# vthost/DAGNN

Hardware: AMD Instinct MI355X
Metric: graphs/sec (higher is better)
Workload: dtype f32

## Files before the change

### dagnn_amd/_lib.py

```python
from __future__ import annotations

import ctypes as C
import os
import threading

from . import build as _build

MAX_DIRS = 2
MAX_GROUPS = 4
MAX_READOUT_JOBS = 24
ATTN_GRAD_MAX_JOBS = 16

DAGNN_OK = 0
_ERRORS = {-22: "DAGNN_EINVAL (bad argument)", -28: "DAGNN_ENOSPC (workspace too small)"}


class DagnnHipError(RuntimeError):
    pass


class OptTensor(C.Structure):
    _fields_ = [("param", C.c_void_p), ("grad", C.c_void_p), ("exp_avg", C.c_void_p), ("exp_avg_sq", C.c_void_p), ("numel", C.c_int64)]


# ... 205 lines not shown

class DvaeSampleArgs(C.Structure):
    _fields_ = [("G", C.c_int64), ("B", C.c_int64), ("n", C.c_int), ("hs", C.c_int), ("L", C.c_int), ("nvt", C.c_int),
                ("start_type", C.c_int), ("end_type", C.c_int), ("bn", C.c_int), ("stochastic", C.c_int),
                ("edge_hidden", C.c_int), ("vertex_hidden", C.c_int), ("h0", C.c_void_p),
                ("w_ih", C.c_void_p * MAX_STACKED), ("w_hh", C.c_void_p * MAX_STACKED), ("b_ih", C.c_void_p * MAX_STACKED),
                ("b_hh", C.c_void_p * MAX_STACKED), ("w_key", C.c_void_p), ("vid_bias", C.c_void_p),
                ("av_w1", C.c_void_p), ("av_b1", C.c_void_p), ("av_w2", C.c_void_p), ("av_b2", C.c_void_p),
                ("ae_w1", C.c_void_p), ("ae_b1", C.c_void_p), ("ae_w2", C.c_void_p), ("ae_b2", C.c_void_p),
                ("u_type", C.c_void_p), ("u_edge", C.c_void_p), ("types", C.c_void_p), ("preds", C.c_void_p),
                ("nv", C.c_void_p), ("states", C.c_void_p), ("work", C.c_void_p), ("work_bytes", C.c_size_t),
                ("agg", C.c_int), ("gate_w", C.c_void_p), ("gate_b", C.c_void_p), ("mapper_w", C.c_void_p)]


DVAE_ENAS, DVAE_BN = 0, 1
DVAE_FIRST_VALID, DVAE_MOST_FREQUENT = 0, 1


class DvaeSelectArgs(C.Structure):
    _fields_ = [("A", C.c_int64), ("B", C.c_int64), ("n", C.c_int), ("nvt", C.c_int), ("start_type", C.c_int),
                ("end_type", C.c_int), ("kind", C.c_int), ("n_nodes", C.c_int), ("select", C.c_int),
                ("types", C.c_void_p), ("preds", C.c_void_p), ("nv", C.c_void_p), ("valid", C.c_void_p),
                ("pick", C.c_void_p), ("n_valid", C.c_void_p), ("n_same", C.c_void_p), ("work", C.c_void_p),
                ("work_bytes", C.c_size_t)]


LP_INT64, LP_FLOAT32, LP_FLOAT64 = 0, 1, 2
PREDICTOR_MAX_NZ, PREDICTOR_MAX_HS, PREDICTOR_ROWS = 128, 1024, 8
DVAE_SET_GRAPHS, DVAE_SET_KEYS = 0, 1
DVAE_SET_MAX_ROWS = 1 << 20
DVAE_SET_HEADER_WORDS, DVAE_SET_COUNT, DVAE_SET_ERR = 16, 4, 5
DVAE_SET_ERR_FULL, DVAE_SET_ERR_HEADER = 1, 2


class DvaeSameDagArgs(C.Structure):
    _fields_ = [("A", C.c_int64), ("B", C.c_int64), ("n", C.c_int), ("types", C.c_void_p), ("preds", C.c_void_p),
                ("nv", C.c_void_p), ("types_true", C.c_void_p), ("preds_true", C.c_void_p), ("nv_true", C.c_void_p),
                ("same", C.c_void_p), ("per_graph", C.c_void_p), ("total", C.c_void_p)]


class DvaeSet(C.Structure):
    _fields_ = [("form", C.c_int), ("width", C.c_int), ("max_rows", C.c_int64), ("data", C.c_void_p), ("bytes", C.c_size_t)]


class DvaeSetRowsArgs(C.Structure):
    _fields_ = [("set", DvaeSet), ("base", C.c_int64), ("A", C.c_int64), ("B", C.c_int64), ("types", C.c_void_p),
                ("preds", C.c_void_p), ("nv", C.c_void_p), ("keys", C.c_void_p), ("mask", C.c_void_p),
                ("member", C.c_void_p), ("count", C.c_void_p)]


class VariantBwdCell(C.Structure):
    _fields_ = [("mode", C.c_int32), ("lands", C.c_int32), ("in_dim", C.c_int32), ("proj_dim", C.c_int32),
                ("recurrent", C.c_int32), ("reserved", C.c_int32)] + \
        [(k, C.c_void_p) for k in ("h", "a", "gi", "gh", "node0", "node1", "alpha", "edge_mat0", "edge_vec0", "edge_mat1",
                                   "edge_vec1", "w_node", "w_query", "w_hh", "w_ih", "g", "g_in", "da", "dgi", "dgh",
                                   "dnode0", "dnode1", "dlogit", "esum", "w_node2")] + \
        [("w_ld", C.c_int32), ("ld_in", C.c_int32), ("ties", C.c_void_p)]


class VariantBwdArgs(C.Structure):
    _fields_ = [("cell", (VariantBwdCell * MAX_STACKED) * MAX_DIRS), ("num_stacked", C.c_int), ("dir_mask", C.c_int),
                ("H", C.c_int), ("ld", C.c_int)]


class VariantArgs(C.Structure):
    _fields_ = [("cell", (VariantCell * MAX_STACKED) * MAX_DIRS), ("num_stacked", C.c_int), ("dir_mask", C.c_int),
                ("H", C.c_int)]


class PrepTable(C.Structure):
    _fields_ = [("type_emb", C.c_void_p), ("attr_emb", C.c_void_p), ("depth_emb", C.c_void_p), ("out", C.c_void_p),
                ("width", C.c_int), ("ld_out", C.c_int)]


PREPARE_MAX_TABLES = 3


class PrepareRows(C.Structure):
    _fields_ = [("x", C.c_void_p), ("depth", C.c_void_p), ("max_depth", C.c_int), ("num_tables", C.c_int),
                ("table", PrepTable * PREPARE_MAX_TABLES), ("stack_src", C.c_void_p * 4), ("stack_out", C.c_void_p)]


class StoreGatherArgs(C.Structure):
    _fields_ = [(k, C.c_void_p) for k in ("node_ptr", "edge_ptr", "tok_ptr", "x", "depth", "layer_f", "layer_b", "src", "dst",
                                          "tok", "depth_max", "y_arr", "ref_ids", "ref_extra", "idx", "offsets")] + \
        [(k, C.c_int64) for k in ("ld_offsets", "B", "N", "E", "S", "R")] + \
        [(k, C.c_void_p) for k in ("out_x", "out_depth", "out_edge_index", "out_edge_attr", "out_batch", "out_ptr",
                                   "out_index0", "out_index1", "out_layer_f", "out_layer_b", "out_llp", "out_y_arr",
                                   "out_ref_ids", "out_ref_extra")]


class DagStoreGatherArgs(C.Structure):
    _fields_ = [(k, C.c_void_p) for k in ("types", "preds", "succs", "layer_f", "layer_b", "y", "idx", "offsets")] + \
        [(k, C.c_int64) for k in ("B", "n", "nvt", "E")] + \
        [(k, C.c_void_p) for k in ("out_x", "out_edge_index", "out_bi_layer_index", "out_batch", "out_ptr", "out_types",
                                   "out_preds", "out_y")]


BN_TABLE_CELLS, BN_MAX_VARS = 8192, 30
BN_STAGE_AUTO, BN_STAGE_LDS, BN_STAGE_GLOBAL = 0, 1, 2


class BnData(C.Structure):
    _fields_ = [("cols", C.c_void_p), ("ld", C.c_int64), ("S", C.c_int64), ("n_var", C.c_int32), ("reserved", C.c_int32),
                ("cards", C.c_int32 * BN_MAX_VARS)]


TABLE_GRADS_MAX_TABLES, TABLE_GRADS_CHUNK = 3, 32


class TableGradsTable(C.Structure):
    _fields_ = [("keys", C.c_void_p), ("key_stride", C.c_int64), ("R", C.c_int64), ("out", C.c_void_p), ("ld_out", C.c_int64)]


class TableGradsArgs(C.Structure):
    _fields_ = [("g", C.c_void_p), ("ld_g", C.c_int64), ("N", C.c_int64), ("H", C.c_int32), ("num_tables", C.c_int32),
                ("table", TableGradsTable * TABLE_GRADS_MAX_TABLES), ("workspace", C.c_void_p), ("workspace_bytes", C.c_size_t),
                ("stages", C.c_int32), ("reserved", C.c_int32)]


TABLE_GRADS_INDEX, TABLE_GRADS_SUM = 1, 2


SGP_MAX_M, SGP_MAX_D, SGP_MAX_Q = 512, 128, 128
SGP_ARGMIN_MEAN, SGP_ARGMIN_EI = 0, 1
SGP_REFINE_MAX_STARTS, SGP_REFINE_HISTORY = 32, 8
SGP_REFINE_MEAN, SGP_REFINE_EI = 0, 1
SGP_REFINE_STATUS = ("running", "converged", "stalled", "budget", "dead")

SYMBOLS = {
    "dagnn_version": (C.c_char_p, []),
    "dagnn_store_gather": (C.c_int, [C.POINTER(StoreGatherArgs), C.c_void_p]),
    "dagnn_dag_store_gather": (C.c_int, [C.POINTER(DagStoreGatherArgs), C.c_void_p]),
    "dagnn_dag_store_layers": (C.c_int, [C.c_void_p, C.c_void_p, C.c_int64, C.c_int, C.c_void_p, C.c_void_p, C.c_void_p]),
    "dagnn_plan_bytes": (C.c_size_t, [C.c_int64, C.c_int64, C.c_int64, C.c_int]),
    "dagnn_plan_is_small": (C.c_int, [C.c_int64, C.c_int64, C.c_int64]),
    "dagnn_plan_layout": (C.c_int, [C.c_int64, C.c_int64, C.c_int64, C.c_int, C.POINTER(C.c_int64)]),
    "dagnn_plan_build": (C.c_int, [C.POINTER(Plan), C.c_void_p, C.c_void_p, C.c_void_p, C.c_void_p, C.c_void_p,
                                   C.c_void_p, C.c_void_p]),
    "dagnn_prepare": (C.c_int, [C.POINTER(Plan), C.c_void_p, C.c_void_p, C.c_void_p, C.c_void_p, C.c_void_p, C.c_void_p,
                                C.c_void_p, C.c_size_t, C.c_int, C.c_int, C.c_int, C.POINTER(PrepareRows), C.c_void_p]),
    "dagnn_encode_ast": (C.c_int, [C.c_void_p, C.c_void_p, C.c_void_p, C.c_void_p, C.c_void_p, C.c_int, C.c_void_p,
                                   C.c_int, C.c_int64, C.c_int, C.c_void_p]),
    "dagnn_gemm_nt_bias": (C.c_int, [C.POINTER(GemmGroup), C.c_int, C.c_int64, C.c_int, C.c_int, C.c_int, C.c_int,
                                     C.c_int, C.c_void_p]),
    "dagnn_pack_whh": (C.c_int, [C.c_void_p, C.c_void_p, C.c_int, C.c_void_p]),
    "dagnn_recurrence_layer": (C.c_int, [C.POINTER(Plan), C.POINTER(LayerArgs), C.c_int, C.c_int, C.c_void_p]),
    "dagnn_pack_slices": (C.c_int, [C.c_void_p, C.c_void_p, C.c_int, C.c_int, C.c_int, C.c_void_p]),
    "dagnn_pack_batch": (C.c_int, [C.POINTER(PackJob), C.c_int, C.c_void_p]),
    "dagnn_pack_mfma": (C.c_int, [C.c_void_p, C.c_void_p, C.c_int, C.c_int, C.c_void_p]),
    "dagnn_frontier_run": (C.c_int, [C.POINTER(Plan), C.POINTER(FrontierArgs), C.POINTER(C.POINTER(C.c_int32)),
                                     C.POINTER(C.c_int32), C.c_void_p]),
    "dagnn_dataflow_groups": (C.c_int, [C.c_int, C.c_int, C.c_int, C.c_int, C.c_int64]),
    "dagnn_dataflow_bytes": (C.c_size_t, [C.c_int64, C.c_int64, C.c_int]),
    "dagnn_dataflow_layout": (C.c_int, [C.c_int64, C.c_int64, C.c_int, C.POINTER(C.c_int64)]),
    "dagnn_dataflow_schedule": (C.c_int, [C.POINTER(Plan), C.c_void_p, C.c_size_t, C.c_int, C.c_int, C.c_int,
                                          C.c_void_p, C.c_void_p]),
    "dagnn_dataflow_run": (C.c_int, [C.POINTER(Plan), C.POINTER(DataflowArgs), C.c_void_p]),
    "dagnn_dataflow_run_wide": (C.c_int, [C.POINTER(Plan), C.POINTER(DataflowArgs), C.c_void_p]),
    "dagnn_tiles_launches": (C.c_int, [C.c_int, C.c_int, C.c_int, C.c_int, C.c_int]),
    "dagnn_tiles_run": (C.c_int, [C.POINTER(Plan), C.POINTER(TilesArgs), C.c_void_p]),
    "dagnn_pack_dataflow": (C.c_int, [C.c_void_p, C.c_void_p, C.c_int, C.c_void_p]),
    "dagnn_pack_dataflow_transposed": (C.c_int, [C.c_void_p, C.c_void_p, C.c_int, C.c_void_p]),
    "dagnn_score_parts": (C.c_int, [C.c_void_p, C.c_int, C.c_int, C.c_void_p, C.c_int64, C.c_void_p]),
    "dagnn_backward_prepare": (C.c_int, [C.POINTER(Plan), C.POINTER(BackwardArgs), C.c_void_p]),
    "dagnn_backward_run": (C.c_int, [C.POINTER(Plan), C.POINTER(BackwardArgs), C.POINTER(C.POINTER(C.c_int32)),
                                     C.POINTER(C.c_int32), C.c_void_p]),
    "dagnn_bwd_dataflow_record_bytes": (C.c_size_t, [C.c_int64]),
    "dagnn_bwd_dataflow_static_bytes": (C.c_size_t, [C.c_int64]),
    "dagnn_bwd_dataflow_static_bytes_h": (C.c_size_t, [C.c_int64, C.c_int]),
    "dagnn_bwd_dataflow_prepare": (C.c_int, [C.POINTER(Plan), C.POINTER(BwdDataflowArgs), C.c_void_p]),
    "dagnn_bwd_dataflow_run": (C.c_int, [C.POINTER(Plan), C.POINTER(BwdDataflowArgs), C.c_void_p]),
    "dagnn_bwd_dataflow_run_wide": (C.c_int, [C.POINTER(Plan), C.POINTER(BwdDataflowArgs), C.c_void_p]),
    "dagnn_colsum_workspace_bytes": (C.c_size_t, [C.c_int, C.c_int]),
    "dagnn_colsum_run": (C.c_int, [C.POINTER(ColsumJob), C.c_int, C.c_int64, C.c_void_p, C.c_size_t, C.c_void_p]),
    "dagnn_wgrad_workspace_bytes": (C.c_size_t, [C.c_int, C.c_int, C.c_int, C.c_int]),
    "dagnn_wgrad_splits": (C.c_int, [C.c_int, C.c_int, C.c_int, C.c_int, C.c_int64]),
    "dagnn_wgrad_run": (C.c_int, [C.POINTER(WgradJob), C.c_int, C.c_int64, C.c_int, C.c_int, C.c_int, C.c_void_p,
                                  C.c_size_t, C.c_void_p]),
    "dagnn_table_grads_workspace_bytes": (C.c_size_t, [C.c_int64, C.c_int, C.POINTER(C.c_int64), C.c_int]),
    "dagnn_table_grads": (C.c_int, [C.POINTER(TableGradsArgs), C.c_void_p]),
    "dagnn_pack_dataflow_batch": (C.c_int, [C.POINTER(DfPackJob), C.c_int, C.c_int, C.c_void_p]),
    "dagnn_attn_grads_run": (C.c_int, [C.POINTER(AttnGradJob), C.c_int, C.c_void_p]),
    "dagnn_readout_pool_batch": (C.c_int, [C.POINTER(Plan), C.POINTER(PoolJob), C.c_int, C.c_void_p, C.c_int, C.c_void_p]),
    "dagnn_readout_pool_backward_batch": (C.c_int, [C.POINTER(Plan), C.POINTER(PoolBwdJob), C.c_int, C.c_void_p, C.c_int,
                                                    C.c_void_p]),
    "dagnn_topo_layers": (C.c_int, [C.c_void_p, C.c_void_p, C.c_int64, C.c_int64, C.c_int64, C.c_void_p, C.c_void_p,
                                    C.c_void_p, C.c_void_p]),
    "dagnn_variant_aggregate": (C.c_int, [C.POINTER(Plan), C.POINTER(VariantAggregator), C.c_int, C.c_int32, C.c_int32,
                                          C.c_void_p]),
    "dagnn_variant_run": (C.c_int, [C.POINTER(Plan), C.POINTER(VariantArgs), C.POINTER(C.POINTER(C.c_int32)),
                                    C.POINTER(C.c_int32), C.c_void_p]),
    "dagnn_variant_mattn_prepare": (C.c_int, [C.POINTER(Plan), C.POINTER(VariantBwdCell), C.c_int, C.c_int, C.c_int32,
                                              C.c_int32, C.c_void_p]),
    "dagnn_variant_max_prepare": (C.c_int, [C.POINTER(Plan), C.POINTER(VariantBwdCell), C.c_int, C.c_int, C.c_int, C.c_int32,
                                            C.c_int32, C.c_void_p]),
    "dagnn_plain_max_weights": (C.c_int, [C.POINTER(Plan), C.POINTER(PlainPull), C.c_int, C.c_int, C.c_int32, C.c_int32, C.c_void_p]),
    "dagnn_plain_edge_grads": (C.c_int, [C.POINTER(Plan), C.POINTER(PlainPull), C.c_int, C.c_int, C.c_int32, C.c_int32, C.c_void_p]),
    "dagnn_variant_aggregator_backward": (C.c_int, [C.POINTER(Plan), C.POINTER(VariantBwdCell), C.c_int, C.c_int, C.c_int32,
                                                    C.c_int32, C.c_void_p]),
    "dagnn_variant_backward_run": (C.c_int, [C.POINTER(Plan), C.POINTER(VariantBwdArgs), C.POINTER(C.POINTER(C.c_int32)),
                                             C.POINTER(C.c_int32), C.c_void_p]),
    "dagnn_vid_colsums": (C.c_int, [C.c_void_p, C.c_int64, C.c_int64, C.c_int, C.c_int, C.c_void_p, C.c_int64, C.c_void_p]),
    "dagnn_iprop_step": (C.c_int, [C.c_void_p, C.c_void_p, C.c_int64, C.c_int, C.c_int, C.c_void_p, C.c_void_p, C.c_void_p,
                                   C.c_void_p, C.c_int, C.POINTER(IpropLayer), C.c_int, C.c_void_p, C.c_void_p]),
    "dagnn_encode_forward": (C.c_int, [C.POINTER(EncodeArgs), C.c_void_p]),
    "dagnn_dvae_decode_saved_bytes": (C.c_size_t, [C.POINTER(DvaeDecodeArgs)]),
    "dagnn_dvae_decode_work_bytes": (C.c_size_t, [C.POINTER(DvaeDecodeArgs)]),
    "dagnn_dvae_decode_forward": (C.c_int, [C.POINTER(DvaeDecodeArgs), C.c_void_p]),
    "dagnn_dvae_decode_backward": (C.c_int, [C.POINTER(DvaeDecodeArgs), C.POINTER(DvaeDecodeGrads), C.c_void_p]),
    "dagnn_dvae_sample_work_bytes": (C.c_size_t, [C.POINTER(DvaeSampleArgs)]),
    "dagnn_dvae_sample": (C.c_int, [C.POINTER(DvaeSampleArgs), C.c_void_p]),
    "dagnn_dvae_select_key_words": (C.c_int, [C.c_int, C.c_int, C.c_int]),
    "dagnn_dvae_select_work_bytes": (C.c_size_t, [C.POINTER(DvaeSelectArgs)]),
    "dagnn_dvae_select": (C.c_int, [C.POINTER(DvaeSelectArgs), C.c_void_p]),
    "dagnn_dvae_same_dag": (C.c_int, [C.POINTER(DvaeSameDagArgs), C.c_void_p]),
    "dagnn_dvae_set_bytes": (C.c_size_t, [C.c_int, C.c_int, C.c_int64]),
    "dagnn_dvae_set_init": (C.c_int, [C.POINTER(DvaeSet), C.c_void_p]),
    "dagnn_dvae_set_add": (C.c_int, [C.POINTER(DvaeSetRowsArgs), C.c_void_p]),
    "dagnn_dvae_set_query": (C.c_int, [C.POINTER(DvaeSetRowsArgs), C.c_void_p]),
    "dagnn_debug_occupy": (C.c_int, [C.c_int, C.c_int, C.c_int64, C.c_void_p, C.c_void_p]),
    "dagnn_tn_product": (C.c_int, [C.c_void_p, C.c_int64, C.c_void_p, C.c_int64, C.c_int64, C.c_int, C.c_int, C.c_void_p, C.c_void_p,
                                   C.c_void_p]),
    "dagnn_seq_ce": (C.c_int, [C.c_void_p, C.c_int64, C.c_void_p, C.c_int, C.c_int, C.c_int, C.c_void_p, C.c_int64, C.c_void_p,
                               C.c_void_p, C.c_void_p, C.c_void_p]),
    "dagnn_heads_argmax_bytes": (C.c_size_t, [C.c_int64, C.c_int, C.c_int]),
    "dagnn_heads_argmax": (C.c_int, [C.c_void_p, C.c_int64, C.c_void_p, C.c_int64, C.c_void_p, C.c_int64, C.c_int, C.c_int, C.c_int,
                                     C.c_void_p, C.c_void_p, C.c_void_p, C.c_size_t, C.c_void_p]),
    "dagnn_heads_score_bytes": (C.c_size_t, [C.c_int64, C.c_int, C.c_int, C.c_int]),
    "dagnn_heads_score": (C.c_int, [C.c_void_p, C.c_int64, C.c_void_p, C.c_int64, C.c_void_p, C.c_int64, C.c_int, C.c_int, C.c_int,
                                    C.c_void_p, C.c_int, C.c_void_p, C.c_void_p, C.c_void_p, C.c_void_p, C.c_void_p, C.c_void_p,
                                    C.c_size_t, C.c_void_p]),
    "dagnn_rows_argmax": (C.c_int, [C.c_void_p, C.c_int64, C.c_int64, C.c_int, C.c_int, C.c_void_p, C.c_void_p]),
    "dagnn_seq_f1_counts": (C.c_int, [C.c_void_p, C.c_int64, C.c_int, C.c_int64, C.c_void_p, C.c_int, C.c_void_p, C.c_void_p,
                                      C.c_void_p]),
    "dagnn_graph_depth": (C.c_int, [C.c_void_p, C.c_void_p, C.c_int64, C.c_int64, C.c_void_p, C.c_void_p]),
    "dagnn_class_ce": (C.c_int, [C.c_void_p, C.c_int64, C.c_void_p, C.c_int, C.c_int, C.c_int, C.c_void_p, C.c_int64, C.c_void_p,
                                 C.c_void_p, C.c_void_p, C.c_void_p]),
    "dagnn_class_hits_bytes": (C.c_size_t, [C.c_int64, C.c_int]),
    "dagnn_class_hits": (C.c_int, [C.c_void_p, C.c_int64, C.c_void_p, C.c_int64, C.c_int, C.c_void_p, C.c_int, C.c_void_p, C.c_size_t,
                                   C.c_void_p, C.c_void_p, C.c_void_p]),
    "dagnn_seq_ce_step": (C.c_int, [C.c_void_p, C.c_int64, C.c_void_p, C.c_int, C.c_int, C.c_int, C.c_void_p, C.c_int64, C.c_void_p,
                                    C.c_void_p, C.c_void_p, C.c_int64, C.c_void_p, C.c_int, C.c_void_p, C.c_void_p, C.c_int64, C.c_int64,
                                    C.c_void_p, C.c_void_p, C.c_void_p, C.c_void_p]),
    "dagnn_class_ce_step": (C.c_int, [C.c_void_p, C.c_int64, C.c_void_p, C.c_int, C.c_int, C.c_int, C.c_void_p, C.c_int64, C.c_void_p,
                                      C.c_void_p, C.c_void_p, C.c_void_p, C.c_void_p, C.c_void_p, C.c_void_p, C.c_void_p]),
    "dagnn_predictor_mse_bytes": (C.c_size_t, [C.c_int, C.c_int, C.c_int, C.c_int]),
    "dagnn_predictor_mse": (C.c_int, [C.c_void_p, C.c_int64, C.c_void_p, C.c_int, C.c_int, C.c_int, C.c_void_p, C.c_void_p, C.c_void_p,
                                      C.c_void_p, C.c_void_p, C.c_void_p, C.c_void_p, C.c_void_p, C.c_size_t, C.c_void_p, C.c_int,
                                      C.c_void_p]),
    "dagnn_predictor_forward": (C.c_int, [C.c_void_p, C.c_int64, C.c_int64, C.c_int, C.c_int, C.c_void_p, C.c_void_p, C.c_void_p,
                                          C.c_void_p, C.c_void_p, C.c_void_p]),
    "dagnn_fit_sums_bytes": (C.c_size_t, [C.c_int64]),
    "dagnn_fit_sums": (C.c_int, [C.c_void_p, C.c_void_p, C.c_int, C.c_int64, C.c_double, C.c_double, C.c_void_p, C.c_void_p,
                                 C.c_size_t, C.c_void_p, C.c_void_p]),
    "dagnn_bn_stage_fits": (C.c_int, [C.POINTER(BnData)]),
    "dagnn_bn_score": (C.c_int, [C.POINTER(BnData), C.c_void_p, C.c_void_p, C.c_int64, C.c_int, C.c_void_p, C.c_void_p, C.c_void_p]),
    "dagnn_bn_rows_to_parents": (C.c_int, [C.c_void_p, C.c_void_p, C.c_void_p, C.c_int64, C.c_int, C.c_int, C.c_int, C.c_int,
                                           C.c_void_p, C.c_void_p, C.c_void_p]),
    "dagnn_sgp_project": (C.c_int, [C.c_void_p, C.c_int64, C.c_int64, C.c_int, C.c_int, C.c_void_p, C.c_int64, C.c_void_p, C.c_float,
                                    C.c_void_p, C.c_int64, C.c_int, C.c_int, C.c_void_p, C.c_void_p, C.c_int64, C.c_int, C.c_void_p,
                                    C.c_void_p, C.c_void_p, C.c_void_p]),
    "dagnn_sgp_ei_step_bytes": (C.c_size_t, [C.c_int64]),
    "dagnn_sgp_ei_step": (C.c_int, [C.c_int, C.c_int64, C.c_void_p, C.c_void_p, C.c_double, C.c_void_p, C.c_int64, C.c_int, C.c_void_p,
                                    C.c_float, C.c_void_p, C.c_void_p, C.c_int64, C.c_int, C.c_void_p, C.c_float, C.c_void_p, C.c_void_p,
                                    C.c_void_p, C.c_size_t, C.c_void_p, C.c_void_p]),
    "dagnn_sgp_energy_grad_bytes": (C.c_size_t, [C.c_int, C.c_int, C.c_int64]),
    "dagnn_sgp_energy_grad": (C.c_int, [C.c_void_p, C.c_int64, C.c_void_p, C.c_int64, C.c_int, C.c_int, C.c_double] + [C.c_void_p] * 14 +
                              [C.c_size_t, C.c_void_p, C.c_void_p]),
    "dagnn_sgp_refine_bytes": (C.c_size_t, [C.c_int, C.c_int, C.c_int]),
    "dagnn_sgp_refine_eval": (C.c_int, [C.c_int] * 5 + [C.c_void_p, C.c_void_p, C.c_void_p, C.c_int64, C.c_void_p, C.c_double, C.c_void_p, C.c_void_p, C.c_int64,
                                        C.c_int, C.c_double, C.c_void_p, C.c_void_p, C.c_size_t, C.c_void_p]),
    "dagnn_sgp_refine_run": (C.c_int, [C.c_int] * 5 + [C.c_void_p] * 6 + [C.c_int64, C.c_void_p, C.c_double, C.c_void_p, C.c_void_p, C.c_int64, C.c_int,
                                       C.c_double, C.c_int, C.c_void_p, C.c_void_p, C.c_void_p, C.c_size_t, C.c_void_p]),
    "dagnn_opt_chunks": (C.c_int64, [C.c_void_p, C.c_int]),
    "dagnn_grad_norm": (C.c_int, [C.c_void_p, C.c_void_p, C.c_int, C.c_void_p, C.c_int64, C.c_void_p, C.c_int, C.c_void_p, C.c_void_p]),
    "dagnn_clip_adam": (C.c_int, [C.c_void_p, C.c_int, C.c_double, C.c_double, C.c_double, C.c_double, C.c_double, C.c_int64, C.c_float,
                                  C.c_void_p, C.c_void_p]),
    "dagnn_score_parts_batch": (C.c_int, [C.c_void_p, C.c_void_p, C.c_int, C.c_int, C.c_int, C.c_int64, C.c_void_p]),
    "dagnn_param_fingerprint": (C.c_int, [C.c_void_p, C.c_void_p, C.c_int, C.c_void_p, C.c_int, C.c_void_p, C.c_int, C.c_void_p]),
    "dagnn_gather_rows_batch": (C.c_int, [C.POINTER(GatherJob), C.c_int, C.c_int64, C.c_int, C.c_void_p, C.c_int, C.c_void_p]),
    "dagnn_gather_rows": (C.c_int, [C.c_void_p, C.c_int, C.c_int, C.c_int64, C.c_int, C.c_int, C.c_void_p, C.c_int,
                                    C.c_int, C.c_void_p]),
}

_lock = threading.Lock()
_lib = None


def lib_path() -> str:
    return _build.LIB


def load():
    global _lib
    if _lib is not None:
        return _lib
    with _lock:
        if _lib is not None:
            return _lib
        path = _build.LIB
        if _build.is_stale():
            try:
                _build.build()
            except Exception as exc:
                if not os.path.exists(path):
                    raise DagnnHipError(
                        "libdagnn_hip.so is missing and could not be built (%s). There is no CPU or "
                        "PyTorch fallback for the DAGNN hot path." % exc) from exc
                if os.environ.get("DAGNN_AMD_ALLOW_STALE", "0") != "1":
                    raise DagnnHipError(
                        "%s is older than its sources and the rebuild failed (%s); refusing to load a library whose "
                        "ABI may differ from this package (set DAGNN_AMD_ALLOW_STALE=1 to load it anyway)" % (path, exc)) from exc
        try:
            lib = C.CDLL(path)
        except OSError as exc:
# ... 20 lines not shown
```

### dagnn_amd/core.py

```python
from __future__ import annotations

from typing import Callable, Dict, List, Optional, Sequence, Tuple

import torch
import torch.nn as nn

from . import engine
from . import route as routing
from ._lib import DagnnHipError


def round_up4(n: int) -> int:
    return (n + 3) // 4 * 4


def round_up(n: int, m: int) -> int:
    return (n + m - 1) // m * m


SCHEDULES = ("lockstep", "pergraph")


class DerivedCache(object):

# ... 16 lines not shown
            self._built = built_marker(params[0] if params else None)
        else:
            meet_built(self._built)
        return self._val


class ParamGuard(object):

    def __init__(self):
        self._key = None
        self._fp = None
        self._args = None

    def reset(self) -> None:
        self._key = None

    def check(self, params: Sequence[torch.Tensor], err: Optional[torch.Tensor]) -> None:
        if not engine.PARAM_GUARD or err is None or not params:
            return
        import ctypes as C
        key = tuple([(p.data_ptr(), p._version) for p in params])
        record = key != self._key
        if record or self._args is None:
            chunks = []
            cap = 96
            for o in range(0, len(params), cap):
                part = [p for p in params[o:o + cap]]
                ptrs = (C.c_void_p * len(part))(*[p.data_ptr() for p in part])
                numel = (C.c_int64 * len(part))(*[p.numel() if p.element_size() == 4 else 0 for p in part])
                chunks.append((ptrs, numel, len(part), o))
            self._args = chunks
            if self._fp is None or self._fp.numel() < len(params) or self._fp.device != err.device:
                self._fp = torch.empty(max(len(params), 1), dtype=torch.int64, device=err.device)
            self._key = key
        lib = engine._lib.load()
        st = engine._stream(err)
        for ptrs, numel, n, o in self._args:
            engine.check(lib.dagnn_param_fingerprint(ptrs, numel, n, self._fp.data_ptr() + 8 * o, 0 if record else 1,
                                                     err.data_ptr(), engine.ERR_PARAMS_MOVED, st), "dagnn_param_fingerprint")


class HipModule(nn.Module):

    def __init__(self):
        super().__init__()
        self._derived = {}
        self._arenas = {}

    def _cache(self, name: str) -> DerivedCache:
        c = self._derived.get(name)
        if c is None:
            c = self._derived[name] = DerivedCache()
        return c

    def invalidate_caches(self) -> None:
        for c in self._derived.values():
            c.invalidate()
        self.__dict__.pop("_param_guard", None)

    def train(self, mode: bool = True):
        self.invalidate_caches()
        return super().train(mode)

    def _guard_params(self, ref: torch.Tensor) -> None:
        if self.training or not engine.PARAM_GUARD or not ref.is_cuda:
            return
        g = self.__dict__.get("_param_guard")
        if g is None:
            params = [p for p in self.parameters() if p.is_cuda and p.dtype == torch.float32]
            g = self.__dict__["_param_guard"] = (ParamGuard(), params)
        g[0].check(g[1], self._arena_for(ref).error_word(ref.device))

    def check(self) -> None:
        for a in list(self._arenas.values()):
            a.check()

    def _arena_for(self, x, role="forward"):
        key = (role, x.device, engine._stream(x))
        arena = self._arenas.get(key)
        if arena is None:
            arena = engine.GranuleArena()
            arena.xcd_first = 2 * sum(1 for k in self._arenas if k[0] == role and k[1] == x.device) % 8
            self._arenas[key] = arena
        return arena

    def _train_params(self):
        flat = []
        for d in self.dirs:
            for i in range(self.num_layers):
                c = getattr(self, "cells_%d" % d)[i]
                a = getattr(self, "node_aggr_%d" % d)[i]
                flat += [c.weight_ih, c.weight_hh, c.bias_ih, c.bias_hh, a.attn_lin.weight, a.attn_lin.bias,
                         a.edge_encoder.weight if a.wea else None, a.edge_encoder.bias if a.wea else None]
        return flat

    def _unflatten(self, flat) -> List[List[Optional[torch.Tensor]]]:
        L = self.num_layers
        h: List[List[Optional[torch.Tensor]]] = [[None] * L for _ in range(2)]
        for q, d in enumerate(self.dirs):
            h[d] = list(flat[q * L:(q + 1) * L])
        return h


def built_marker(t):
    if t is None or not t.is_cuda:
        return None
    st = torch.cuda.current_stream(t.device)
    ev = torch.cuda.Event()
    ev.record(st)
    return (ev, st.cuda_stream, {st.cuda_stream}, t.device)


def meet_built(built) -> None:
    if built is None:
        return
    ev, _, seen, dev = built
    cur = torch.cuda.current_stream(dev)
    if cur.cuda_stream not in seen:
        cur.wait_event(ev)
        seen.add(cur.cuda_stream)


def _pad_gate_rows(w: torch.Tensor, H: int, Hp: int) -> torch.Tensor:
    if Hp == H:
        return w.contiguous()
    out = w.new_zeros((3 * Hp,) + tuple(w.shape[1:]))
    for g in range(3):
        out[g * Hp:g * Hp + H] = w[g * H:(g + 1) * H]
    return out


def _pad_cols(w: torch.Tensor, cols: int) -> torch.Tensor:
    if w.shape[-1] == cols:
        return w.contiguous()
    out = w.new_zeros(tuple(w.shape[:-1]) + (cols,))
    out[..., :w.shape[-1]] = w
    return out


class CellParams(object):

    __slots__ = ("w_ih", "b_ih", "w_hh_t", "b_hh", "w_key", "edge_gain", "vid_bias", "w_hh_pk", "w_ih_pk",
                 "b_ih_dev", "Hp", "key_raw", "w_hh_raw", "w_hh_df", "w_ih_df", "w_hh_bt", "w_ih_bt", "df_ok", "gain_src", "fold", "built",
                 "agg", "agg_w", "agg_b")


def pack_dataflow(cells, transposed_too: bool = False) -> None:
    cells = list(cells)
    todo = []
    for c in cells:
        if c.w_hh_df is None:
            todo.append((c, "w_hh_df", c.w_hh_raw, False))
            if c.b_ih_dev is not None:
                todo.append((c, "w_ih_df", c.w_ih, False))
        if transposed_too and c.w_hh_bt is None:
            todo.append((c, "w_hh_bt", c.w_hh_raw, True))
            if c.b_ih_dev is not None:
                todo.append((c, "w_ih_bt", c.w_ih, True))
    gains = [c for c in cells if c.gain_src is not None]
    if not todo:
        fill_gains(gains)
        if cells:
            meet_built(cells[0].built)
        return
    packed_all = engine.pack_dataflow_batch([(w, tr) for _, _, w, tr in todo], todo[0][0].Hp,
                                            gains=[(c.gain_src[0], c.gain_src[1], c.edge_gain) for c in gains])
    for c in gains:
        c.gain_src = None
    for (c, name, _, _), packed in zip(todo, packed_all):
        setattr(c, name, packed)
    marker = built_marker(packed_all[0])
    for c in cells:
        c.built = marker


def fill_gains(cells) -> None:
    for c in cells:
        if c.gain_src is not None:
            c.edge_gain.copy_(c.gain_src[0].t() @ c.gain_src[1])
            c.gain_src = None


def pack_lockstep(cells, force: bool = False) -> None:
    cells = list(cells)
    if cells and cells[0].df_ok and not force:
        pack_dataflow(cells)
        return
    fill_gains(cells)
    if cells and engine.TILES and cells[0].Hp == 512 and not force:
        return
    cells = [c for c in cells if c.w_hh_pk is None]
    todo = []
    for c in cells:
        todo.append((c, "w_hh_pk", c.w_hh_raw))
        if c.b_ih_dev is not None:
            todo.append((c, "w_ih_pk", c.w_ih))
    if not todo:
        return
    for (c, name, _), packed in zip(todo, engine.pack_batch([w for _, _, w in todo], todo[0][0].Hp)):
        setattr(c, name, packed)


def derive_cell(w_ih, w_hh, b_ih, b_hh, attn_w, H: int, dq: int, in_is_hidden: bool,
                edge_w: Optional[torch.Tensor], vid_nodes: int, schedule: str = "pergraph",
                key_dim: Optional[int] = None, pack: bool = True, stacked: int = 1) -> CellParams:
    lock = schedule == "lockstep"
    Hp, use_df = routing.width(H, stacked, 0 if edge_w is None else int(edge_w.shape[1]), key_dim is None or key_dim == H,
                             vid_nodes, edge_w is not None) if lock else (round_up4(H), False)
    c = CellParams()
    c.Hp = Hp
    c.fold = None
    c.built = None
    wi = _pad_gate_rows(w_ih.detach().float(), H, Hp)
    if in_is_hidden:
        wi = _pad_cols(wi, Hp)
    c.w_ih = wi
    c.b_ih = _pad_gate_rows(b_ih.detach().float(), H, Hp)
    whh = _pad_cols(_pad_gate_rows(w_hh.detach().float(), H, Hp), Hp)
    c.w_hh_raw = whh
    c.w_hh_t = None if lock else engine.pack_whh(whh)
    c.w_hh_pk = c.w_ih_pk = None
    c.w_hh_df = c.w_ih_df = None
    c.w_hh_bt = c.w_ih_bt = None
    c.df_ok = use_df
    if lock and pack and not use_df:
        c.w_hh_pk = {js: engine.pack_slices(whh, Hp, js) for js in (16, 32)}
        c.w_hh_pk["mfma"] = engine.pack_mfma(whh, Hp)
        if in_is_hidden:
            c.w_ih_pk = {js: engine.pack_slices(wi, Hp, js) for js in (16, 32)}
            c.w_ih_pk["mfma"] = engine.pack_mfma(wi, Hp)
    c.b_ih_dev = c.b_ih if (lock and in_is_hidden) else None
    if lock and pack and use_df:
        pack_dataflow([c])
    c.b_hh = _pad_gate_rows(b_hh.detach().float(), H, Hp)
    kd = H if key_dim is None else key_dim
    key = attn_w.detach().float()[0, dq:dq + kd]
    c.key_raw = key.contiguous()
    c.w_key = _pad_cols(key, Hp) if kd == H else None
    c.gain_src = None
    if edge_w is None:
        c.edge_gain = None
    elif pack or not lock:
        c.edge_gain = (edge_w.detach().float().t() @ key).contiguous()
    else:
        c.edge_gain = torch.empty(edge_w.shape[1], dtype=torch.float32, device=edge_w.device)
        c.gain_src = (edge_w.detach().float().contiguous(), c.key_raw)
    c.vid_bias = attn_w.detach().float()[0, dq + kd:dq + kd + vid_nodes].contiguous() if vid_nodes else None
    return c


_OFF_DATAFLOW_SEEN = set()


def _warn_off_dataflow(dev, ndirs: int, L: int, r: routing.Route) -> None:
    Hp, why = r.Hp, r.why
    key = (str(dev), ndirs, L, Hp)
    if why in routing.QUIET or key in _OFF_DATAFLOW_SEEN:
        return
    _OFF_DATAFLOW_SEEN.add(key)
    import warnings
    cells = ndirs * (2 * L - 1)
    cus = torch.cuda.get_device_properties(dev).multi_processor_count
    if why == routing.LIB and cells > 24:
        why = "%d kernel cells (directions x (2 x stacked layers - 1)) > 24" % cells
    elif why == routing.LIB and cells * (Hp // 32) > cus:
        why = "%d kernel cells x %d slices need more than the %d CUs of this device" % (cells, Hp // 32, cus)
    warnings.warn("dagnn_amd: this model (hidden %d, %d stacked layers, %d direction(s)) runs on the per-layer launch path, "
                  "not the persistent dataflow kernel: %s" % (Hp, L, ndirs, why), RuntimeWarning, stacklevel=3)


def run_stack_lockstep(plan: engine.PlanHandle, x: torch.Tensor, cells: Dict[Tuple[int, int], CellParams],
                       dirs: Sequence[int], L: int, H: int, vid_nodes: int = 0,
                       arena: Optional[engine.GranuleArena] = None, static_score=None,
                       record: Optional[engine.PassRecord] = None, gi0: Optional[Sequence[torch.Tensor]] = None,
                       route: Optional[routing.Route] = None) -> List[List[torch.Tensor]]:
    c0 = cells[(dirs[0], 0)]
    Hp, keys_hidden = c0.Hp, c0.w_key is not None and static_score is None
    N, dev = x.shape[0], x.device
    if gi0 is None:
        gi0 = engine.gemm_nt_bias([x] * len(dirs), [cells[(d, 0)].w_ih for d in dirs], [cells[(d, 0)].b_ih for d in dirs])
    gi = [None, None]
    for q, d in enumerate(dirs):
        gi[d] = gi0[q]
    ld = engine.frontier_ld(Hp)
    h = [[torch.empty(N, ld, dtype=torch.float32, device=dev) if d in dirs else None for _ in range(L)]
         for d in range(2)]
    plan.wait_ready()
    active, train = arena is not None and N > 0, record is not None
    if route is None or route.Hp != Hp:
        route = routing.before_plan(dev, H, L, len(dirs), plan.R, plan.B, keys_hidden, vid_nodes, c0.edge_gain is not None, train,
                                    Hp=Hp, active=active)
    route = routing.with_plan(route, dev, plan, dirs, L, N, keys_hidden, active, train)
    if arena is not None:
        arena.poll()
    if route.kind == "tiles":
        engine.tiles_run(plan, dirs, L, Hp, cells, gi, h, arena, vid_mod=vid_nodes)
    elif route.kind == "launches+tiles":
        pack_lockstep(cells.values(), force=True)
        engine.frontier_run(plan, dirs, L, Hp, cells, gi, h, vid_mod=vid_nodes, arena=None, static_score=static_score,
                            stop_layer=route.split, chains=arena)
        engine.tiles_run(plan, dirs, L, Hp, cells, gi, h, arena, first_layer=route.split, vid_mod=vid_nodes)
    elif route.kind == "dataflow":
        pack_dataflow(cells.values(), transposed_too=train and bool(engine.BWD_DATAFLOW))
        engine.dataflow_run(plan, dirs, L, Hp, cells, gi, h, route.groups, vid_mod=vid_nodes, arena=arena,
                            static_score=static_score, score_parts=train, record=record if engine.BWD_DATAFLOW else None,
                            training=train, stat_rows=route.stat_rows)
    else:
# ... 53 lines not shown
```

### dagnn_amd/csrc/dataflow.hip

```cpp
#include "sched_dev.h"
#include <type_traits>


namespace {

typedef float v2f __attribute__((ext_vector_type(2)));

__global__ void __launch_bounds__(256) df_assign_kernel(const int32_t* __restrict__ plan, PlanLayout L, int32_t* ws,
                                                         DfLayout S, int B, int G, int c_layer, int c_row, const int32_t* __restrict__ status) {
    if (status && status[0] != 0) return;
    if (blockIdx.x > 0) {
        df_fill_body(ws, S, (int64_t)(blockIdx.x - 1) * blockDim.x + threadIdx.x, (int64_t)(gridDim.x - 1) * blockDim.x);
        return;
    }
    constexpr int CAP = 4096;
    __shared__ int32_t s_g[CAP], s_d[CAP], s_n[CAP];
    df_assign_block<CAP>(plan, L, ws, S, B, G, c_layer, c_row, s_g, s_d, s_n);
}

__global__ void __launch_bounds__(256) df_count_kernel(const int32_t* __restrict__ plan, PlanLayout L, int32_t* ws,
                                                        DfLayout S, const int32_t* __restrict__ status) {
    if (status && status[0] != 0) return;
    df_count_body(plan, L, ws, S, blockIdx.x, blockIdx.y);
}

__global__ void __launch_bounds__(256) df_prefix_kernel(int32_t* ws, DfLayout S, int G, const int32_t* __restrict__ status) {
    if (status && status[0] != 0) return;
    df_prefix_body(ws, S, blockIdx.x, blockIdx.y);
}

__global__ void __launch_bounds__(64) df_base_kernel(int32_t* ws, DfLayout S, int G, const int32_t* __restrict__ status) {
    if (status && status[0] != 0) return;
    const int base = df_base_wave(ws, S, G, blockIdx.x, threadIdx.x);
    if ((int)threadIdx.x < G) ws[S.gtab[blockIdx.x] + 2 * threadIdx.x] = base;
}

__global__ void __launch_bounds__(256) df_lbase_kernel(const int32_t* __restrict__ plan, PlanLayout L, int32_t* ws,
                                                        DfLayout S, int B, int G, const int32_t* __restrict__ status) {
    if (status && status[0] != 0) return;
    df_lbase_body(plan, L, ws, S, B, G, blockIdx.x * 4 + (threadIdx.x >> 6), gridDim.x * 4, blockIdx.y);
}

__global__ void __launch_bounds__(256) df_records_kernel(const int32_t* __restrict__ plan, PlanLayout L, int32_t* ws,
                                                          DfLayout S, int N, const int32_t* __restrict__ status) {
    if (status && status[0] != 0) return;
    df_records_body(plan, L, ws, S, N, blockIdx.x, blockIdx.y, ws + S.gtab[blockIdx.y], 2);
}

enum { DF_RECURRENT = 0, DF_PROJECTION = 1 };
enum { DFK_REC0 = 0, DFK_RECP = 1, DFK_PROJ = 2 };
#ifdef DF_STAMPS
constexpr bool DF_PROF = true;
#else
constexpr bool DF_PROF = false;
#endif

typedef unsigned pgran_t __attribute__((ext_vector_type(4)));

struct DfCell {
    const float4* w;
    const float* bias;
    const float* wkey;
    const float* sscore;
    const float* gain;
    const float* vid;
    const float* gi0;
    const pgran_t* p_in;
    float* h_out;
    gran_t* g_out;
    const gran_t* g_in;
    float* aux_out;
    const float* agg_w;
    const float* agg_b;
    int dir;
    int kind;
    int variant;
    int partner;
    int agg;
};

#define DF_MAX_KCELLS 24
#define DF_MAX_WGS 320
#define DF_IDLE_ROLE 0xffffu

struct DfArgs {
    DfCell cell[DF_MAX_KCELLS];
    const int32_t* sched;
    int64_t gtab[2], grec[2];
    int64_t col[2], eattr[2];
    int ncell, H, ld_h, gld, pld, R, vid_mod, groups, N;
    unsigned epoch, spin_limit;
    int dbg_wg;
    const int32_t* status;
    int* err;
    unsigned long long* dbg;
    gran_t* xcc_tab;
    int nroles;
    int aux_stat;
    unsigned short role[DF_MAX_WGS];
};

static_assert(sizeof(DfArgs) + 8 <= 4096, "the cell and role tables must fit the kernel-argument segment");

__device__ __forceinline__ float df_dpp_row_sum16(float v) {
#define DF_DPP_ADD(ctrl) \
    v += __builtin_bit_cast(float, __builtin_amdgcn_update_dpp(0, __builtin_bit_cast(int, v), ctrl, 0xf, 0xf, true))
    DF_DPP_ADD(0x111); DF_DPP_ADD(0x112); DF_DPP_ADD(0x114); DF_DPP_ADD(0x118);
#undef DF_DPP_ADD
    return v;
}

__device__ __forceinline__ float df_wave_sum(float v) {
    v = df_dpp_row_sum16(v);
    v += __builtin_bit_cast(float, __builtin_amdgcn_update_dpp(0, __builtin_bit_cast(int, v), 0x142, 0xa, 0xf, false));
    v += __builtin_bit_cast(float, __builtin_amdgcn_update_dpp(0, __builtin_bit_cast(int, v), 0x143, 0xc, 0xf, false));
    return __builtin_bit_cast(float, __builtin_amdgcn_readlane(__builtin_bit_cast(int, v), 63));
}

__device__ __forceinline__ float df_sigm(float x) { return __builtin_amdgcn_rcpf(1.0f + __expf(-x)); }
__device__ __forceinline__ float df_tanh(float x) { return 1.0f - 2.0f * __builtin_amdgcn_rcpf(1.0f + __expf(2.0f * x)); }

static_assert(DF_NCW * 8 == DF_JS && DF_NLW % DF_NLS == 0 && DF_WPS == DF_RB, "workgroup shape: a loader wave per row of a block");
template <int KPT> struct DfPad { static constexpr int kp8 = 2 * KPT; static constexpr int seg = kp8 + 4; static constexpr int row = 8 * seg + 8; };

constexpr int DF_CSLEEP_N = 1;
constexpr int DF_WSLEEP_N = 1;
constexpr int DF_RD = 6;
constexpr int DF_GD = 2;
constexpr int DF_GI_LANES = 3 * DF_JS / 4;
constexpr int DF_GIRING = DF_NSLOT + DF_GD + 2;

__host__ inline int df_sets_for(int groups) { return (groups + DF_NLS - 1) / DF_NLS; }

struct DfLds {
    float* ring;
    float* giring;
    int* rec;
    int* rdy;
    int* dn;
    int* local;
    float* bias;
};

template <int KPT> struct DfSlot {
    static constexpr int AP = DfPad<KPT>::row;
    static constexpr int a_off = 0;
    static constexpr int gi_off = DF_RB * AP;
    static constexpr int v_off = gi_off + DF_RB * 3 * DF_JS;
    static constexpr int words = v_off + 4;
};

__device__ __forceinline__ int df_flag_ld(const int* p) { return __hip_atomic_load(p, __ATOMIC_RELAXED, __HIP_MEMORY_SCOPE_WORKGROUP); }
__device__ __forceinline__ void df_flag_st(int* p, int v) { __hip_atomic_store(p, v, __ATOMIC_RELAXED, __HIP_MEMORY_SCOPE_WORKGROUP); }

__device__ __forceinline__ bool df_wait4(const int* f, int target, int* err, unsigned limit) {
    unsigned spins = 0;
    for (;;) {
        int m = min(min(df_flag_ld(f), df_flag_ld(f + 1)), min(df_flag_ld(f + 2), df_flag_ld(f + 3)));
        if (m >= target) return true;
        __builtin_amdgcn_s_sleep(DF_WSLEEP_N);
        if (++spins > 4 * limit) { __hip_atomic_fetch_or(err, 2, __ATOMIC_RELAXED, __HIP_MEMORY_SCOPE_AGENT); return false; }
        if ((spins & 1023) == 0 && __hip_atomic_load(err, __ATOMIC_RELAXED, __HIP_MEMORY_SCOPE_AGENT) != 0) return false;
    }
}

__device__ __forceinline__ bool df_retry(unsigned& spins, int* err, unsigned limit) {
    __builtin_amdgcn_s_sleep(1);
    if (++spins > limit) { __hip_atomic_fetch_or(err, 1, __ATOMIC_RELAXED, __HIP_MEMORY_SCOPE_AGENT); return false; }
    if ((spins & 255) == 0 && __hip_atomic_load(err, __ATOMIC_RELAXED, __HIP_MEMORY_SCOPE_AGENT) != 0) return false;
    return true;
}

template <int KPT, int KIND, int RR, bool EXTRA, bool PLAIN = false>
__device__ __forceinline__ void df_loader(const int32_t* __restrict__ plan, const DfArgs& S,
                                          const DfCell& C, int sl, int group, const DfLds& lds, int w, int set) {
    constexpr int H = 16 * KPT;
    constexpr int SEG = DfPad<KPT>::seg, KP8 = DfPad<KPT>::kp8;
    typedef DfSlot<KPT> Slot;
    const int lane = threadIdx.x & 63;
    const int d = C.dir;
    const int32_t* tab = S.sched + S.gtab[d] + 2 * group;
    const int rec_base = tab[0], nblk = tab[1];
    const int32_t* __restrict__ recs = S.sched + S.grec[d] + 16 * (int64_t)rec_base;
    const int32_t* __restrict__ col = plan + S.col[d];
    const float* __restrict__ eattr = reinterpret_cast<const float*>(plan + S.eattr[d]);
    constexpr bool proj = KIND == DFK_PROJ;
    const int R = proj ? 0 : (RR >= 0 ? RR : (C.gain ? S.R : 0));
    const unsigned epoch = S.epoch, spin_limit = S.spin_limit;
    int* const err = S.err;
    const gran_t* const g_src = proj ? C.g_in : C.g_out;
    const int gld = S.gld, pld = S.pld;
    const pgran_t* const p_in = KIND == DFK_RECP ? C.p_in : nullptr;
    const float* const gi0 = KIND == DFK_REC0 ? C.gi0 : nullptr;
    const float* const sscore = EXTRA ? C.sscore : nullptr;
    const float* const vid = EXTRA ? C.vid : nullptr;
    const float* const gainp = proj ? nullptr : C.gain;
    const int vid_mod = EXTRA ? S.vid_mod : 1;
    const float gain0 = R >= 1 ? C.gain[0] : 0.f, gain1 = R >= 2 ? C.gain[1] : 0.f;
    unsigned long long* const dbg = (DF_PROF && S.dbg) ? S.dbg + 2 * gridDim.x : nullptr;
    const gran_t ready = (gran_t)epoch << 32;
    int* const dn = lds.dn + set * DF_NCW;
    constexpr int NQ4 = H / 64;
    float wk[4] = {0.f, 0.f, 0.f, 0.f};
    int cpos[4];
#pragma unroll
    for (int q = 0; q < 4; ++q) {
        const int c = 64 * q + lane;
        cpos[q] = c + (SEG - KP8) * (c / KP8);
        if (!proj && !PLAIN && !(EXTRA && C.sscore) && q < NQ4) wk[q] = C.wkey[c];
    }
    const int agg = PLAIN ? C.agg : 0;
    const int Rp = (PLAIN && C.agg_w) ? S.R : 0;
    float ew0[4] = {0.f, 0.f, 0.f, 0.f}, ew1[4] = {0.f, 0.f, 0.f, 0.f}, ebv[4] = {0.f, 0.f, 0.f, 0.f};
    if (PLAIN && C.agg_w) {
#pragma unroll
        for (int q = 0; q < 4; ++q) {
            const int c = 64 * q + lane;
            if (q < NQ4) {
                if (Rp >= 1) ew0[q] = C.agg_w[(int64_t)c * Rp];
                if (Rp >= 2) ew1[q] = C.agg_w[(int64_t)c * Rp + 1];
                ebv[q] = C.agg_b ? C.agg_b[c] : 0.f;
            }
        }
    }
    const bool prof_wave = DF_PROF && dbg != nullptr && (int)blockIdx.x == S.dbg_wg && w == 0 && lane == 0;
    bool prof = prof_wave;

    struct Sweep { gran_t x[4][4]; pgran_t xp; };
    const unsigned lane8 = 8u * lane, lanepx16 = 16u * (lane & (DF_JS - 1));
    constexpr bool has_gi0 = KIND == DFK_REC0;
#define DF_ROW_LD(e)                                                            \
    "global_load_dwordx2 %[x" #e "0], %[vo], %[b" #e "] offset:0 sc1\n\t"        \
    "global_load_dwordx2 %[x" #e "1], %[vo], %[b" #e "] offset:%[o1] sc1\n\t"    \
    "global_load_dwordx2 %[x" #e "2], %[vo], %[b" #e "] offset:%[o2] sc1\n\t"    \
    "global_load_dwordx2 %[x" #e "3], %[vo], %[b" #e "] offset:%[o3] sc1\n\t"
#define DF_ROWS_0 ""
#define DF_ROWS_1 DF_ROW_LD(0)
#define DF_ROWS_2 DF_ROWS_1 DF_ROW_LD(1)
#define DF_ROWS_3 DF_ROWS_2 DF_ROW_LD(2)
#define DF_ROWS_4 DF_ROWS_3 DF_ROW_LD(3)
#define DF_PROJ_0 ""
#define DF_PROJ_1 "global_load_dwordx4 %[p0], %[vp], %[c0] offset:0 sc1\n\t"
#define DF_DMA_0 "s_waitcnt vmcnt(0)"
#define DF_DMA_1                                                                                   \
    "s_mov_b32 %[km], m0\n\ts_mov_b64 %[ke], exec\n\ts_mov_b64 exec, 0xffff\n\ts_mov_b32 m0, %[rl]\n\t" \
    "s_nop 0\n\tglobal_load_lds_dword %[ra], off\n\t"                                              \
    "s_mov_b64 exec, %[ke]\n\ts_mov_b32 m0, %[km]\n\ts_waitcnt vmcnt(1)"
#define DF_DMA_2                                                                                   \
    "s_mov_b32 %[km], m0\n\ts_mov_b64 %[ke], exec\n\ts_mov_b64 exec, 0xffff\n\ts_mov_b32 m0, %[rl]\n\t" \
    "s_nop 0\n\tglobal_load_lds_dword %[ra], off\n\t"                                              \
    "s_bfm_b64 exec, %[gx], 0\n\ts_mov_b32 m0, %[gl]\n\ts_nop 0\n\tglobal_load_lds_dwordx4 %[ga], off\n\t" \
    "s_mov_b64 exec, %[ke]\n\ts_mov_b32 m0, %[km]\n\ts_waitcnt vmcnt(2)"
#define DF_TRIP(n, p, d)                                                                                                   \
    asm volatile(DF_ROWS_##n DF_PROJ_##p DF_DMA_##d                                                                        \
                 : [x00] "=v"(W.x[0][0]), [x01] "=v"(W.x[0][1]), [x02] "=v"(W.x[0][2]), [x03] "=v"(W.x[0][3]),             \
                   [x10] "=v"(W.x[1][0]), [x11] "=v"(W.x[1][1]), [x12] "=v"(W.x[1][2]), [x13] "=v"(W.x[1][3]),             \
                   [x20] "=v"(W.x[2][0]), [x21] "=v"(W.x[2][1]), [x22] "=v"(W.x[2][2]), [x23] "=v"(W.x[2][3]),             \
                   [x30] "=v"(W.x[3][0]), [x31] "=v"(W.x[3][1]), [x32] "=v"(W.x[3][2]), [x33] "=v"(W.x[3][3]),             \
                   [p0] "=v"(W.xp), [km] "=&s"(keep_m0), [ke] "=&s"(keep_exec), [ra] "+v"(ra), [ga] "+v"(ga)  \
                 : [vo] "v"(lane8), [vp] "v"(lanepx16), [b0] "s"(b0), [b1] "s"(b1), [b2] "s"(b2), [b3] "s"(b3),            \
                   [c0] "s"(c0p), [rl] "s"(rl), [gl] "s"(gl),    \
                   [o1] "n"(O1), [o2] "n"(O2), [o3] "n"(O3), [gx] "n"(DF_GI_LANES)                                          \
                 : "memory")
#define DF_CASE(n, p, d) case (n) * 6 + (p) * 3 + (d): DF_TRIP(n, p, d); break;
#define DF_CASES(n) DF_CASE(n, 0, 0) DF_CASE(n, 0, 1) DF_CASE(n, 0, 2) DF_CASE(n, 1, 0) DF_CASE(n, 1, 1) DF_CASE(n, 1, 2)

    int lw = w * DF_RPW;
    int* rec_ring;
    unsigned rec_ring_a, gi_ring_a;
    const int32_t* rec_w;
    auto set_row = [&](int row) {
        lw = row;
        rec_ring = lds.rec + (set * DF_RB + lw) * (8 * 16);
        rec_ring_a = __builtin_amdgcn_readfirstlane((unsigned)(uintptr_t)rec_ring);
        gi_ring_a = __builtin_amdgcn_readfirstlane((unsigned)(uintptr_t)(lds.giring + (set * DF_GIRING * DF_RB + lw) * (3 * DF_JS)));
        rec_w = recs + 16 * lw + (lane & 15);
    };
    set_row(lw);
    const int64_t wstride = 16 * DF_RB;
    const int gi_lane_off = ((lane % DF_GI_LANES) / (DF_JS / 4)) * H + sl * DF_JS + 4 * (lane % (DF_JS / 4));
    auto rec_src = [&](int j) -> const void* { return rec_w + (int64_t)min(j, nblk - 1) * wstride; };
    auto rec_dst = [&](int j) -> unsigned { return rec_ring_a + (j & 7) * 64; };
    auto gi_src = [&](int node) -> const void* { return gi0 + (int64_t)max(node, 0) * 3 * H + gi_lane_off; };
    auto gi_dst = [&](int blk) -> unsigned { return gi_ring_a + (blk % DF_GIRING) * (DF_RB * 3 * DF_JS * 4); };
    auto glds4 = [&](const void* gsrc, unsigned lds_dst) {
        unsigned keep;
        asm volatile("s_mov_b32 %0, m0\n\ts_mov_b32 m0, %2\n\ts_nop 0\n\tglobal_load_lds_dword %1, off\n\ts_mov_b32 m0, %0"
                     : "=&s"(keep) : "v"(gsrc), "s"(lds_dst) : "memory");
    };
    auto glds16 = [&](const void* gsrc, unsigned lds_dst) {
        unsigned keep;
        asm volatile("s_mov_b32 %0, m0\n\ts_mov_b32 m0, %2\n\ts_nop 0\n\tglobal_load_lds_dwordx4 %1, off\n\ts_mov_b32 m0, %0"
                     : "=&s"(keep) : "v"(gsrc), "s"(lds_dst) : "memory");
    };
    auto rec_dma = [&](int j) { if (lane < 16) glds4(rec_src(j), rec_dst(j)); };
    auto gi_dma = [&](int blk, int node) { if (lane < DF_GI_LANES) glds16(gi_src(node), gi_dst(blk)); };
    if (nblk > 0) {
        for (int rr = 0; rr < DF_RPW; ++rr) {
            set_row(w * DF_RPW + rr);
#pragma unroll
            for (int j = 0; j < DF_RD; ++j) rec_dma(j);
            asm volatile("s_waitcnt vmcnt(0)" ::: "memory");
            if (has_gi0) {
#pragma unroll
                for (int j = 0; j < DF_GD; ++j) gi_dma(j, __builtin_amdgcn_readfirstlane(rec_ring[j * 16]));
                asm volatile("s_waitcnt vmcnt(0)" ::: "memory");
            }
        }
    }

    Sweep A;
    for (int b = 0; b < nblk; ++b) {
      const int j = b;
      bool slot_free = b < DF_NSLOT;
#pragma unroll 1
      for (int rr = 0; rr < DF_RPW; ++rr) {
        if (DF_RPW > 1) { set_row(w * DF_RPW + rr); prof = prof_wave && rr == 0; }
        const int cur = rec_ring[(j & 7) * 16 + (lane & 15)];
#define DF_W(i) __builtin_amdgcn_readlane(cur, i)
        const int4 r0 = make_int4(DF_W(0), DF_W(1), DF_W(2), DF_W(3));
        const int4 r1 = make_int4(DF_W(4), DF_W(5), DF_W(6), DF_W(7));
        const int4 r2 = make_int4(DF_W(8), DF_W(9), DF_W(10), DF_W(11));
        const int4 r3 = make_int4(DF_W(12), DF_W(13), DF_W(14), DF_W(15));
#undef DF_W
        const int v2 = __builtin_amdgcn_readfirstlane(rec_ring[((j + DF_GD) & 7) * 16]);
        const int slot = b % DF_NSLOT;
        float* sbase = lds.ring + (set * DF_NSLOT + slot) * Slot::words;
        int* v_s = reinterpret_cast<int*>(sbase + Slot::v_off);
        const int v = r0.x;
        if (prof) dbg[8 * (int64_t)(DF_NLS * b + set) + 4] = wall_clock64();
        unsigned polls = 0;
        constexpr int O1 = (NQ4 > 1 ? 1 : 0) * 512, O2 = (NQ4 > 2 ? 2 : NQ4 - 1) * 512, O3 = (NQ4 - 1) * 512;
        auto trip = [&](Sweep& W, int nn, bool pp, int dma, const int (&pj)[4], const pgran_t* gp_in) {
            const gran_t* b0 = g_src + (unsigned)pj[0] * (unsigned)gld;
            const gran_t* b1 = g_src + (unsigned)pj[1] * (unsigned)gld;
            const gran_t* b2 = g_src + (unsigned)pj[2] * (unsigned)gld;
            const gran_t* b3 = g_src + (unsigned)pj[3] * (unsigned)gld;
            const pgran_t* c0p = gp_in;
            const void* ra = rec_src(j + DF_RD);
            const unsigned rl = rec_dst(j + DF_RD);
            const void* ga = has_gi0 ? gi_src(v2) : ra;
            const unsigned gl = gi_dst(b + DF_GD);
            unsigned keep_m0;
            unsigned long long keep_exec;
            switch (nn * 6 + (pp ? 3 : 0) + dma) {
                DF_CASES(0) DF_CASES(1) DF_CASES(2) DF_CASES(3)
                default: DF_CASES(4)
            }
        };
        if (v >= 0) {
            const int eb = r0.y;
            const int deg = proj ? 1 : ((PLAIN && agg == 3) ? 0 : r0.z - r0.y);
            float acc[4] = {0.f, 0.f, 0.f, 0.f};
            float m = -INFINITY, l = 0.f;
            bool p_pending = KIND == DFK_RECP;
            float pv[3] = {0.f, 0.f, 0.f};
            const pgran_t* gp_in = p_pending ? p_in + (unsigned)v * (unsigned)pld + sl * DF_JS : reinterpret_cast<const pgran_t*>(g_src);
            float ff0[4] = {0.f, 0.f, 0.f, 0.f}, ff1[4] = {0.f, 0.f, 0.f, 0.f};
            auto chunk_ids = [&](int c0, int (&pj)[4], float (&fe)[4]) -> int {
                const int nn = max(0, min(4, deg - c0));
#pragma unroll
                for (int e = 0; e < 4; ++e) { pj[e] = 0; fe[e] = 0.f; }
                if (PLAIN && Rp > 0) {
                    if (c0 == 0) {
                        ff0[0] = __int_as_float(r2.x); ff0[1] = __int_as_float(r2.z); ff0[2] = __int_as_float(r3.x); ff0[3] = __int_as_float(r3.z);
                        if (Rp >= 2) { ff1[0] = __int_as_float(r2.y); ff1[1] = __int_as_float(r2.w); ff1[2] = __int_as_float(r3.y); ff1[3] = __int_as_float(r3.w); }
                    } else {
#pragma unroll
                        for (int e = 0; e < 4; ++e) {
                            ff0[e] = ff1[e] = 0.f;
                            if (e < nn) {
                                ff0[e] = eattr[(int64_t)(eb + c0 + e) * Rp];
                                if (Rp >= 2) ff1[e] = eattr[(int64_t)(eb + c0 + e) * Rp + 1];
                            }
                        }
                    }
                }
                if (proj) {
                    pj[0] = v;
                } else if (c0 == 0) {
                    pj[0] = r1.x; pj[1] = r1.y; pj[2] = r1.z; pj[3] = r1.w;
                    if (R >= 1 && R <= 2) {
                        fe[0] = gain0 * __int_as_float(r2.x) + gain1 * __int_as_float(r2.y);
                        fe[1] = gain0 * __int_as_float(r2.z) + gain1 * __int_as_float(r2.w);
                        fe[2] = gain0 * __int_as_float(r3.x) + gain1 * __int_as_float(r3.y);
                        fe[3] = gain0 * __int_as_float(r3.z) + gain1 * __int_as_float(r3.w);
                    }
                } else {
#pragma unroll
                    for (int e = 0; e < 4; ++e) if (e < nn) pj[e] = col[eb + c0 + e];
                }
                if (R > 2 || (R > 0 && c0 > 0)) {
#pragma unroll
                    for (int e = 0; e < 4; ++e) {
                        fe[e] = 0.f;
                        if (e < nn) for (int r = 0; r < R; ++r) fe[e] = fmaf(gainp[r], eattr[(int64_t)(eb + c0 + e) * R + r], fe[e]);
                    }
                }
                return nn;
            };
            auto arrived = [&](const Sweep& W, int nn) -> bool {
                bool all = true;
#pragma unroll
                for (int e = 0; e < 4; ++e) {
                    if (e < nn) {
                        bool ok = true;
#pragma unroll
                        for (int q = 0; q < 4; ++q) ok = ok && (unsigned)(W.x[e][q] >> 32) == epoch;
                        all = all && __all(ok);
                    }
                }
                return all;
            };
            auto fold_n = [&](auto nn_c, const int (&pj)[4], const float (&fe)[4], const Sweep& W) {
                constexpr int NN = decltype(nn_c)::value;
#define DF_ROW(e, q) __uint_as_float((unsigned)W.x[e][q])
                float s[NN];
#pragma unroll
                for (int e = 0; e < NN; ++e) s[e] = DF_ROW(e, 0) * wk[0] + DF_ROW(e, 1) * wk[1] + DF_ROW(e, 2) * wk[2] + DF_ROW(e, 3) * wk[3];
                if (!sscore) {
#pragma unroll
                    for (int e = 0; e < NN; ++e) s[e] = df_wave_sum(s[e]);
                }
                float mc = m;
#pragma unroll
                for (int e = 0; e < NN; ++e) {
                    float sv = sscore ? sscore[pj[e]] : s[e];
                    if (vid) sv += vid[pj[e] % vid_mod];
                    sv += fe[e];
                    s[e] = sv;
                    mc = fmaxf(mc, sv);
                }
                const float sc = __expf(m - mc);
#pragma unroll
                for (int q = 0; q < 4; ++q) acc[q] *= sc;
                l *= sc;
#pragma unroll
                for (int e = 0; e < NN; ++e) {
                    const float p = __expf(s[e] - mc);
                    l += p;
#pragma unroll
                    for (int q = 0; q < 4; ++q) acc[q] = fmaf(p, DF_ROW(e, q), acc[q]);
                }
                m = mc;
#undef DF_ROW
            };
            auto fold = [&](const int (&pj)[4], const float (&fe)[4], int nn, const Sweep& W) {
                switch (nn) {
                    case 1: fold_n(std::integral_constant<int, 1>(), pj, fe, W); break;
                    case 2: fold_n(std::integral_constant<int, 2>(), pj, fe, W); break;
                    case 3: fold_n(std::integral_constant<int, 3>(), pj, fe, W); break;
                    default: fold_n(std::integral_constant<int, 4>(), pj, fe, W); break;
                }
            };
            int c0 = 0;
            do {
                int pj[4];
                float fe[4];
                const int nn = chunk_ids(c0, pj, fe);
                unsigned spins = 0;
                unsigned long long t_issue = 0ull;
                int dma = c0 == 0 ? (has_gi0 ? 2 : 1) : 0;
                for (;;) {
                    if (prof) t_issue = wall_clock64();
                    trip(A, nn, p_pending, dma, pj, gp_in);
                    dma = 0;
                    const bool rows_ok = arrived(A, nn);
                    if (p_pending) {
                        if (__all(A.xp.x == epoch)) {
                            pv[0] = __uint_as_float(A.xp.y); pv[1] = __uint_as_float(A.xp.z); pv[2] = __uint_as_float(A.xp.w);
                            p_pending = false;
                        }
                    }
                    ++polls;
                    if ((rows_ok && !p_pending) || !df_retry(spins, err, spin_limit)) break;
                }
                if (prof && c0 == 0) {
                    dbg[8 * (int64_t)(DF_NLS * b + set) + 5] = wall_clock64(); dbg[8 * (int64_t)(DF_NLS * b + set) + 6] = polls;
                    if (DF_NLS * b + set >= 8) dbg[8 * (int64_t)(DF_NLS * b + set) + 7] = t_issue;
                }
                if (PLAIN) {
#pragma unroll
                    for (int e = 0; e < 4; ++e) {
                        if (e < nn) {
#pragma unroll
                            for (int q = 0; q < 4; ++q) {
                                const float mv = __uint_as_float((unsigned)A.x[e][q]) + fmaf(ff0[e], ew0[q], fmaf(ff1[e], ew1[q], ebv[q]));
                                acc[q] = agg == 2 ? ((c0 == 0 && e == 0) ? mv : fmaxf(acc[q], mv)) : acc[q] + mv;
                            }
                        }
                    }
                } else if (deg == 1) {
#pragma unroll
                    for (int q = 0; q < 4; ++q) acc[q] = __uint_as_float((unsigned)A.x[0][q]);
                    l = 1.f;
                } else if (nn > 0) {
                    fold(pj, fe, nn, A);
                }
                c0 += 4;
            } while (c0 < deg);
            if (prof) { asm volatile("" :: "v"(acc[0]), "v"(acc[3]), "v"(l)); dbg[(1 << 19) + 8 * (int64_t)(DF_NLS * b + set) + 4] = wall_clock64(); }
            if (deg > 1 && !PLAIN) {
                const float inv = __builtin_amdgcn_rcpf(l + 1e-16f);
#pragma unroll
                for (int q = 0; q < 4; ++q) acc[q] *= inv;
            }
            if (!slot_free) { df_wait4(dn, b - DF_NSLOT + 1, err, spin_limit); slot_free = true; }
            float* a_row = sbase + Slot::a_off + lw * Slot::AP;
#pragma unroll
            for (int q = 0; q < NQ4; ++q) a_row[cpos[q]] = acc[q];
            if (KIND == DFK_RECP && lane < DF_JS) {
#pragma unroll
                for (int g = 0; g < 3; ++g) sbase[Slot::gi_off + lw * (3 * DF_JS) + g * DF_JS + lane] = pv[g];
            }
        } else {
            const int none[4] = {0, 0, 0, 0};
            trip(A, 0, false, has_gi0 ? 2 : 1, none, reinterpret_cast<const pgran_t*>(g_src));
            if (!slot_free) { df_wait4(dn, b - DF_NSLOT + 1, err, spin_limit); slot_free = true; }
        }
        if (lane == 0) v_s[lw] = v;
      }
        if (prof_wave) dbg[(1 << 19) + 8 * (int64_t)(DF_NLS * b + set) + 5] = wall_clock64();
        asm volatile("s_waitcnt lgkmcnt(0)" ::: "memory");
        if (lane == 0) df_flag_st(lds.rdy + set * DF_WPS + w, b + 1);
        if (prof_wave) dbg[8 * (int64_t)(DF_NLS * b + set) + 3] = wall_clock64();
    }
    asm volatile("s_waitcnt vmcnt(0)" ::: "memory");
#undef DF_TRIP
#undef DF_CASE
#undef DF_CASES
}

struct DfSweep { gran_t x[4][5]; pgran_t xp; };
// ... 369 lines not shown
    const bool local_st = !proj && lds.local[0] != 0;
    const int ld_h = S.ld_h, gld = S.gld, pld = S.pld, num_nodes = S.N;
    unsigned long long* const dbg = (DF_PROF && S.dbg) ? S.dbg + 2 * gridDim.x : nullptr;
    const bool prof = DF_PROF && dbg != nullptr && (int)blockIdx.x == S.dbg_wg && cw == 0 && lane == 0;

    typedef int i4v __attribute__((ext_vector_type(4)));
    typedef __attribute__((address_space(3))) const volatile i4v* lds_i4p;
    const lds_i4p rdy_p = (lds_i4p)(uintptr_t)(unsigned)(uintptr_t)lds.rdy;
    const bool lane_st = (lane & 16) == 0;
    int* const dn_or_dump = lane == 0 ? lds.dn + cw : reinterpret_cast<int*>(lds.bias) + lane;
    const int dn_step = lane == 0 ? DF_NCW : 0;
    const int nb0 = nb[0], nb1 = nb[1];
    static_assert(DF_NLS == 2 && DF_WPS == 4, "two streams per workgroup, four ready flags each");

    auto run = [&](auto local_c, auto aux_c) {
        constexpr bool LOCAL = decltype(local_c)::value;
        constexpr int AUX = decltype(aux_c)::value;
        int done0 = 0, done1 = 0, pref = 0;
        int m0 = 0, m1 = 0;
        auto flags_min = [&](const i4v& r0, const i4v& r1) {
            m0 = __builtin_amdgcn_readfirstlane(min(min(r0.x, r0.y), min(r0.z, r0.w)));
            m1 = __builtin_amdgcn_readfirstlane(min(min(r1.x, r1.y), min(r1.z, r1.w)));
        };
        for (int left = nb0 + nb1; left > 0; --left) {
            int l0 = m0 - done0, l1 = m1 - done1;
            if (l0 <= 0 && l1 <= 0) {
                unsigned spins = 0;
                for (;;) {
                    const i4v r0 = rdy_p[0], r1 = rdy_p[1];
                    flags_min(r0, r1);
                    l0 = m0 - done0; l1 = m1 - done1;
                    if (l0 > 0 || l1 > 0) break;
                    __builtin_amdgcn_s_sleep(DF_CSLEEP_N);
                    bool give_up = false;
                    if (++spins > 4 * spin_limit) {
                        __hip_atomic_fetch_or(err, 2, __ATOMIC_RELAXED, __HIP_MEMORY_SCOPE_AGENT);
                        give_up = true;
                    }
                    if ((spins & 1023) == 0 && __hip_atomic_load(err, __ATOMIC_RELAXED, __HIP_MEMORY_SCOPE_AGENT) != 0) give_up = true;
                    if (give_up) { l0 = nb0 - done0; l1 = nb1 - done1; break; }
                }
            }
            const unsigned k0 = ((unsigned)(l0 - 1) << 1) | (unsigned)pref, k1 = ((unsigned)(l1 - 1) << 1) | (unsigned)(pref ^ 1);
            const int st = k1 < k0 ? 1 : 0;
            pref = st ^ 1;
            const int b = st ? done1 : done0;
            done0 += st ^ 1;
            done1 += st;
            const float* sbase = lds.ring + (st * DF_NSLOT + (b & (DF_NSLOT - 1))) * Slot::words;
            static_assert((DF_NSLOT & (DF_NSLOT - 1)) == 0 && (DF_GIRING & (DF_GIRING - 1)) == 0, "ring sizes are powers of two");
            if (prof) dbg[8 * (int64_t)(DF_NLS * b + st) + 0] = wall_clock64();
            const int gv = reinterpret_cast<const int*>(sbase + Slot::v_off)[row_l];
            float gi_r = 0.f, gi_z = 0.f, gi_n = 0.f, aval = 0.f;
            if (!proj) {
                const float* gp = (gi_ring ? lds.giring + (st * DF_GIRING + (b & (DF_GIRING - 1))) * (DF_RB * 3 * DF_JS) : sbase + Slot::gi_off) +
                                  row_l * (3 * DF_JS) + unit_l;
                gi_r = gp[0]; gi_z = gp[DF_JS]; gi_n = gp[2 * DF_JS];
                aval = sbase[Slot::a_off + row_l * Slot::AP + apos];
            }
            float g3[3];
            float rg = 0.f, zg = 0.f;
            {
                const float* a_seg = sbase + Slot::a_off + x * Slot::AP + ks * SEG;
                float4 bv[NK4];
#pragma unroll
                for (int q = 0; q < NK4; ++q) bv[q] = *reinterpret_cast<const float4*>(a_seg + 4 * q);
                if (KPT <= 16) __builtin_amdgcn_sched_barrier(0);
                f4v acc[3] = {(f4v){0.f, 0.f, 0.f, 0.f}, (f4v){0.f, 0.f, 0.f, 0.f}, (f4v){0.f, 0.f, 0.f, 0.f}};
                auto reduce = [&](const f4v& A) -> float {
                    float e0, e1, f;
                    asm("s_nop 5\n\t"
                        "v_add_f32_dpp %0, %3, %3 row_shl:4 row_mask:0xf bank_mask:0x5\n\t"
                        "v_add_f32_dpp %1, %4, %4 row_shl:4 row_mask:0xf bank_mask:0x5\n\t"
                        "v_add_f32_dpp %0, %5, %5 row_shr:4 row_mask:0xf bank_mask:0xa\n\t"
                        "v_add_f32_dpp %1, %6, %6 row_shr:4 row_mask:0xf bank_mask:0xa\n\t"
                        "s_nop 1\n\t"
                        "v_add_f32_dpp %2, %0, %0 row_shl:8 row_mask:0xf bank_mask:0x3\n\t"
                        "v_add_f32_dpp %2, %1, %1 row_shr:8 row_mask:0xf bank_mask:0xc"
                        : "=&v"(e0), "=&v"(e1), "=&v"(f) : "v"(A[0]), "v"(A[1]), "v"(A[2]), "v"(A[3]));
                    return df_row_pair_sum(f);
                };
#pragma unroll
                for (int q = 0; q < NK4; ++q) {
                    const float bq[4] = {bv[q].x, bv[q].y, bv[q].z, bv[q].w};
#pragma unroll
                    for (int e = 0; e < 4; ++e) {
                        acc[0] = __builtin_amdgcn_mfma_f32_4x4x1f32(bq[e], wr[4 * q + e], acc[0], 0, 0, 0);
                        acc[1] = __builtin_amdgcn_mfma_f32_4x4x1f32(bq[e], wz[4 * q + e], acc[1], 0, 0, 0);
                        acc[2] = __builtin_amdgcn_mfma_f32_4x4x1f32(bq[e], wn[4 * q + e], acc[2], 0, 0, 0);
                    }
                }
                {
                    __builtin_amdgcn_sched_barrier(0);
                    const i4v r0 = rdy_p[0], r1 = rdy_p[1];
#pragma unroll
                    for (int a = 0; a < 3; ++a) g3[a] = reduce(acc[a]);
                    flags_min(r0, r1);
                }
            }
            if (prof) dbg[8 * (int64_t)(DF_NLS * b + st) + 1] = wall_clock64();
            const float p_r = g3[0] + b_r, p_z = g3[1] + b_z, p_n = g3[2] + b_n;
            float hv = 0.f, ng = 0.f;
            if (!proj) {
                rg = df_sigm(p_r + gi_r);
                zg = df_sigm(p_z + gi_z);
                ng = df_tanh(fmaf(rg, p_n, gi_n));
                hv = fmaf(zg, aval - ng, ng);
            }
            asm volatile("s_waitcnt lgkmcnt(0)" ::: "memory");
            df_flag_st(dn_or_dump + st * dn_step, b + 1);
            if (lane_st && (unsigned)gv < (unsigned)num_nodes) {
                if (proj) {
                    pgran_t* po = reinterpret_cast<pgran_t*>(g_out) + df_idx(gv, pld, unit);
                    const pgran_t pv = {epoch, __float_as_uint(p_r), __float_as_uint(p_z), __float_as_uint(p_n)};
                    asm volatile("global_store_dwordx4 %0, %1, off sc1" :: "v"(po), "v"(pv) : "memory");
                } else {
                    if (LOCAL) g_out[df_idx(gv, gld, unit)] = gran_pack(epoch, hv);
                    else __hip_atomic_store(g_out + df_idx(gv, gld, unit), gran_pack(epoch, hv), __ATOMIC_RELAXED, __HIP_MEMORY_SCOPE_AGENT);
                    h_out[df_idx(gv, ld_h, unit)] = hv;
                }
                if (AUX == 1) {
                    float* ao = aux_out + df_idx(gv, 3 * H, unit);
                    ao[0] = p_r; ao[H] = p_z; ao[2 * H] = p_n;
                }
                if (AUX == 2 && !proj) {
                    const float cn = (1.0f - zg) * (1.0f - ng * ng);
                    const float cz = (aval - ng) * zg * (1.0f - zg);
                    const float cr = cn * p_n * rg * (1.0f - rg);
                    const float cnr = cn * rg;
                    const float cq = zg * aval + cr * (p_r - b_r) + cz * (p_z - b_z) + cnr * (p_n - b_n);
                    char* const rec = reinterpret_cast<char*>(aux_out) + ((unsigned)gv * (unsigned)(4 * df_stat_floats(H)) + stat_col);
                    auto put = [&](auto rs_c) {
                        constexpr int RS = 4 * decltype(rs_c)::value;
                        *reinterpret_cast<float*>(rec + DF_ST_H * RS) = hv; *reinterpret_cast<float*>(rec + DF_ST_CR * RS) = cr;
                        *reinterpret_cast<float*>(rec + DF_ST_CZ * RS) = cz; *reinterpret_cast<float*>(rec + DF_ST_CNR * RS) = cnr;
                        *reinterpret_cast<float*>(rec + DF_ST_CN * RS) = cn; *reinterpret_cast<float*>(rec + DF_ST_Z * RS) = zg;
                        *reinterpret_cast<float*>(rec + DF_ST_CQ * RS) = cq;
                    };
                    if (H > 256 && sl >= 256 / DF_JS) put(std::integral_constant<int, 64>());
                    else put(std::integral_constant<int, DF_STAT_SP>());
                }
            }
            if (prof) dbg[8 * (int64_t)(DF_NLS * b + st) + 2] = wall_clock64();
        }
    };
    typedef std::integral_constant<int, 0> aux0;
    typedef std::integral_constant<int, 1> aux1;
    typedef std::integral_constant<int, 2> aux2;
    if (!aux_out) { if (local_st) run(std::true_type(), aux0()); else run(std::false_type(), aux0()); }
    else if (proj || !S.aux_stat) { if (local_st) run(std::true_type(), aux1()); else run(std::false_type(), aux1()); }
    else { if (local_st) run(std::true_type(), aux2()); else run(std::false_type(), aux2()); }
}

template <int KPT>
__global__ void __launch_bounds__(DF_THREADS, DF_THREADS / 256) dataflow_kernel(const int32_t* __restrict__ plan, DfArgs S) {
    extern __shared__ __attribute__((aligned(16))) float smem[];
    typedef DfSlot<KPT> Slot;
    constexpr int NS = 16 * KPT / DF_JS;
    const int tid = threadIdx.x;
    if (S.status && S.status[0] != 0) {
        if (tid == 0) __hip_atomic_fetch_or(S.err, 4 | ((S.status[0] & 0xff) << 8), __ATOMIC_RELAXED, __HIP_MEMORY_SCOPE_AGENT);
        return;
    }
    if (S.sched[0] != S.groups || S.sched[1] != DF_MAGIC || S.sched[2] != DF_RB) {
        if (tid == 0) __hip_atomic_fetch_or(S.err, 8, __ATOMIC_RELAXED, __HIP_MEMORY_SCOPE_AGENT);
        return;
    }
    const int wave = __builtin_amdgcn_readfirstlane(tid >> 6);
    int pair, c, sl;
    if (S.nroles > 0) {
        const unsigned role = S.role[blockIdx.x];
        if (role == DF_IDLE_ROLE) return;
        pair = (int)(role >> 10); c = (int)((role >> 5) & 31u); sl = (int)(role & 31u);
    } else {
        const int per_pair = S.ncell * NS;
        pair = blockIdx.x / per_pair;
        const int rem = blockIdx.x - pair * per_pair;
        c = rem / NS; sl = rem - c * NS;
    }
    const DfCell& C = S.cell[c];
    DfLds lds;
    lds.ring = smem;
    lds.giring = lds.ring + DF_NLS * DF_NSLOT * Slot::words;
    lds.rec = reinterpret_cast<int*>(lds.giring + DF_NLS * DF_GIRING * DF_RB * 3 * DF_JS);
    int* flags = lds.rec + DF_NLS * DF_RB * 8 * 16;
    lds.rdy = flags;
    lds.dn = flags + DF_NLW;
    lds.local = flags + DF_NLW + DF_NLS * DF_NCW;
    lds.bias = reinterpret_cast<float*>(flags + 32);
    if (tid < DF_NLW + DF_NLS * DF_NCW + 1) flags[tid] = 0;
    static_assert(DF_NLW + DF_NLS * DF_NCW + 1 <= 32, "flag words");
    if (tid >= 64 && tid < 64 + 3 * DF_JS) lds.bias[tid - 64] = C.bias[((tid - 64) / DF_JS) * (16 * KPT) + sl * DF_JS + (tid - 64) % DF_JS];
    if (S.nroles > 0 && wave == 0) {
        unsigned xcc;
        asm volatile("s_getreg_b32 %0, hwreg(HW_REG_XCC_ID)" : "=s"(xcc));
        xcc &= 15u;
        if ((tid & 63) == 0)
            __hip_atomic_store(S.xcc_tab + blockIdx.x, gran_pack(S.epoch, __uint_as_float(xcc)), __ATOMIC_RELAXED, __HIP_MEMORY_SCOPE_AGENT);
        if (C.kind == DF_RECURRENT) {
            bool same = true;
            for (int b0 = 0; b0 < S.nroles; b0 += 64) {
                const int b = b0 + (tid & 63);
                const unsigned r = b < S.nroles ? S.role[b] : DF_IDLE_ROLE;
                const int rc = (int)((r >> 5) & 31u);
                const bool member = r != DF_IDLE_ROLE && (int)(r >> 10) == pair && (rc == c || rc == C.partner);
                unsigned spins = 0;
                bool have = !member;
                unsigned theirs = xcc;
                for (;;) {
                    if (!have) {
                        const gran_t g = gran_ld(S.xcc_tab + b);
                        if ((unsigned)(g >> 32) == S.epoch) { theirs = (unsigned)g; have = true; }
                    }
                    if (__all(have) || !df_retry(spins, S.err, S.spin_limit)) break;
                }
                same = same && have && theirs == xcc;
            }
            if (__all(same) && (tid & 63) == 0) lds.local[0] = 1;
        }
    }
    if (DF_PROF && S.dbg && tid == 0) S.dbg[2 * blockIdx.x] = wall_clock64();
    if (DF_PROF && S.dbg && (int)blockIdx.x == S.dbg_wg && (tid & 63) == 0)
        if (wave < 8) S.dbg[2 * gridDim.x + 8 * (int64_t)wave + 7] = 0x100000000ull | __builtin_amdgcn_s_getreg(4 | (0 << 6) | (31 << 11));
    __syncthreads();
    const int variant = C.variant;
    if (wave < DF_NCW) {
        const int cw = wave;
        switch ((variant >> 2) & 3) {
            case DFK_REC0: df_compute<KPT, DFK_REC0>(S, C, sl, pair, lds, cw); break;
            case DFK_RECP: df_compute<KPT, DFK_RECP>(S, C, sl, pair, lds, cw); break;
            default: df_compute<KPT, DFK_PROJ>(S, C, sl, pair, lds, cw); break;
        }
    } else {
        const int set = (wave - DF_NCW) / DF_WPS;
        const int grp = df_group_of_stream(pair, set, S.groups);
        const int w = (wave - DF_NCW) % DF_WPS;
        if (grp >= 0) {
#define DF_LOADER_CASE(K, RR, EX) case (K) * 4 + ((RR) == 2 ? 2 : 0) + ((EX) ? 1 : 0): df_loader<KPT, K, RR, EX>(plan, S, C, sl, grp, lds, w, set); break;
            if (variant == DFK_REC0 * 4 + 2) { df_loader_fast<KPT, DFK_REC0>(plan, S, C, sl, grp, lds, w, set); }
            else if (variant == DFK_RECP * 4 + 2) { df_loader_fast<KPT, DFK_RECP>(plan, S, C, sl, grp, lds, w, set); }
            else if ((variant >> 2) == DFK_PROJ) { df_loader_fast<KPT, DFK_PROJ>(plan, S, C, sl, grp, lds, w, set); }
            else if constexpr (KPT <= 16) {
                if (variant >= 16) {
                    if (((variant >> 2) & 3) == DFK_REC0) df_loader<KPT, DFK_REC0, -1, false, true>(plan, S, C, sl, grp, lds, w, set);
                    else df_loader<KPT, DFK_RECP, -1, false, true>(plan, S, C, sl, grp, lds, w, set);
                } else
                switch (variant) {
                    DF_LOADER_CASE(DFK_REC0, 2, false) DF_LOADER_CASE(DFK_REC0, 2, true)
                    DF_LOADER_CASE(DFK_REC0, -1, false) DF_LOADER_CASE(DFK_REC0, -1, true)
                    DF_LOADER_CASE(DFK_RECP, 2, false) DF_LOADER_CASE(DFK_RECP, 2, true)
                    DF_LOADER_CASE(DFK_RECP, -1, false) DF_LOADER_CASE(DFK_RECP, -1, true)
                    default: df_loader<KPT, DFK_PROJ, -1, false>(plan, S, C, sl, grp, lds, w, set); break;
                }
            } else {
                if (tid % 64 == 0) __hip_atomic_fetch_or(S.err, 8, __ATOMIC_RELAXED, __HIP_MEMORY_SCOPE_AGENT);
            }
#undef DF_LOADER_CASE
        }
    }
    if (DF_PROF && S.dbg && tid == 0) S.dbg[2 * blockIdx.x + 1] = wall_clock64();
}

template <int KPT> size_t df_lds_bytes() {
    return (size_t)DF_NLS * (DF_NSLOT * DfSlot<KPT>::words + DF_GIRING * DF_RB * 3 * DF_JS + DF_RB * 8 * 16) * 4 + 128 + 3 * DF_JS * 4 + 128;
}

struct DfPackPos { int sl, g, k4, unit, ks, kp; };
__device__ __forceinline__ DfPackPos df_pack_pos(int64_t idx, int H, bool transposed) {
    (void)transposed;
    DfPackPos P;
    P.kp = H >> 3;
    const int nk4 = P.kp >> 2, nq = 3 * nk4;
    const int tc = (int)(idx & 255);
    const int64_t rest = idx >> 8;
    const int q = (int)(rest % nq);
    P.sl = (int)(rest / nq);
    P.g = q / nk4; P.k4 = q - P.g * nk4;
    P.unit = P.sl * DF_JS + 8 * (tc >> 6) + 4 * ((tc >> 5) & 1) + (tc & 3); P.ks = (tc >> 2) & 7;
    return P;
}

__global__ void __launch_bounds__(256) df_pack_kernel(const float* __restrict__ W, float4* __restrict__ out, int H, int64_t total,
                                                       int transposed) {
    for (int64_t idx = (int64_t)blockIdx.x * blockDim.x + threadIdx.x; idx < total; idx += (int64_t)gridDim.x * blockDim.x) {
        const DfPackPos P = df_pack_pos(idx, H, transposed != 0);
        const int sl = P.sl, g = P.g, k4 = P.k4, unit = P.unit, ks = P.ks, kp8 = P.kp;
        (void)sl;
        if (!transposed) {
            out[idx] = *reinterpret_cast<const float4*>(W + (int64_t)(g * H + unit) * H + ks * kp8 + 4 * k4);
        } else {
            const float* src = W + (int64_t)(g * H + ks * kp8 + 4 * k4) * H + unit;
            out[idx] = make_float4(src[0], src[H], src[2 * (int64_t)H], src[3 * (int64_t)H]);
        }
    }
}

struct DfPackJobs { dagnn_df_pack_job j[DAGNN_MAX_PACK_JOBS]; };
__global__ void __launch_bounds__(256) df_pack_batch_kernel(DfPackJobs P, int H, int64_t total) {
    const dagnn_df_pack_job& J = P.j[blockIdx.y];
    const float* __restrict__ W = J.w;
    if (J.transposed == 2) {
        if (blockIdx.x == 0 && (int)threadIdx.x < J.cols) {
            float acc = 0.f;
            for (int j = 0; j < J.rows; ++j) acc = fmaf(W[(int64_t)j * J.cols + threadIdx.x], J.aux[j], acc);
            J.out[threadIdx.x] = acc;
        }
        return;
    }
    float4* __restrict__ out = reinterpret_cast<float4*>(J.out);
    for (int64_t idx = (int64_t)blockIdx.x * blockDim.x + threadIdx.x; idx < total; idx += (int64_t)gridDim.x * blockDim.x) {
        const DfPackPos P = df_pack_pos(idx, H, J.transposed != 0);
        const int g = P.g, k4 = P.k4, unit = P.unit, ks = P.ks, kp8 = P.kp;
        if (!J.transposed) {
            out[idx] = *reinterpret_cast<const float4*>(W + (int64_t)(g * H + unit) * H + ks * kp8 + 4 * k4);
        } else {
            const float* src = W + (int64_t)(g * H + ks * kp8 + 4 * k4) * H + unit;
            out[idx] = make_float4(src[0], src[H], src[2 * (int64_t)H], src[3 * (int64_t)H]);
        }
    }
}

struct DfScoreJobs { float* h[DAGNN_MAX_PACK_JOBS]; const float* wkey[DAGNN_MAX_PACK_JOBS]; };
__global__ void __launch_bounds__(256) df_score_parts_kernel(DfScoreJobs J, int ld_h, int H, int64_t N) {
    float* __restrict__ h = J.h[blockIdx.y];
    const float* __restrict__ wkey = J.wkey[blockIdx.y];
    const int lane = threadIdx.x & 63;
    const int64_t v = (int64_t)blockIdx.x * 4 + (threadIdx.x >> 6);
    if (v >= N) return;
    float* row = h + v * ld_h;
    for (int l4 = lane; 4 * l4 < ((H + 255) & ~255); l4 += 64) {
        float s = 0.f;
        if (4 * l4 < H) {
            const float4 x = reinterpret_cast<const float4*>(row)[l4];
            const float4 w = reinterpret_cast<const float4*>(wkey)[l4];
            s = x.x * w.x + x.y * w.y + x.z * w.z + x.w * w.w;
        }
        s += __shfl_xor(s, 1, 64);
        s += __shfl_xor(s, 2, 64);
        if ((l4 & 3) == 0 && 4 * l4 < H) row[H + (l4 >> 2)] = s;
    }
}

}

#if defined(DF_WIDE_TU)
constexpr int DF_TU_MAX_H = 320;
#else
constexpr int DF_TU_MAX_H = 256;
extern "C" size_t dagnn_dataflow_bytes(int64_t N, int64_t B, int groups) {
    if (N < 0 || B < 0 || groups < 1 || groups > DF_MAX_GROUPS) return 0;
    return (size_t)df_layout_words(N, B, groups).total * sizeof(int32_t);
}

extern "C" int dagnn_dataflow_layout(int64_t N, int64_t B, int groups, int64_t* o) {
    if (!o || groups < 1 || groups > DF_MAX_GROUPS) return DAGNN_EINVAL;
    DfLayout S = df_layout_words(N, B, groups);
    const int64_t w[13] = {S.grp_of, S.gdepth, S.gload, S.loff, S.gtab[0], S.gtab[1], S.lcnt[0], S.lcnt[1],
                           S.glbase[0], S.glbase[1], S.grec[0], S.grec[1], S.total};
    for (int i = 0; i < 13; ++i) o[i] = w[i] * 4;
    return DAGNN_OK;
}

extern "C" int dagnn_dataflow_groups(int num_cus, int num_dirs, int num_stacked, int H, int64_t B) {
    if (num_cus <= 0 || num_dirs < 1 || num_dirs > DAGNN_MAX_DIRS || num_stacked < 1 || H <= 0 || (H % 64) || H > 320 || B <= 0)
        return 0;
    const int kcells = num_dirs * (2 * num_stacked - 1);
    if (kcells > DF_MAX_KCELLS) return 0;
    int64_t g = (int64_t)DF_NLS * (num_cus / (kcells * (H / DF_JS)));
    if (g > DF_MAX_GROUPS) g = DF_MAX_GROUPS;
    if (g > B) g = B;
    return (int)g;
}

extern "C" int dagnn_dataflow_schedule(const dagnn_plan* pl, void* ws_, size_t ws_bytes, int groups, int cost_layer,
                                       int cost_row, const int32_t* status, void* stream_) {
    if (!pl || !pl->data || !ws_ || groups < 1 || groups > DF_MAX_GROUPS || cost_layer < 0 || cost_row < 0)
        return DAGNN_EINVAL;
    const int64_t N = pl->N, B = pl->B;
    DfLayout S = df_layout_words(N, B, groups);
    if ((size_t)S.total * 4 > ws_bytes) return DAGNN_ENOSPC;
    PlanLayout L = dagnn_plan_layout_words(pl->N, pl->E, pl->B, pl->num_edge_feats);
    hipStream_t st = (hipStream_t)stream_;
    int32_t* ws = (int32_t*)ws_;
    const int32_t* plan = (const int32_t*)pl->data;
    if (B == 0 || N == 0) {
        hipError_t e = hipMemsetAsync(ws, 0, (size_t)S.grec[0] * 4, st);
        if (e != hipSuccess) return DAGNN_EHIP(e);
        e = hipMemsetAsync(ws + S.grec[0], 0xff, (size_t)(S.total - S.grec[0]) * 4, st);
        return e == hipSuccess ? DAGNN_OK : DAGNN_EHIP(e);
    }
    if (!(pl->flags & DAGNN_PLAN_GENERAL_BUILD) && dagnn_plan_is_small(N, 0, B))
        return dagnn_dataflow_schedule_small(pl, ws, groups, cost_layer, cost_row, status, st);
    hipLaunchKernelGGL(df_assign_kernel, dim3(1 + 512), dim3(256), 0, st, plan, L, ws, S, (int)B, groups, cost_layer, cost_row, status);
    DAGNN_CHECK_LAUNCH();
    hipLaunchKernelGGL(df_count_kernel, dim3((unsigned)B, 2), dim3(256), 0, st, plan, L, ws, S, status);
    DAGNN_CHECK_LAUNCH();
    hipLaunchKernelGGL(df_prefix_kernel, dim3((unsigned)groups, 2), dim3(256), 0, st, ws, S, groups, status);
    DAGNN_CHECK_LAUNCH();
    hipLaunchKernelGGL(df_base_kernel, dim3(2), dim3(64), 0, st, ws, S, groups, status);
    DAGNN_CHECK_LAUNCH();
    int64_t lb = (N + groups + 3) / 4;
    if (lb > 2048) lb = 2048;
    hipLaunchKernelGGL(df_lbase_kernel, dim3((unsigned)lb, 2), dim3(256), 0, st, plan, L, ws, S, (int)B, groups, status);
    DAGNN_CHECK_LAUNCH();
    hipLaunchKernelGGL(df_records_kernel, dim3((unsigned)((N + 255) / 256), 2), dim3(256), 0, st, plan, L, ws, S, (int)N, status);
    DAGNN_CHECK_LAUNCH();
    return DAGNN_OK;
}

static int df_pack(const float* w, float* out, int H, int transposed, void* stream) {
    if (!w || !out || H <= 0 || (H % 64) || H > 320) return DAGNN_EINVAL;
    const int64_t total = (int64_t)3 * H * H / 4;
    int64_t blocks = (total + 255) / 256;
    if (blocks > 4096) blocks = 4096;
    hipLaunchKernelGGL(df_pack_kernel, dim3((unsigned)blocks), dim3(256), 0, (hipStream_t)stream, w,
                       reinterpret_cast<float4*>(out), H, total, transposed);
    DAGNN_CHECK_LAUNCH();
    return DAGNN_OK;
}

extern "C" int dagnn_pack_dataflow(const float* w, float* out, int H, void* stream) { return df_pack(w, out, H, 0, stream); }

extern "C" int dagnn_pack_dataflow_transposed(const float* w, float* out, int H, void* stream) { return df_pack(w, out, H, 1, stream); }

extern "C" int dagnn_pack_dataflow_batch(const dagnn_df_pack_job* jobs, int njob, int H, void* stream) {
    if (!jobs || njob <= 0 || njob > DAGNN_MAX_PACK_JOBS || H <= 0 || (H % 64) || H > 320) return DAGNN_EINVAL;
    DfPackJobs P;
    for (int q = 0; q < njob; ++q) {
        if (!jobs[q].w || !jobs[q].out) return DAGNN_EINVAL;
        if (jobs[q].transposed == 2 && (!jobs[q].aux || jobs[q].rows <= 0 || jobs[q].cols <= 0 || jobs[q].cols > 256)) return DAGNN_EINVAL;
        P.j[q] = jobs[q];
    }
    const int64_t total = (int64_t)3 * H * H / 4;
    int64_t blocks = (total + 255) / 256;
    if (blocks > 1024) blocks = 1024;
    hipLaunchKernelGGL(df_pack_batch_kernel, dim3((unsigned)blocks, (unsigned)njob), dim3(256), 0, (hipStream_t)stream, P, H, total);
    DAGNN_CHECK_LAUNCH();
    return DAGNN_OK;
}

extern "C" int dagnn_score_parts_batch(float* const* h, const float* const* w_key, int n, int ld_h, int H, int64_t N, void* stream) {
    if (!h || !w_key || n <= 0 || n > DAGNN_MAX_PACK_JOBS || H <= 0 || (H % 16) || ld_h < H + H / 16 || N < 0) return DAGNN_EINVAL;
    if (N == 0) return DAGNN_OK;
    DfScoreJobs J;
    for (int q = 0; q < n; ++q) {
        if (!h[q] || !w_key[q]) return DAGNN_EINVAL;
        J.h[q] = h[q]; J.wkey[q] = w_key[q];
    }
    hipLaunchKernelGGL(df_score_parts_kernel, dim3((unsigned)((N + 3) / 4), (unsigned)n), dim3(256), 0, (hipStream_t)stream, J, ld_h, H, N);
    DAGNN_CHECK_LAUNCH();
    return DAGNN_OK;
}

extern "C" int dagnn_score_parts(float* h, int ld_h, int H, const float* w_key, int64_t N, void* stream) {
    return dagnn_score_parts_batch(&h, &w_key, 1, ld_h, H, N, stream);
}

#endif

#if defined(DF_WIDE_TU)
extern "C" int dagnn_dataflow_run_wide(const dagnn_plan* pl, const dagnn_dataflow_args* a, void* stream) {
    if (!pl || !pl->data || !a || !a->schedule) return DAGNN_EINVAL;
    if (a->H <= 256) return DAGNN_EINVAL;
    if (pl->num_edge_feats != 2 || a->vid_mod > 0) return DAGNN_EINVAL;
    for (int d = 0; d < 2; ++d)
        for (int i = 0; i < a->num_stacked && i < DAGNN_MAX_STACKED; ++i)
            if (((a->dir_mask >> d) & 1) && (a->cell[d][i].static_score || !a->cell[d][i].edge_gain)) return DAGNN_EINVAL;
#else
extern "C" int dagnn_dataflow_run(const dagnn_plan* pl, const dagnn_dataflow_args* a, void* stream) {
    if (!pl || !pl->data || !a || !a->schedule) return DAGNN_EINVAL;
    if (a->H > 256) return dagnn_dataflow_run_wide(pl, a, stream);
#endif
    const int H = a->H, Ls = a->num_stacked, dir_mask = a->dir_mask & 3, G = a->groups;
    if (H <= 0 || (H % 64) || H > DF_TU_MAX_H || Ls <= 0 || Ls > DAGNN_MAX_STACKED || !dir_mask || a->ld_h < H || a->gld < H ||
        (Ls > 1 && a->pld < H) || G < 1 || G > DF_MAX_GROUPS || a->epoch == 0 || !a->err)
        return DAGNN_EINVAL;
    if (pl->B == 0 || pl->N == 0) return DAGNN_OK;
    if ((int64_t)pl->N * a->gld >= (1ll << 31) || (int64_t)pl->N * a->pld >= (1ll << 31)) return DAGNN_EINVAL;
    if (pl->N >= (1 << 24) || (int64_t)pl->N * a->ld_h >= (1ll << 31) || (int64_t)pl->N * 3 * H >= (1ll << 31) || a->ld_h >= (1 << 24) ||
        a->gld >= (1 << 24) || a->pld >= (1 << 24))
        return DAGNN_EINVAL;
    if (a->stat_rows && (int64_t)pl->N * df_stat_floats(H) * 4 >= (1ll << 32)) return DAGNN_EINVAL;
    DfArgs S;
    int nc = 0;
    for (int d = 0; d < 2; ++d) {
        if (!((dir_mask >> d) & 1)) continue;
        for (int i = 0; i < Ls; ++i) {
            const dagnn_dataflow_cell& c = a->cell[d][i];
            if (c.agg < 0 || c.agg > 3 || (c.agg != 0 && (pl->num_edge_feats > 2 || a->vid_mod > 0 || c.static_score))) return DAGNN_EINVAL;
            if (!c.w_hh || !c.b_hh || (c.agg == 0 && !c.w_key && !c.static_score) || !c.h_out || !c.granules) return DAGNN_EINVAL;
            if (i == 0 ? !c.gi0 : (!c.w_ih || !c.b_ih || !c.proj_granules)) return DAGNN_EINVAL;
            if (nc + (i > 0 ? 2 : 1) > DF_MAX_KCELLS) return DAGNN_EINVAL;
            if (a->stat_rows && (!c.gh_out || c.gi_out)) return DAGNN_EINVAL;
            if (i > 0) {
                DfCell& P = S.cell[nc++];
                P.w = (const float4*)c.w_ih; P.bias = c.b_ih;
                P.wkey = nullptr; P.sscore = nullptr; P.gain = nullptr; P.vid = nullptr; P.gi0 = nullptr; P.p_in = nullptr;
                P.agg_w = nullptr; P.agg_b = nullptr; P.agg = 0;
                P.h_out = nullptr;
                if ((uintptr_t)c.proj_granules & 15) return DAGNN_EINVAL;
                P.g_out = (gran_t*)c.proj_granules;
                P.g_in = (const gran_t*)a->cell[d][i - 1].granules;
                P.aux_out = c.gi_out;
                P.dir = d; P.kind = DF_PROJECTION; P.variant = DFK_PROJ * 4; P.partner = -1;
                S.cell[nc - 2].partner = nc - 1;
            }
            DfCell& K = S.cell[nc++];
            K.w = (const float4*)c.w_hh; K.bias = c.b_hh;
            K.wkey = c.static_score ? nullptr : c.w_key;
            K.sscore = c.static_score;
            K.gain = pl->num_edge_feats > 0 ? c.edge_gain : nullptr;
            K.vid = a->vid_mod > 0 ? c.vid_bias : nullptr;
            K.gi0 = i == 0 ? c.gi0 : nullptr;
            K.p_in = i > 0 ? (const pgran_t*)c.proj_granules : nullptr;
            K.h_out = c.h_out;
            K.g_out = (gran_t*)c.granules;
            K.g_in = nullptr;
            K.aux_out = c.gh_out;
            K.dir = d; K.kind = DF_RECURRENT;
            K.variant = (i == 0 ? DFK_REC0 : DFK_RECP) * 4 + ((K.gain && pl->num_edge_feats == 2) ? 2 : 0) + ((K.sscore || K.vid) ? 1 : 0);
            K.partner = -1;
            K.agg = c.agg; K.agg_w = c.agg != 0 ? c.agg_edge_w : nullptr; K.agg_b = c.agg != 0 ? c.agg_edge_b : nullptr;
            if (c.agg != 0) { K.variant = 16 * c.agg + (i == 0 ? DFK_REC0 : DFK_RECP) * 4; K.gain = nullptr; K.wkey = nullptr; }
        }
    }
    const DfLayout SL = df_layout_words(pl->N, pl->B, G);
    S.sched = (const int32_t*)a->schedule;
    PlanLayout L = dagnn_plan_layout_words(pl->N, pl->E, pl->B, pl->num_edge_feats);
    for (int d = 0; d < 2; ++d) { S.gtab[d] = SL.gtab[d]; S.grec[d] = SL.grec[d]; S.col[d] = L.col[d]; S.eattr[d] = L.eattr[d]; }
    S.spin_limit = a->spin_limit ? a->spin_limit : (1u << 22);
    S.N = (int)pl->N;
    S.aux_stat = a->stat_rows ? 1 : 0;
    S.ncell = nc; S.H = H; S.ld_h = a->ld_h; S.gld = a->gld; S.pld = a->pld; S.R = pl->num_edge_feats;
    S.vid_mod = a->vid_mod > 0 ? a->vid_mod : 1;
    S.groups = G; S.epoch = a->epoch; S.err = (int*)a->err;
    S.dbg = (unsigned long long*)a->debug_timing;
    S.dbg_wg = a->debug_wg;
    S.status = (const int32_t*)a->plan_status;
    const int32_t* plan = (const int32_t*)pl->data;
    unsigned grid = (unsigned)(df_sets_for(G) * nc * (H / DF_JS));
    S.nroles = 0; S.xcc_tab = (gran_t*)a->xcc_table;
    if (a->num_cus >= 8 && a->num_cus <= DF_MAX_WGS && a->xcc_table && df_sets_for(G) < 64 && nc <= 31) {
        const int NS = H / DF_JS, sets = df_sets_for(G), cap = a->num_cus / 8;
        int fill[8] = {0, 0, 0, 0, 0, 0, 0, 0};
        const int xrot = (a->xcd_first % 8 + 8) % 8;
        for (int b = 0; b < DF_MAX_WGS; ++b) S.role[b] = DF_IDLE_ROLE;
        bool ok = true;
        int top = 0;
        for (int pass = 0; pass < 2 && ok; ++pass)
            for (int set = 0; set < sets && ok; ++set)
                for (int c = 0; c < nc && ok; ++c) {
                    if (S.cell[c].kind != DF_RECURRENT || (S.cell[c].partner >= 0) != (pass == 0)) continue;
                    const int members[2] = {c, S.cell[c].partner};
                    const int size = NS * (members[1] >= 0 ? 2 : 1);
                    int x = 0;
                    while (x < 8 && fill[x] + size > cap) ++x;
                    if (x == 8) { ok = false; break; }
                    for (int m = 0; m < 2; ++m) {
                        if (members[m] < 0) continue;
                        for (int sl = 0; sl < NS; ++sl) {
                            const int b = fill[x]++ * 8 + (x + xrot) % 8;
                            S.role[b] = (unsigned short)((set << 10) | (members[m] << 5) | sl);
                            if (b + 1 > top) top = b + 1;
                        }
                    }
                }
        if (ok) { S.nroles = top; grid = (unsigned)top; }
    }
    hipStream_t st = (hipStream_t)stream;
#define DF_LAUNCH(KPT)                                                                                                   \
    do {                                                                                                                 \
        const void* fn = reinterpret_cast<const void*>(dataflow_kernel<KPT>);                                            \
        const hipError_t ea = hipFuncSetAttribute(fn, hipFuncAttributeMaxDynamicSharedMemorySize, (int)df_lds_bytes<KPT>()); \
        if (ea != hipSuccess) return DAGNN_EHIP(ea);                                                                     \
        hipLaunchKernelGGL((dataflow_kernel<KPT>), dim3(grid), dim3(DF_THREADS), df_lds_bytes<KPT>(), st, plan, S);      \
    } while (0)
#if defined(DF_WIDE_TU)
    DF_LAUNCH(20);
#else
    switch (H / 16) {
        case 4: DF_LAUNCH(4); break;
        case 8: DF_LAUNCH(8); break;
        case 12: DF_LAUNCH(12); break;
        default: DF_LAUNCH(16); break;
    }
#endif
#undef DF_LAUNCH
    DAGNN_CHECK_LAUNCH();
    return DAGNN_OK;
}
```

### dagnn_amd/engine.py

```python
from __future__ import annotations

import ctypes as C
import os
from typing import List, Optional, Sequence, Tuple

import torch

from . import _lib
from ._lib import (BackwardArgs, BwdDataflowArgs, DagnnHipError, DataflowArgs, FrontierArgs, GemmGroup, LayerArgs, Plan,
                   TilesArgs, check)


class KernelTimer(object):

    def __init__(self, only=None):
        self.spans = {}
        self.only = set(only) if only else None

    def span(self, name, device):
        if self.only is not None and name not in self.only:
            return _NoSpan()
        return _Span(self, name, device)

    def summary(self):
# ... 297 lines not shown
                spl.append(host[soff:soff + T].copy())
            self._schedule, self._splits = out, spl
        return self._schedule

    def read_splits(self):
        self.read_schedule()
        return self._splits

    def dataflow_schedule(self, groups: int, launch: bool = True) -> torch.Tensor:
        cache = self.__dict__.setdefault("_df", {})
        pending = self.__dict__.setdefault("_df_pending", {})
        key = (int(groups), DF_COST_LAYER, DF_COST_ROW)
        if key not in cache:
            meta = getattr(self, "_df_host", None)
            if meta is not None and meta.get("key") == key:
                cache[key] = meta["words"]
            else:
                lib = _lib.load()
                nbytes = lib.dagnn_dataflow_bytes(self.N, self.B, key[0])
                ws = pending.pop(key, None)
                if ws is None:
                    ws = torch.empty((nbytes + 3) // 4, dtype=torch.int32, device=self.ws.device)
                if not launch:
                    pending[key] = ws
                    return ws
                with _span("dataflow_schedule", self.ws):
                    check(lib.dagnn_dataflow_schedule(C.byref(self.desc), ws.data_ptr(), nbytes, key[0], key[1], key[2],
                                                      self.status.data_ptr(), _stream(self.ws)), "dagnn_dataflow_schedule")
                cache[key] = ws
        return cache[key]

    def dataflow_layout(self, groups: int) -> dict:
        off = (C.c_int64 * 13)()
        check(_lib.load().dagnn_dataflow_layout(self.N, self.B, int(groups), off), "dagnn_dataflow_layout")
        names = ["grp_of", "gdepth", "gload", "loff", "gtab0", "gtab1", "lcnt0", "lcnt1", "glbase0", "glbase1", "grec0",
                 "grec1", "total"]
        return {k: int(v) // 4 for k, v in zip(names, off)}

    def check_status(self) -> None:
        s = int(self.status[0])
        if s:
            msgs = [m for b, m in ((1, "edges not grouped by graph"), (2, "edge crosses graphs / out of range"),
                                   (4, "batch vector not sorted"), (8, "layer id >= nodes of its graph")) if s & b]
            raise DagnnHipError("plan contract violated: " + ", ".join(msgs))


def build_plan(edge_index: torch.Tensor, layer_fwd: torch.Tensor, layer_bwd: torch.Tensor, batch: torch.Tensor,
               num_graphs: int, edge_attr: Optional[torch.Tensor] = None, launch: bool = True) -> PlanHandle:
    edge_index = _dev(edge_index, "edge_index", torch.int64)
    layer_fwd = _dev(layer_fwd, "layer ids", torch.int64)
    layer_bwd = _dev(layer_bwd, "layer ids", torch.int64)
    batch = _dev(batch, "batch", torch.int64)
    N, E = layer_fwd.numel(), edge_index.shape[1]
    R = 0
    if edge_attr is not None:
        edge_attr = _dev(edge_attr, "edge_attr", torch.float32).view(E, -1)
        R = edge_attr.shape[1]
    plan = PlanHandle(N, E, num_graphs, R, edge_index.device)
    plan._keep = (edge_index, layer_fwd, layer_bwd, batch, edge_attr)
    if launch:
        plan.launch_build()
    return plan


def encode_ast(x: torch.Tensor, depth: torch.Tensor, type_w: torch.Tensor, attr_w: torch.Tensor,
               depth_w: Optional[torch.Tensor], max_depth: int) -> torch.Tensor:
    x = _dev(x, "x", torch.int64)
    if not (depth.is_cuda and depth.dtype == torch.int64 and depth.is_contiguous()):
        raise DagnnHipError("node_depth must be a contiguous int64 GPU tensor (it is clamped in place)")
    N, H = x.shape[0], type_w.shape[1]
    out = torch.empty(N, H, dtype=torch.float32, device=x.device)
    check(_lib.load().dagnn_encode_ast(x.data_ptr(), depth.data_ptr(), _dev(type_w, "type table").data_ptr(),
                                       _dev(attr_w, "attribute table").data_ptr(),
                                       None if depth_w is None else _dev(depth_w, "depth table").data_ptr(), int(max_depth), out.data_ptr(), H,
                                       N, H, _stream(x)), "dagnn_encode_ast")
    return out


def gemm_nt_bias(A: Sequence[torch.Tensor], W: Sequence[torch.Tensor], bias: Sequence[Optional[torch.Tensor]],
                 out: Optional[Sequence[torch.Tensor]] = None) -> List[torch.Tensor]:
    n = len(A)
    A = [_rows(a, "A") for a in A]
    if len({a.stride(0) for a in A}) > 1:
        A = [a.contiguous() for a in A]
    lda = A[0].stride(0)
    W = [_dev(w, "W", torch.float32) for w in W]
    M, K = A[0].shape
    Nc = W[0].shape[0]
    for a, w in zip(A, W):
        if tuple(a.shape) != (M, K) or tuple(w.shape) != (Nc, K):
            raise DagnnHipError("grouped GEMM needs identical shapes per group")
    if out is None:
        out = [torch.empty(M, Nc, dtype=torch.float32, device=A[0].device) for _ in range(n)]
    groups = (GemmGroup * n)()
    keep = []
    for g in range(n):
        b = None if bias[g] is None else _dev(bias[g], "bias", torch.float32)
        keep.append(b)
        groups[g] = GemmGroup(A[g].data_ptr(), W[g].data_ptr(), _ptr(b), out[g].data_ptr())
    with _span("gemm_nt_bias", A[0]):
        check(_lib.load().dagnn_gemm_nt_bias(groups, n, M, Nc, K, lda, K, Nc, _stream(A[0])), "dagnn_gemm_nt_bias")
    return list(out)


def pack_whh(w_hh: torch.Tensor) -> torch.Tensor:
    w_hh = _dev(w_hh, "weight_hh", torch.float32)
    H = w_hh.shape[1]
    out = torch.empty(H, 3 * H, dtype=torch.float32, device=w_hh.device)
    check(_lib.load().dagnn_pack_whh(w_hh.data_ptr(), out.data_ptr(), H, _stream(w_hh)), "dagnn_pack_whh")
    return out


def pack_slices(w: torch.Tensor, H: int, slice_units: int) -> torch.Tensor:
    w = _dev(w, "weight", torch.float32)
    K = w.shape[1]
    out = torch.empty(3 * H * K, dtype=torch.float32, device=w.device)
    check(_lib.load().dagnn_pack_slices(w.data_ptr(), out.data_ptr(), H, K, slice_units, _stream(w)),
          "dagnn_pack_slices")
    return out


def pack_mfma(w: torch.Tensor, H: int) -> torch.Tensor:
    w = _dev(w, "weight", torch.float32)
    out = torch.empty(3 * H * w.shape[1], dtype=torch.float32, device=w.device)
    check(_lib.load().dagnn_pack_mfma(w.data_ptr(), out.data_ptr(), H, w.shape[1], _stream(w)), "dagnn_pack_mfma")
    return out


def pack_batch(mats: Sequence[torch.Tensor], H: int):
    mats = [_dev(w, "weight", torch.float32) for w in mats]
    outs = []
    for base in range(0, len(mats), _lib.MAX_PACK_JOBS):
        chunk = mats[base:base + _lib.MAX_PACK_JOBS]
        jobs = (_lib.PackJob * len(chunk))()
        for j, w in zip(jobs, chunk):
            o = {k: torch.empty(3 * H * w.shape[1], dtype=torch.float32, device=w.device) for k in (16, 32, "mfma")}
            outs.append(o)
            j.w, j.out_slices16, j.out_slices32, j.out_mfma = w.data_ptr(), o[16].data_ptr(), o[32].data_ptr(), \
                o["mfma"].data_ptr()
            j.H, j.K = H, w.shape[1]
        check(_lib.load().dagnn_pack_batch(jobs, len(chunk), _stream(chunk[0])), "dagnn_pack_batch")
    return outs


def pack_dataflow(w: torch.Tensor, H: int) -> torch.Tensor:
    w = _dev(w, "weight", torch.float32)
    if tuple(w.shape) != (3 * H, H):
        raise DagnnHipError("pack_dataflow needs a [3H, H] matrix, got %s" % (tuple(w.shape),))
    out = torch.empty(3 * H * H, dtype=torch.float32, device=w.device)
    check(_lib.load().dagnn_pack_dataflow(w.data_ptr(), out.data_ptr(), H, _stream(w)), "dagnn_pack_dataflow")
    return out


def pack_dataflow_batch(mats, H: int, gains=()):
    lib = _lib.load()
    outs, jobs, keep = [], [], []
    for w, tr in mats:
        w = _dev(w, "weight", torch.float32)
        if tuple(w.shape) != (3 * H, H):
            raise DagnnHipError("pack_dataflow_batch needs [3H, H] matrices, got %s" % (tuple(w.shape),))
        o = torch.empty(3 * H * H, dtype=torch.float32, device=w.device)
        keep.append(w)
        outs.append(o)
        jobs.append(_lib.DfPackJob(w.data_ptr(), o.data_ptr(), None, 1 if tr else 0, 0, 0))
    for ew, key, out in gains:
        ew, key = _dev(ew, "edge_encoder.weight", torch.float32), _dev(key, "key weights", torch.float32)
        keep += [ew, key]
        jobs.append(_lib.DfPackJob(ew.data_ptr(), out.data_ptr(), key.data_ptr(), 2, ew.shape[0], ew.shape[1]))
    for k0 in range(0, len(jobs), _lib.MAX_PACK_JOBS):
        part = jobs[k0:k0 + _lib.MAX_PACK_JOBS]
        arr = (_lib.DfPackJob * len(part))(*part)
        check(lib.dagnn_pack_dataflow_batch(arr, len(part), H, _stream(keep[0])), "dagnn_pack_dataflow_batch")
    return outs


RESERVED_CUS = _env_int("DAGNN_AMD_RESERVED_CUS", -1)
RCCL_MAX_WORKGROUPS = 64
_COLLECTIVE = {"registered": False, "group": None}


def register_collective(group=None) -> None:
    _COLLECTIVE["registered"] = True
    _COLLECTIVE["group"] = group


def reserved_cus_info(training: bool):
    if RESERVED_CUS >= 0:
        return (RESERVED_CUS if training else 0), "DAGNN_AMD_RESERVED_CUS=%d" % RESERVED_CUS
    if not training:
        return 0, "inference passes overlap no collective"
    import torch.distributed as dist
    if not (dist.is_available() and dist.is_initialized()):
        return 0, "no communicator"
    try:
        world = dist.get_world_size(_COLLECTIVE["group"]) if _COLLECTIVE["registered"] else dist.get_world_size()
    except (RuntimeError, ValueError):
        world = 1
    if world <= 1:
        return 0, "the gradient exchange's group has one rank"
    pinned = _env_int("NCCL_MAX_NCHANNELS", 0)
    ch = pinned if pinned > 0 else RCCL_MAX_WORKGROUPS
    r = min((ch + 7) // 8 * 8, RCCL_MAX_WORKGROUPS)
    return r, ("NCCL_MAX_NCHANNELS=%d pins RCCL's workgroups" % pinned if pinned > 0 else
               "RCCL may run up to %d channels (one workgroup each); NCCL_MAX_NCHANNELS pins fewer" % RCCL_MAX_WORKGROUPS)


def reserved_cus(training: bool) -> int:
    return reserved_cus_info(training)[0]


def effective_cus(device, training: bool = False) -> int:
    n = _num_cus(device)
    r = reserved_cus(training)
    return max(n - r, 8) if r > 0 else n


def dataflow_groups(device, num_dirs: int, num_stacked: int, H: int, B: int, training: bool = False) -> int:
    if not DATAFLOW or not (H <= 256 or (H == 320 and DF_WIDE)):
        return 0
    cus = effective_cus(device, training)
    g = _lib.load().dagnn_dataflow_groups(cus, int(num_dirs), int(num_stacked), int(H), int(B))
    return min(g, DF_GROUPS) if DF_GROUPS > 0 else g


class PassRecord(object):
    __slots__ = ("h_buf", "gi0", "Hp", "route", "gh", "gi", "stat")

    def __init__(self, route=None):
        self.h_buf = self.gi0 = self.Hp = None
        self.route, self.gh, self.gi, self.stat = route, {}, {}, {}

    def handover(self) -> Optional[str]:
        return "stat" if self.stat else "preact" if self.gh else None


def dataflow_run(plan: PlanHandle, dirs: Sequence[int], L: int, H: int, cells, gi0, h, groups: int, vid_mod: int = 0,
                 arena: Optional["GranuleArena"] = None, static_score=None, score_parts: bool = False,
                 record: Optional[PassRecord] = None, training: bool = False, stat_rows: bool = False) -> None:
    if arena is None:
        raise DagnnHipError("the dataflow kernel needs a GranuleArena (persistent, zero-initialised granule buffers)")
    lib = _lib.load()
    args = dataflow_args(plan, dirs, L, H, cells, gi0, h, groups, vid_mod, arena, static_score, record, training, None, stat_rows)
    with persistent_launch(plan.ws), _span("dataflow_run", plan.ws):
        check(lib.dagnn_dataflow_run(C.byref(plan.desc), C.byref(args), _stream(plan.ws)), "dagnn_dataflow_run")
    if score_parts and static_score is None:
        pairs = [(h[d][i], cells[(d, i)].w_key) for d in dirs for i in range(L)]
        for o in range(0, len(pairs), 16):
            part = pairs[o:o + 16]
            hp = (C.c_void_p * len(part))(*[t.data_ptr() for t, _ in part])
            wp = (C.c_void_p * len(part))(*[w.data_ptr() for _, w in part])
            check(lib.dagnn_score_parts_batch(hp, wp, len(part), part[0][0].shape[1], H, plan.N, _stream(plan.ws)), "dagnn_score_parts_batch")
    arena.watch(plan, folded=True)


def lib_static_floats(N: int, H: int) -> int:
    return int(_lib.load().dagnn_bwd_dataflow_static_bytes_h(int(N), int(H))) // 4


STAT_FWD = _env_int("DAGNN_AMD_STAT_FWD", 1)


def dataflow_args(plan: PlanHandle, dirs: Sequence[int], L: int, H: int, cells, gi0, h, groups: int, vid_mod: int = 0,
                  arena: Optional["GranuleArena"] = None, static_score=None, record: Optional[PassRecord] = None,
                  training: bool = False, args=None, stat_rows: bool = False):
    if args is None:
        args = DataflowArgs()
    gld = H + H // 16
    keys = [(d, i) for d in dirs for i in range(L)] + [("p", d, i) for d in dirs for i in range(1, L)]
    gran, epoch, err = arena.get(keys, plan.N, gld, plan.ws.device, widths={k: 2 * H for k in keys if k[0] == "p"})
    mask = 0
    for d in dirs:
        mask |= 1 << d
        for i in range(L):
            c, fc = cells[(d, i)], args.cell[d][i]
            fc.w_hh = c.w_hh_df.data_ptr()
            fc.w_ih = c.w_ih_df.data_ptr() if c.w_ih_df is not None else None
            fc.b_hh, fc.b_ih = c.b_hh.data_ptr(), _ptr(c.b_ih_dev)
            if static_score is not None:
                fc.static_score = _dev(static_score[(d, i)], "static score", torch.float32).data_ptr()
            else:
                fc.w_key = c.w_key.data_ptr()
            fc.edge_gain = _ptr(c.edge_gain) if plan.R > 0 else None
            fc.vid_bias = _ptr(c.vid_bias) if vid_mod > 0 else None
            agg = getattr(c, "agg", 0)
            if agg:
                fc.agg, fc.agg_edge_w, fc.agg_edge_b = int(agg), _ptr(getattr(c, "agg_w", None)), _ptr(getattr(c, "agg_b", None))
                fc.w_key = fc.static_score = fc.edge_gain = None
            fc.gi0 = gi0[d].data_ptr() if i == 0 else None
            fc.h_out = h[d][i].data_ptr()
            fc.granules = gran[(d, i)].data_ptr()
            fc.proj_granules = gran[("p", d, i)].data_ptr() if i > 0 else None
            if record is not None and stat_rows:
                nfl = lib_static_floats(plan.N, H)
                record.stat[(d, i)] = (torch.empty if H in (256, 320) else torch.zeros)(nfl, dtype=torch.float32, device=plan.ws.device)
                fc.gh_out = record.stat[(d, i)].data_ptr()
                args.stat_rows = 1
            elif record is not None:
                record.gh[(d, i)] = torch.empty(plan.N, 3 * H, dtype=torch.float32, device=plan.ws.device)
                fc.gh_out = record.gh[(d, i)].data_ptr()
                if i > 0:
                    record.gi[(d, i)] = torch.empty(plan.N, 3 * H, dtype=torch.float32, device=plan.ws.device)
                    fc.gi_out = record.gi[(d, i)].data_ptr()
    args.num_stacked, args.dir_mask, args.H, args.ld_h, args.gld = L, mask, H, h[dirs[0]][0].shape[1], gld
    args.pld = H
    args.vid_mod, args.groups, args.epoch = int(vid_mod), int(groups), epoch
    sched = plan.dataflow_schedule(groups)
    args.schedule, args.err = sched.data_ptr(), err.data_ptr()
    args.debug_timing = DEBUG_TIMING.data_ptr() if DEBUG_TIMING is not None else None
    args.spin_limit = SPIN_LIMIT
    args.debug_wg = DEBUG_WG
    if DF_XCD:
        args.num_cus = effective_cus(plan.ws.device, training)
        args.xcc_table = arena.xcc_table(plan.ws.device).data_ptr()
        args.xcd_first = arena.xcd_first
    args.plan_status = plan.status.data_ptr()
    return args


DF_WIDE = _env_int("DAGNN_AMD_DF_WIDE", 1)


def state_width(H: int, num_stacked: int = 1, num_edge_feats: int = 0, wide_ok: bool = False) -> int:
    Hp = (int(H) + 63) // 64 * 64
    if Hp == 320 and wide_ok and DATAFLOW and DF_WIDE and num_edge_feats == 2:
        return 320
    if TILES and TILES_PAD and 256 < Hp < 512 and num_edge_feats <= 2 and (num_stacked >= 2 or Hp > 384 or TILES_PAD >= 2):
        Hp = 512
    return Hp


def tiles_launches(device, num_dirs: int, num_stacked: int, H: int, num_edge_feats: int, num_nodes: int = 0) -> int:
    if not TILES:
        return 0
    if TILES == 1 and (num_stacked < 2 or num_nodes > TILES_MAX_NODES):
        return 0
    return _lib.load().dagnn_tiles_launches(_num_cus(device), int(num_dirs), int(num_stacked), int(H), int(num_edge_feats))


def tiles_batch_too_flat(plan: PlanHandle, dirs: Sequence[int]) -> bool:
    if TILES != 1 or TILES_MAX_MEAN_ROWS <= 0 or plan.N <= 1536:
        return False
    sched = plan.read_schedule()
    T = max([len(sched[d]) - 1 for d in dirs] + [1])
    return plan.N > TILES_MAX_MEAN_ROWS * T


def tiles_tail_split(plan: PlanHandle, dirs: Sequence[int]):
    if TILES_TAIL_ROWS <= 0:
        return None
    import numpy as np
    sched = plan.read_schedule()
    first, tail = [0, 0], 0
    for d in dirs:
        rows = np.diff(sched[d].astype(np.int64))
        wide = np.nonzero(rows > TILES_TAIL_ROWS)[0]
        first[d] = int(wide[-1]) + 1 if len(wide) else 0
        tail = max(tail, len(rows) - first[d])
    return first if tail >= 32 else None


def tiles_run(plan: PlanHandle, dirs: Sequence[int], L: int, H: int, cells, gi0, h, arena: "GranuleArena",
              first_layer: Optional[Sequence[int]] = None, vid_mod: int = 0) -> None:
    if arena is None:
        raise DagnnHipError("the tile kernel needs a GranuleArena (persistent, zero-initialised progress counters)")
    args = TilesArgs()
    bufs, epoch, err = arena.get(["tiles"], 4096, 1, plan.ws.device)
    mask = 0
    for d in dirs:
        mask |= 1 << d
        for i in range(L):
            c, fc = cells[(d, i)], args.cell[d][i]
            fc.w_hh = c.w_hh_raw.data_ptr()
            fc.b_hh = c.b_hh.data_ptr()
            if i > 0:
# ... 1645 lines not shown
```

### dagnn_amd/host_plan.py

```python
from __future__ import annotations

from typing import Dict, List, Optional, Sequence, Tuple

import numpy as np
import torch

PLAN_MAGIC = 0x44414731
THIN_ROWS = 14


def _align4(w: int) -> int:
    return (w + 3) & ~3


def plan_layout(N: int, E: int, B: int, R: int) -> Dict[str, int]:
    o = 16
    L: Dict[str, int] = {}

    def take(name: str, n: int) -> None:
        nonlocal o
        L[name] = o
        o = _align4(o + n)

    take("node_ptr", B + 1)
# ... 4 lines not shown
            take("%s%d" % (name, d), n)
    take("items", 2 * B)
    for name, n in (("slot", N), ("cursor", N + B), ("eidx", E), ("blptr", N + 2), ("blsplit", N + 2),
                    ("lbase", N + B), ("rowrec", 16 * N), ("brec", 16 * N)):
        for d in (0, 1):
            take("%s%d" % (name, d), n)
    L["total"] = o
    return L


def _np(t) -> np.ndarray:
    return t.detach().cpu().numpy() if isinstance(t, torch.Tensor) else np.asarray(t)


def build_plan_host(edge_index, layer_fwd, layer_bwd, batch, num_graphs: int, edge_attr=None,
                    return_written: bool = False):
    ei = _np(edge_index).astype(np.int64).reshape(2, -1)
    batch = _np(batch).astype(np.int64).reshape(-1)
    layers = [_np(layer_fwd).astype(np.int64).reshape(-1), _np(layer_bwd).astype(np.int64).reshape(-1)]
    N, E, B = batch.shape[0], ei.shape[1], int(num_graphs)
    R = 0
    ea = None
    if edge_attr is not None:
        ea = np.ascontiguousarray(_np(edge_attr), dtype=np.float32).reshape(E, -1)
        R = ea.shape[1]
    if N and (np.any(np.diff(batch) < 0) or batch[0] < 0 or batch[-1] >= B):
        raise ValueError("plan contract violated: batch vector not sorted / out of range")
    if E:
        if ei.min() < 0 or ei.max() >= N or np.any(batch[ei[0]] != batch[ei[1]]):
            raise ValueError("plan contract violated: edge crosses graphs / out of range")
        if np.any(np.diff(batch[ei[0]]) < 0):
            raise ValueError("plan contract violated: edges not grouped by graph")
    L = plan_layout(N, E, B, R)
    ws = np.zeros(L["total"], dtype=np.int32)
    written = np.zeros(L["total"], dtype=bool) if return_written else None

    def put(name: str, values, index=None) -> None:
        values = np.asarray(values)
        if index is None:
            index = np.arange(values.shape[0])
        ws[L[name] + index] = values.astype(np.int32, copy=False) if values.dtype != np.int32 else values
        if written is not None:
            written[L[name] + index] = True

    ws[0:5] = (N, E, B, R, PLAN_MAGIC)
    if written is not None:
        written[0:5] = True
    gids = np.arange(B + 1)
    node_ptr = np.searchsorted(batch, gids, side="left")
    edge_ptr = np.searchsorted(batch[ei[0]], gids, side="left") if E else np.zeros(B + 1, dtype=np.int64)
    put("node_ptr", node_ptr)
    put("edge_ptr", edge_ptr)
    n_of = np.diff(node_ptr)
    ids = np.arange(N)
    sched: List[np.ndarray] = []
    splits: List[np.ndarray] = []
    depths = []
    for d in (0, 1):
        layer = np.clip(layers[d], 0, np.maximum(n_of[batch] - 1, 0)) if N else layers[d]
        depth = np.zeros(B, dtype=np.int64)
        if N:
            np.maximum.at(depth, batch, layer + 1)
        depths.append(depth)
        put("depth%d" % d, depth)
        order = np.lexsort((ids, layer, batch))
        pos = np.empty(N, dtype=np.int64)
        pos[order] = ids
        put("order%d" % d, order)
        big = int(n_of.max()) + 2 if B else 2
        key_sorted = batch[order] * big + layer[order]
        g_rep = np.repeat(np.arange(B), depth + 1)
        t_rep = np.arange(g_rep.shape[0]) - np.repeat(np.cumsum(depth + 1) - (depth + 1), depth + 1)
        ls_idx = node_ptr[g_rep] + g_rep + t_rep
        ls_val = np.searchsorted(key_sorted, g_rep * big + t_rep, side="left")
        put("lstart%d" % d, ls_val, ls_idx)
        feed, other = (ei[1], ei[0]) if d == 0 else (ei[0], ei[1])
        p_e = pos[feed]
        perm = np.argsort(p_e, kind="stable")
        col = other[perm]
        put("col%d" % d, col)
        put("eidx%d" % d, perm)
        if R:
            put("eattr%d" % d, ea[perm].reshape(-1).view(np.int32))
        p_sorted = p_e[perm]
        row_begin = np.searchsorted(p_sorted, ids, side="left")
        g_of_pos = batch[order]
        rp = np.zeros(N + B, dtype=np.int64)
        rp[ids + g_of_pos] = row_begin
        rp[node_ptr[1:] + np.arange(B)] = edge_ptr[1:]
        put("rowptr%d" % d, rp)
        T = int(depth.max()) if B else 0
        width = np.bincount(layer, minlength=T) if N else np.zeros(0, dtype=np.int64)
        bl = np.zeros(N + 2, dtype=np.int64)
        bl[1:T + 1] = np.cumsum(width[:T])
        bl[N + 1] = T
        put("blptr%d" % d, bl)
        sched.append(bl[:T + 1].astype(np.int32))
        fat = np.flatnonzero(width[:T] > THIN_ROWS)
        thr = int(fat[-1]) + 1 if fat.size else 0
        ws[5 + d] = thr
        if written is not None:
            written[5 + d] = True
        deep = depth > thr
        by_layer = np.lexsort((ids, deep[batch], layer)) if N else ids
        slot = np.empty(N, dtype=np.int64)
        slot[by_layer] = ids
        put("slot%d" % d, slot)
        split = np.zeros(N + 2, dtype=np.int64)
        if N:
            split[:T] = bl[:T] + np.bincount(layer[~deep[batch]], minlength=T)[:T]
        put("blsplit%d" % d, split)
        splits.append(split[:T].astype(np.int32))
        g2 = np.repeat(np.arange(B), depth)
        t2 = np.arange(g2.shape[0]) - np.repeat(np.cumsum(depth) - depth, depth)
        base2 = node_ptr[g2] + g2 + t2
        ls_full = np.zeros(N + B + 1, dtype=np.int64)
        ls_full[ls_idx] = ls_val
        cnt2 = ls_full[base2 + 1] - ls_full[base2]
        by_tg = np.lexsort((g2, deep[g2], t2))
        c = cnt2[by_tg]
        lb = np.empty(g2.shape[0], dtype=np.int64)
        lb[by_tg] = np.cumsum(c) - c
        put("lbase%d" % d, lb, base2)
        rec = np.zeros((N, 16), dtype=np.int32)
        eb = row_begin[pos]
        ee = np.empty(N, dtype=np.int64)
        ee_sorted = rp[ids + g_of_pos + 1]
        ee[order] = ee_sorted
        rec[:, 0], rec[:, 1], rec[:, 2], rec[:, 3] = ids, eb, ee, batch
        eattr_bits = ea[perm].view(np.int32) if R else None
        for q in range(4):
            ok = eb + q < ee
            src = np.minimum(eb + q, max(E - 1, 0))
            if E:
                rec[:, 4 + q] = np.where(ok, col[src], 0)
                if R >= 1:
                    rec[:, 8 + 2 * q] = np.where(ok, eattr_bits[src, 0], 0)
                if R >= 2:
                    rec[:, 9 + 2 * q] = np.where(ok, eattr_bits[src, 1], 0)
        out = np.empty((N, 16), dtype=np.int32)
        out[slot] = rec
        put("rowrec%d" % d, out.reshape(-1))
    key = np.stack(depths, 1).reshape(-1) if B else np.zeros(0, dtype=np.int64)
    put("items", np.argsort(-key, kind="stable"))
    if return_written:
        return ws, sched, splits, written
    return ws, sched, splits


DF_MAGIC = 0x44463031
DF_RB = 4


def dataflow_layout(N: int, B: int, G: int) -> Dict[str, int]:
    o = 16
    L: Dict[str, int] = {}

    def take(name: str, n: int) -> None:
        nonlocal o
        L[name] = o
        o = _align4(o + n)

    take("grp_of", B)
    take("gdepth", G)
    take("gload", G)
    take("loff", G + 1)
    for name, n in (("gtab", 2 * G), ("lcnt", N + G + 1), ("glbase", N + B), ("grec", 16 * (4 * N + 4))):
        for d in (0, 1):
            take("%s%d" % (name, d), n)
    L["total"] = o
    return L


def build_dataflow_schedule_host(plan_words, N: int, E: int, B: int, R: int, groups: int, cost_layer: int = 4,
                                 cost_row: int = 1) -> np.ndarray:
    ws = _np(plan_words).astype(np.int32, copy=False)
    P = plan_layout(N, E, B, R)
    S = dataflow_layout(N, B, groups)
    out = np.zeros(S["total"], dtype=np.int32)
    out[S["grec0"]:] = -1
    if B == 0 or N == 0:
        return out
    G = int(groups)
    node_ptr = ws[P["node_ptr"]:P["node_ptr"] + B + 1].astype(np.int64)
    n_of = np.diff(node_ptr)
    depth = [ws[P["depth%d" % d]:P["depth%d" % d] + B].astype(np.int64) for d in (0, 1)]
    items = ws[P["items"]:P["items"] + 2 * B]
    load = np.zeros(G, dtype=np.int64)
    gdepth = np.zeros(G, dtype=np.int64)
    empty = np.ones(G, dtype=bool)
    grp = np.zeros(B, dtype=np.int64)
    order = [int(it) >> 1 for it in items if not (it & 1)]
    if B <= 4096 and len(order) > 0 and int(n_of.min()) == int(n_of.max()):
        for j, g in enumerate(order):
            grp[g] = j % G
        for k in range(min(G, len(order))):
            dg = int(max(depth[0][order[k]], depth[1][order[k]]))
            gdepth[k] = dg
            load[k] = cost_layer * dg + cost_row * int(n_of[0]) * ((len(order) - k + G - 1) // G)
        order = []
    for g in order:
        dg = int(max(depth[0][g], depth[1][g]))
        cand = load + cost_row * int(n_of[g]) + np.where(empty, cost_layer * dg, 0)
        k = int(np.argmin(cand))
        load[k] = cand[k]
        if empty[k]:
            gdepth[k], empty[k] = dg, False
        grp[g] = k
    out[0:3] = (G, DF_MAGIC, DF_RB)
    out[S["grp_of"]:S["grp_of"] + B] = grp
    out[S["gdepth"]:S["gdepth"] + G] = gdepth
    out[S["gload"]:S["gload"] + G] = np.minimum(load, 0x7fffffff)
    loff = np.concatenate([[0], np.cumsum(gdepth + 1)])
    out[S["loff"]:S["loff"] + G + 1] = loff
    for d in (0, 1):
        g2 = np.repeat(np.arange(B), depth[d])
        t2 = np.arange(g2.shape[0]) - np.repeat(np.cumsum(depth[d]) - depth[d], depth[d])
        base2 = node_ptr[g2] + g2 + t2
        ls = ws[P["lstart%d" % d]:P["lstart%d" % d] + N + B].astype(np.int64)
        cnt2 = ls[base2 + 1] - ls[base2]
        k2 = grp[g2]
        cnt = np.zeros(int(loff[G]), dtype=np.int64)
        np.add.at(cnt, loff[k2] + t2, cnt2)
        padded = (cnt + DF_RB - 1) // DF_RB * DF_RB
        pref = np.zeros_like(cnt)
        nblk = np.zeros(G, dtype=np.int64)
        for k in range(G):
            a, b = int(loff[k]), int(loff[k + 1])
            seg = padded[a:b].copy()
            seg[-1] = 0
            c = np.cumsum(seg) - seg
            c[-1] = seg[:-1].sum()
            pref[a:b] = c
            nblk[k] = c[-1] // DF_RB
        out[S["lcnt%d" % d]:S["lcnt%d" % d] + int(loff[G])] = pref
        base = np.cumsum(nblk * DF_RB) - nblk * DF_RB
        gt = np.empty(2 * G, dtype=np.int64)
        gt[0::2], gt[1::2] = base, nblk
        out[S["gtab%d" % d]:S["gtab%d" % d] + 2 * G] = gt
        order2 = np.lexsort((g2, t2, k2))
        c = cnt2[order2]
        run_key = k2[order2] * (int(gdepth.max()) + 2) + t2[order2]
        start = np.concatenate([[True], run_key[1:] != run_key[:-1]])
        csum = np.cumsum(c) - c
        run_base = np.maximum.accumulate(np.where(start, csum, 0))
        within = csum - run_base
        glb = np.empty(g2.shape[0], dtype=np.int64)
        glb[order2] = pref[loff[k2[order2]] + t2[order2]] + within
        out[S["glbase%d" % d] + base2] = glb
        order = ws[P["order%d" % d]:P["order%d" % d] + N].astype(np.int64)
        slot = ws[P["slot%d" % d]:P["slot%d" % d] + N].astype(np.int64)
        rowrec = ws[P["rowrec%d" % d]:P["rowrec%d" % d] + 16 * N].reshape(N, 16)
        p = np.arange(N)
        v = order[p]
        recs = rowrec[slot[v]]
        g = recs[:, 3].astype(np.int64)
        glb_full = np.zeros(N + B + 1, dtype=np.int64)
        glb_full[base2] = glb
        reps = cnt2
        t_of_p = np.empty(N, dtype=np.int64)
        b_of_p = np.empty(N, dtype=np.int64)
        lsv = ls[base2]
        idx = np.repeat(np.arange(base2.shape[0]), reps)
        pos_sorted = np.repeat(lsv, reps) + (np.arange(idx.shape[0]) - np.repeat(np.cumsum(reps) - reps, reps))
        t_of_p[pos_sorted] = t2[idx]
        b_of_p[pos_sorted] = base2[idx]
        rec_idx = base[grp[g]] + glb_full[b_of_p] + (p - ls[b_of_p])
        dst = out[S["grec%d" % d]:S["grec%d" % d] + 16 * (4 * N + 4)].reshape(-1, 16)
        dst[rec_idx] = recs
    return out


def attach_plan(batch, num_graphs: Optional[int] = None, dataflow_groups: int = 0, cost_layer: int = 4, cost_row: int = 1):
    B = int(num_graphs if num_graphs is not None else getattr(batch, "num_graphs", int(batch.batch[-1]) + 1))
    ea = getattr(batch, "edge_attr", None)
    ws, sched, splits = build_plan_host(batch.edge_index, batch._bi_layer_idx0, batch._bi_layer_idx1, batch.batch, B, ea)
    batch._dagnn_plan = torch.from_numpy(ws)
    N, E = int(batch.batch.shape[0]), int(batch.edge_index.shape[1])
    R = 0 if ea is None else int(ea.reshape(E, -1).shape[1])
    batch._dagnn_plan_meta = dict(N=N, E=E, B=B, R=R, schedule=sched, splits=splits)
    if dataflow_groups > 0:
        batch._dagnn_df = torch.from_numpy(build_dataflow_schedule_host(ws, N, E, B, R, dataflow_groups, cost_layer, cost_row))
        batch._dagnn_plan_meta["dataflow_key"] = (int(dataflow_groups), int(cost_layer), int(cost_row))
    return batch
```

### include/dagnn_hip.h

```cpp
#ifndef DAGNN_HIP_H
#define DAGNN_HIP_H

#include <stddef.h>
#include <stdint.h>

#ifdef __cplusplus
extern "C" {
#endif

#define DAGNN_OK 0
#define DAGNN_EINVAL (-22)
#define DAGNN_ENOSPC (-28)
#define DAGNN_EHIP(e) (-(1000 + (int)(e)))

#define DAGNN_MAX_DIRS 2
#define DAGNN_MAX_GROUPS 4

const char* dagnn_version(void);


typedef struct dagnn_plan {
    void* data;
    size_t bytes;
    int64_t N, E, B;
// ... 17 lines not shown
#define DAGNN_PREPARE_MAX_TABLES 3
typedef struct dagnn_prepare_rows {
    const int64_t* x;
    int64_t* depth;
    int max_depth;
    int num_tables;
    struct {
        const float *type_emb, *attr_emb, *depth_emb;
        float* out;
        int width, ld_out;
    } table[DAGNN_PREPARE_MAX_TABLES];
    const int64_t* stack_src[4];
    int64_t* stack_out;
} dagnn_prepare_rows;

int dagnn_prepare(const dagnn_plan* plan, const int64_t* edge_index, const int64_t* layer_fwd, const int64_t* layer_bwd,
                  const int64_t* batch, const float* edge_attr, int32_t* status,
                  void* schedule, size_t schedule_bytes, int groups, int cost_layer, int cost_row,
                  const dagnn_prepare_rows* rows , void* stream);

typedef struct dagnn_gemm_group {
    const float* A;
    const float* W;
    const float* bias;
    float* C;
} dagnn_gemm_group;

int dagnn_gemm_nt_bias(const dagnn_gemm_group* groups , int num_groups,
                       int64_t M, int Nc, int K, int lda, int ldw, int ldc, void* stream);

int dagnn_pack_whh(const float* w_hh , float* w_hh_t , int H, void* stream);

typedef struct dagnn_layer_args {
    const float* gi[DAGNN_MAX_DIRS];
    const float* w_hh_t[DAGNN_MAX_DIRS];
    const float* b_hh[DAGNN_MAX_DIRS];
    const float* w_key[DAGNN_MAX_DIRS];
    const float* edge_gain[DAGNN_MAX_DIRS];
    const float* vid_bias[DAGNN_MAX_DIRS];
    float* h[DAGNN_MAX_DIRS];
    float* score[DAGNN_MAX_DIRS];
    int vid_mod;
    int ld_h;
    int static_score;
    void* debug_timing;
} dagnn_layer_args;

int dagnn_recurrence_layer(const dagnn_plan* plan , const dagnn_layer_args* args , int dir_mask,
                           int H, void* stream);

int dagnn_pack_slices(const float* w , float* out , int H, int K, int slice_units,
                      void* stream);

int dagnn_pack_mfma(const float* w , float* out, int H, int K, void* stream);

#define DAGNN_MAX_PACK_JOBS 16
typedef struct dagnn_pack_job {
    const float* w;
    float* out_slices16;
    float* out_slices32;
    float* out_mfma;
    int32_t H, K;
} dagnn_pack_job;
int dagnn_pack_batch(const dagnn_pack_job* jobs , int num_jobs, void* stream);

typedef struct dagnn_frontier_cell {
    const float* w_hh_pk16;
    const float* w_hh_pk32;
    const float* w_ih_pk16;
    const float* w_ih_pk32;
    const float* w_hh_mfma;
    const float* w_ih_mfma;
    const float* b_hh;
    const float* b_ih;
    const float* w_key;
    const float* static_score;
    const float* edge_gain;
    const float* vid_bias;
    const float* gi0;
    float* h_out;
    void* granules;
} dagnn_frontier_cell;

#define DAGNN_MAX_STACKED 8
typedef struct dagnn_frontier_args {
    dagnn_frontier_cell cell[DAGNN_MAX_DIRS][DAGNN_MAX_STACKED];
    int num_stacked;
    int dir_mask;
    int H, ld_h, vid_mod;
    int num_cus;
    int rb4_max_wgs;
    int mfma_min_rows;
    void* agg_scratch;
    int agg_scratch_rows;
    int tail_replicas;
    int tail_slice_units;
    int tail_max_blocks;
    unsigned epoch;
    void* tail_err;
    void* debug_timing;
    void* side_stream;
    const int32_t* layer_split[DAGNN_MAX_DIRS];
    void* fork_event;
    void* join_event;
} dagnn_frontier_args;

int dagnn_frontier_run(const dagnn_plan* plan , const dagnn_frontier_args* args ,
                       const int32_t* const* layer_ptr , const int32_t* num_layers ,
                       void* stream);

typedef struct dagnn_dataflow_cell {
    const float* w_hh;
    const float* w_ih;
    const float* b_hh;
    const float* b_ih;
    const float* w_key;
    const float* static_score;
    const float* edge_gain;
    const float* vid_bias;
    const float* gi0;
    float* h_out;
    void* granules;
    void* proj_granules;
    float* gh_out;
    float* gi_out;
    const float* agg_edge_w;
    const float* agg_edge_b;
    int agg;
} dagnn_dataflow_cell;
#define DAGNN_DF_AGG_ATTN 0
#define DAGNN_DF_AGG_ADD 1
#define DAGNN_DF_AGG_MAX 2
#define DAGNN_DF_AGG_NONE 3

typedef struct dagnn_dataflow_args {
    dagnn_dataflow_cell cell[DAGNN_MAX_DIRS][DAGNN_MAX_STACKED];
    int num_stacked, dir_mask;
    int H, ld_h, gld, pld, vid_mod;
    int groups;
    unsigned epoch;
    const void* schedule;
    void* err;
    void* debug_timing;
    unsigned spin_limit;
    int debug_wg;
    int num_cus;
    void* xcc_table;
    const void* plan_status;
    int xcd_first;
    int stat_rows;
} dagnn_dataflow_args;

int dagnn_dataflow_groups(int num_cus, int num_dirs, int num_stacked, int H, int64_t B);
size_t dagnn_dataflow_bytes(int64_t N, int64_t B, int groups);
int dagnn_dataflow_schedule(const dagnn_plan* plan , void* workspace, size_t workspace_bytes, int groups,
                            int cost_layer, int cost_row, const int32_t* plan_status , void* stream);
int dagnn_dataflow_run(const dagnn_plan* plan , const dagnn_dataflow_args* args , void* stream);
int dagnn_dataflow_run_wide(const dagnn_plan* plan , const dagnn_dataflow_args* args , void* stream);
int dagnn_pack_dataflow(const float* w , float* out , int H, void* stream);
int dagnn_pack_dataflow_transposed(const float* w , float* out , int H, void* stream);
typedef struct dagnn_df_pack_job {
    const float* w;
    float* out;
    const float* aux;
    int32_t transposed;
    int32_t rows, cols;
} dagnn_df_pack_job;
int dagnn_pack_dataflow_batch(const dagnn_df_pack_job* jobs , int njob, int H, void* stream);
int dagnn_score_parts(float* h , int ld_h, int H, const float* w_key , int64_t N, void* stream);
int dagnn_score_parts_batch(float* const* h, const float* const* w_key, int n, int ld_h, int H, int64_t N, void* stream);
int dagnn_dataflow_layout(int64_t N, int64_t B, int groups, int64_t* offsets13 );

typedef struct dagnn_tiles_cell {
    const float* w_hh;
    const float* w_ih;
    const float* b_hh;
    const float* b_ih;
    const float* w_key;
    const float* edge_gain;
    const float* gi0;
    float* h_out;
    const float* vid_bias;
} dagnn_tiles_cell;

typedef struct dagnn_tiles_args {
    dagnn_tiles_cell cell[DAGNN_MAX_DIRS][DAGNN_MAX_STACKED];
    int num_stacked, dir_mask;
    int H, ld_h;
    int num_cus;
    unsigned epoch;
    void* counters;
    void* err;
    unsigned spin_limit;
    const void* plan_status;
    int first_layer[DAGNN_MAX_DIRS];
    void* debug_timing;
    int vid_mod;
} dagnn_tiles_args;

int dagnn_tiles_launches(int num_cus, int num_dirs, int num_stacked, int H, int num_edge_feats);
int dagnn_tiles_run(const dagnn_plan* plan , const dagnn_tiles_args* args , void* stream);

typedef struct dagnn_backward_cell {
    const float* w_hh;
    const float* w_ih;
    const float* w_key;
    const float* edge_gain;
    const float* vid_bias;
    const float* static_score;
    const float* h;
    float* a;
    float* alpha;
    const float* gi;
    const float* gh;
    float* g_ext;
    float* da;
    float* dgi;
    float* dgh;
    float* sigma;
    float* edge_feat_grad;
    void* da_granules;
    void* du_granules;
    const float* g_ext_static;
} dagnn_backward_cell;

typedef struct dagnn_backward_args {
    dagnn_backward_cell cell[DAGNN_MAX_DIRS][DAGNN_MAX_STACKED];
    int num_stacked, dir_mask, H, ld_h;
    int vid_mod;
    int num_cus;
    int thin_wgs;
    int tail_replicas;
    int tail_max_blocks;
    unsigned epoch;
    void* tail_err;
    void* side_stream;
    const int32_t* layer_split[DAGNN_MAX_DIRS];
    void* fork_event;
    void* join_event;
} dagnn_backward_args;

int dagnn_backward_prepare(const dagnn_plan* plan , const dagnn_backward_args* args , void* stream);
int dagnn_backward_run(const dagnn_plan* plan , const dagnn_backward_args* args ,
                       const int32_t* const* layer_ptr , const int32_t* num_layers , void* stream);

typedef struct dagnn_bwd_dataflow_cell {
    const float* w_hh_t;
    const float* w_ih_t;
    const float* w_key;
    const float* alpha;
    const float* gi;
    const float* gh;
    const float* a;
    const float* b_hh;
    const float* h;
    const float* g_ext;
    float* stat;
    void* da_granules;
    void* q_granules;
    void* dgi_granules;
    void* du_granules;
    float* dgi;
    float* dgh;
    float* sigma;
    float* edge_feat_grad;
} dagnn_bwd_dataflow_cell;

typedef struct dagnn_bwd_dataflow_args {
    dagnn_bwd_dataflow_cell cell[DAGNN_MAX_DIRS][DAGNN_MAX_STACKED];
    int num_stacked, dir_mask, H, ld_h, ld_g, gld, groups;
    unsigned epoch, spin_limit;
    const void* schedule;
    void* records;
    void* err;
    const void* plan_status;
    int num_cus;
    void* xcc_table;
    int xcd_first;
    int stat_rows_written;
    int pull_rows;
} dagnn_bwd_dataflow_args;

size_t dagnn_bwd_dataflow_record_bytes(int64_t N);
size_t dagnn_bwd_dataflow_static_bytes(int64_t N);
size_t dagnn_bwd_dataflow_static_bytes_h(int64_t N, int H);
int dagnn_bwd_dataflow_prepare(const dagnn_plan* plan , const dagnn_bwd_dataflow_args* args , void* stream);
int dagnn_bwd_dataflow_run(const dagnn_plan* plan , const dagnn_bwd_dataflow_args* args , void* stream);
int dagnn_bwd_dataflow_run_wide(const dagnn_plan* plan , const dagnn_bwd_dataflow_args* args , void* stream);

#define DAGNN_PULL_ROW 256
typedef struct dagnn_plain_pull {
    const float* h;
    const float* a;
    const float* edge_mat;
    const float* edge_vec;
    float* weights;
    const void* da_granules;
    float* esum;
    int ld_h, ld_a, gld;
} dagnn_plain_pull;
int dagnn_plain_max_weights(const dagnn_plan* plan , const dagnn_plain_pull* c , int dir, int H,
                            int32_t row_begin, int32_t row_end, void* stream);
int dagnn_plain_edge_grads(const dagnn_plan* plan , const dagnn_plain_pull* c , int dir, int H,
                           int32_t row_begin, int32_t row_end, void* stream);

typedef struct dagnn_wgrad_job {
    const float* dg;
    const float* in;
    float* d_weight;
    float* d_bias;
    int ld_dg, ld_in, in_dim;
} dagnn_wgrad_job;
typedef struct dagnn_colsum_job {
// ... 562 lines not shown
```

Before: 103,900.

## Add MFMA projection role that shares workgroups across two group sets

Replaces the generic loader path for projection cells (H<=256) with a dedicated loader/compute pair that stages 16-row tiles in LDS and computes the input projection with fp32 MFMA, splitting K across waves and exchanging partial sums through LDS. One projection workgroup now serves two group sets (pshare=2), which frees CUs and lets inference with two stacked layers use more groups. It also adds a new weight packing layout for this role. This brings in extra LDS use, new inter-wave spin synchronisation and more complex role assignment, with risk of stalls or lower occupancy.

```diff
diff --git a/dagnn_amd/_lib.py b/dagnn_amd/_lib.py
--- a/dagnn_amd/_lib.py
+++ b/dagnn_amd/_lib.py
@@ -381,6 +381,7 @@
     "dagnn_frontier_run": (C.c_int, [C.POINTER(Plan), C.POINTER(FrontierArgs), C.POINTER(C.POINTER(C.c_int32)),
                                      C.POINTER(C.c_int32), C.c_void_p]),
     "dagnn_dataflow_groups": (C.c_int, [C.c_int, C.c_int, C.c_int, C.c_int, C.c_int64]),
+    "dagnn_dataflow_groups_shared": (C.c_int, [C.c_int, C.c_int, C.c_int, C.c_int, C.c_int64]),
     "dagnn_dataflow_bytes": (C.c_size_t, [C.c_int64, C.c_int64, C.c_int]),
     "dagnn_dataflow_layout": (C.c_int, [C.c_int64, C.c_int64, C.c_int, C.POINTER(C.c_int64)]),
     "dagnn_dataflow_schedule": (C.c_int, [C.POINTER(Plan), C.c_void_p, C.c_size_t, C.c_int, C.c_int, C.c_int,
@@ -391,6 +392,7 @@
     "dagnn_tiles_run": (C.c_int, [C.POINTER(Plan), C.POINTER(TilesArgs), C.c_void_p]),
     "dagnn_pack_dataflow": (C.c_int, [C.c_void_p, C.c_void_p, C.c_int, C.c_void_p]),
     "dagnn_pack_dataflow_transposed": (C.c_int, [C.c_void_p, C.c_void_p, C.c_int, C.c_void_p]),
+    "dagnn_pack_dataflow_proj": (C.c_int, [C.c_void_p, C.c_void_p, C.c_int, C.c_void_p]),
     "dagnn_score_parts": (C.c_int, [C.c_void_p, C.c_int, C.c_int, C.c_void_p, C.c_int64, C.c_void_p]),
     "dagnn_backward_prepare": (C.c_int, [C.POINTER(Plan), C.POINTER(BackwardArgs), C.c_void_p]),
     "dagnn_backward_run": (C.c_int, [C.POINTER(Plan), C.POINTER(BackwardArgs), C.POINTER(C.POINTER(C.c_int32)),
diff --git a/dagnn_amd/core.py b/dagnn_amd/core.py
--- a/dagnn_amd/core.py
+++ b/dagnn_amd/core.py
@@ -192,7 +192,7 @@
         if c.w_hh_df is None:
             todo.append((c, "w_hh_df", c.w_hh_raw, False))
             if c.b_ih_dev is not None:
-                todo.append((c, "w_ih_df", c.w_ih, False))
+                todo.append((c, "w_ih_df", c.w_ih, engine.PACK_PROJ16 if c.Hp <= 256 else False))
         if transposed_too and c.w_hh_bt is None:
             todo.append((c, "w_hh_bt", c.w_hh_raw, True))
             if c.b_ih_dev is not None:
diff --git a/dagnn_amd/csrc/dataflow.hip b/dagnn_amd/csrc/dataflow.hip
--- a/dagnn_amd/csrc/dataflow.hip
+++ b/dagnn_amd/csrc/dataflow.hip
@@ -96,6 +96,7 @@
     unsigned long long* dbg;
     gran_t* xcc_tab;
     int nroles;
+    int pshare;
     int aux_stat;
     unsigned short role[DF_MAX_WGS];
 };
@@ -184,17 +185,17 @@
     const int32_t* __restrict__ recs = S.sched + S.grec[d] + 16 * (int64_t)rec_base;
     const int32_t* __restrict__ col = plan + S.col[d];
     const float* __restrict__ eattr = reinterpret_cast<const float*>(plan + S.eattr[d]);
-    constexpr bool proj = KIND == DFK_PROJ;
-    const int R = proj ? 0 : (RR >= 0 ? RR : (C.gain ? S.R : 0));
+    static_assert(KIND != DFK_PROJ, "projection cells have loaders of their own: df_proj16_loader (H <= 256), df_loader_fast (H = 320)");
+    const int R = RR >= 0 ? RR : (C.gain ? S.R : 0);
     const unsigned epoch = S.epoch, spin_limit = S.spin_limit;
     int* const err = S.err;
-    const gran_t* const g_src = proj ? C.g_in : C.g_out;
+    const gran_t* const g_src = C.g_out;
     const int gld = S.gld, pld = S.pld;
     const pgran_t* const p_in = KIND == DFK_RECP ? C.p_in : nullptr;
     const float* const gi0 = KIND == DFK_REC0 ? C.gi0 : nullptr;
     const float* const sscore = EXTRA ? C.sscore : nullptr;
     const float* const vid = EXTRA ? C.vid : nullptr;
-    const float* const gainp = proj ? nullptr : C.gain;
+    const float* const gainp = C.gain;
     const int vid_mod = EXTRA ? S.vid_mod : 1;
     const float gain0 = R >= 1 ? C.gain[0] : 0.f, gain1 = R >= 2 ? C.gain[1] : 0.f;
     unsigned long long* const dbg = (DF_PROF && S.dbg) ? S.dbg + 2 * gridDim.x : nullptr;
@@ -207,7 +208,7 @@
     for (int q = 0; q < 4; ++q) {
         const int c = 64 * q + lane;
         cpos[q] = c + (SEG - KP8) * (c / KP8);
-        if (!proj && !PLAIN && !(EXTRA && C.sscore) && q < NQ4) wk[q] = C.wkey[c];
+        if (!PLAIN && !(EXTRA && C.sscore) && q < NQ4) wk[q] = C.wkey[c];
     }
     const int agg = PLAIN ? C.agg : 0;
     const int Rp = (PLAIN && C.agg_w) ? S.R : 0;
@@ -350,7 +351,7 @@
         };
         if (v >= 0) {
             const int eb = r0.y;
-            const int deg = proj ? 1 : ((PLAIN && agg == 3) ? 0 : r0.z - r0.y);
+            const int deg = (PLAIN && agg == 3) ? 0 : r0.z - r0.y;
             float acc[4] = {0.f, 0.f, 0.f, 0.f};
             float m = -INFINITY, l = 0.f;
             bool p_pending = KIND == DFK_RECP;
@@ -376,9 +377,7 @@
                         }
                     }
                 }
-                if (proj) {
-                    pj[0] = v;
-                } else if (c0 == 0) {
+                if (c0 == 0) {
                     pj[0] = r1.x; pj[1] = r1.y; pj[2] = r1.z; pj[3] = r1.w;
                     if (R >= 1 && R <= 2) {
                         fe[0] = gain0 * __int_as_float(r2.x) + gain1 * __int_as_float(r2.y);
@@ -1054,6 +1053,218 @@
     else { if (local_st) run(std::true_type(), aux2()); else run(std::false_type(), aux2()); }
 }
 
+constexpr int DP_ROWS = 4 * DF_RB;
+constexpr int DP_DEPTH = 2;
+constexpr int DP_XR = 24;
+constexpr int DP_XCH = 2 * 2 * 2 * 6 * 64;
+template <int KPT> __host__ __device__ constexpr size_t df_lds_bytes() {
+    return (size_t)DF_NLS * (DF_NSLOT * DfSlot<KPT>::words + DF_GIRING * DF_RB * 3 * DF_JS + DF_RB * 8 * 16) * 4 + 128 + 3 * DF_JS * 4 + 128;
+}
+template <int KPT> __host__ __device__ constexpr size_t df_lds_total() { return df_lds_bytes<KPT>() + (KPT <= 16 ? DP_XCH * 4 : 0); }
+template <int KPT> struct DpLds {
+    static constexpr int rowp = 16 * KPT + 4;
+    static constexpr int tile = DP_ROWS * rowp;
+    static constexpr int ids_off = DF_NLS * DP_DEPTH * tile;
+    static constexpr int end = ids_off + DF_NLS * DP_DEPTH * DP_ROWS;
+};
+
+__device__ __forceinline__ bool dp_pick_a(int ia, int na, int ib, int nb) {
+    if (ia >= na) return false;
+    if (ib >= nb) return true;
+    return (long long)ia * nb <= (long long)ib * na;
+}
+__device__ __forceinline__ int dp_tile_blocks(const DfArgs& S) { return S.pshare > 1 ? 4 : 2; }
+__device__ __forceinline__ int dp_tiles(const DfArgs& S, int d, int g) {
+    const int tb = dp_tile_blocks(S);
+    return g < S.groups ? (S.sched[S.gtab[d] + 2 * g + 1] + tb - 1) / tb : 0;
+}
+
+template <int KPT>
+__device__ __forceinline__ void df_proj16_loader(const DfArgs& S, const DfCell& C, int pp, float* smem, int* flags, int w, int set) {
+    constexpr int H = 16 * KPT, NQ4 = H / 64;
+    typedef DpLds<KPT> P;
+    const int lane = threadIdx.x & 63;
+    const int d = C.dir;
+    int base[2], nblk[2], nt[2];
+    const int tb = dp_tile_blocks(S);
+#pragma unroll
+    for (int q = 0; q < 2; ++q) {
+        const int g = DF_NLS * S.pshare * pp + S.pshare * set + q;
+        const bool have = q < S.pshare && g < S.groups;
+        base[q] = have ? S.sched[S.gtab[d] + 2 * g] : 0;
+        nblk[q] = have ? S.sched[S.gtab[d] + 2 * g + 1] : 0;
+        nt[q] = (nblk[q] + tb - 1) / tb;
+    }
+    const int32_t* __restrict__ recs = S.sched + S.grec[d];
+    const unsigned epoch = S.epoch, spin_limit = S.spin_limit;
+    int* const err = S.err;
+    const gran_t* const g_src = C.g_in;
+    const unsigned gld = (unsigned)S.gld;
+    int* const rdy = flags + set * DF_WPS + w;
+    const int* const dn = flags + DF_NLS * DF_WPS + set * DF_NCW;
+    float* const tiles = smem + set * DP_DEPTH * P::tile;
+    int* const ids = reinterpret_cast<int*>(smem + P::ids_off) + set * DP_DEPTH * DP_ROWS;
+    const unsigned lane8 = 8u * lane;
+    const int total = nt[0] + nt[1];
+    auto ids_of = [&](int q, int j) -> int {
+        const int blk = tb * j + (lane & 3);
+        return ((lane & 3) < tb && blk < nblk[q]) ? recs[16 * ((int64_t)base[q] + 4 * blk + w)] : -1;
+    };
+    int it[2] = {0, 0};
+    int q = dp_pick_a(0, nt[0], 0, nt[1]) ? 0 : 1;
+    int cur = total > 0 ? ids_of(q, 0) : -1;
+    DfSweep A;
+    for (int t = 0; t < total; ++t) {
+        ++it[q];
+        int nxt = -1;
+        q = dp_pick_a(it[0], nt[0], it[1], nt[1]) ? 0 : 1;
+        if (t + 1 < total) nxt = ids_of(q, it[q]);
+        const int v0 = __builtin_amdgcn_readlane(cur, 0), v1 = __builtin_amdgcn_readlane(cur, 1);
+        const int v2 = __builtin_amdgcn_readlane(cur, 2), v3 = __builtin_amdgcn_readlane(cur, 3);
+        const int vl = v0 >= 0 ? v0 : v1 >= 0 ? v1 : v2 >= 0 ? v2 : v3;
+        if (t >= DP_DEPTH) df_wait4(dn, t - DP_DEPTH + 1, err, spin_limit);
+        asm volatile("" ::: "memory");
+        const int slot = t % DP_DEPTH;
+        if (vl >= 0) {
+            DfTripArgs T;
+            T.b[0] = g_src + (unsigned)(v0 >= 0 ? v0 : vl) * gld;
+            T.b[1] = g_src + (unsigned)(v1 >= 0 ? v1 : vl) * gld;
+            T.b[2] = g_src + (unsigned)(v2 >= 0 ? v2 : vl) * gld;
+            T.b[3] = g_src + (unsigned)(v3 >= 0 ? v3 : vl) * gld;
+            T.c = reinterpret_cast<const pgran_t*>(g_src);
+            T.ra = g_src; T.rl = 0u; T.ga = g_src; T.gl = 0u;
+            df_trip<NQ4, H, 4, 0, 0>(A, T, lane8, 0u);
+            if (!df_landed<4, 0, NQ4>(A, epoch)) {
+                unsigned spins = 0;
+                bool more;
+                do {
+                    more = df_retry(spins, err, spin_limit);
+                    df_trip<NQ4, H, 4, 0, 0>(A, T, lane8, 0u);
+                } while (more && !df_landed<4, 0, NQ4>(A, epoch));
+            }
+            float* const trow = tiles + slot * P::tile + w * P::rowp + lane;
+#pragma unroll
+            for (int k = 0; k < 4; ++k)
+#pragma unroll
+                for (int c = 0; c < NQ4; ++c) trow[4 * k * P::rowp + 64 * c] = __uint_as_float((unsigned)A.x[k][c]);
+        }
+        if (lane < 4) ids[slot * DP_ROWS + 4 * lane + w] = cur;
+        asm volatile("s_waitcnt lgkmcnt(0)" ::: "memory");
+        df_flag_st(rdy, t + 1);
+        cur = nxt;
+    }
+    asm volatile("s_waitcnt vmcnt(0)" ::: "memory");
+}
+
+template <int KPT>
+__device__ __forceinline__ void df_proj16_compute(const DfArgs& S, const DfCell& C, int sl, int pp, float* smem, int* flags,
+                                                  float* xch, int cw) {
+    constexpr int H = 16 * KPT, KH = H / 2, NS4 = KH / 16;
+    typedef DpLds<KPT> P;
+    const int tc = threadIdx.x & 255;
+    const int lane = tc & 63, n = lane & 15, kq = lane >> 4;
+    const int uh = cw >> 1, kh = cw & 1;
+    const int d = C.dir;
+    float wgt[3][NS4][4];
+    {
+        const float4* wp = C.w + (int64_t)sl * (3 * NS4) * 256 + tc;
+#pragma unroll
+        for (int g = 0; g < 3; ++g)
+#pragma unroll
+            for (int s = 0; s < NS4; ++s) {
+                const float4 x = wp[(g * NS4 + s) * 256];
+                wgt[g][s][0] = x.x; wgt[g][s][1] = x.y; wgt[g][s][2] = x.z; wgt[g][s][3] = x.w;
+            }
+#pragma unroll
+        for (int g = 0; g < 3; ++g)
+#pragma unroll
+            for (int s = 0; s < NS4; ++s)
+#pragma unroll
+                for (int e = 0; e < 4; ++e) asm volatile("" : "+v"(wgt[g][s][e]));
+    }
+    const int unit = sl * DF_JS + 16 * uh + n;
+    float b_r = C.bias[unit], b_z = C.bias[H + unit], b_n = C.bias[2 * H + unit];
+    asm volatile("" : "+v"(b_r), "+v"(b_z), "+v"(b_n));
+    const float s_r = kh ? 0.f : b_r, s_z = kh ? 0.f : b_z, s_n = kh ? 0.f : b_n;
+    const unsigned epoch = S.epoch, spin_limit = S.spin_limit;
+    int* const err = S.err;
+    pgran_t* const p_out = reinterpret_cast<pgran_t*>(C.g_out);
+    float* const aux_out = C.aux_out;
+    const int pld = S.pld, num_nodes = S.N;
+    int nts[2];
+#pragma unroll
+    for (int s = 0; s < 2; ++s) {
+        const int g0 = DF_NLS * S.pshare * pp + S.pshare * s;
+        nts[s] = dp_tiles(S, d, g0) + (S.pshare > 1 ? dp_tiles(S, d, g0 + 1) : 0);
+    }
+    const int total = nts[0] + nts[1];
+    const int* const rdy = flags;
+    int* const dn = flags + DF_NLS * DF_WPS;
+    int* const xr = flags + DP_XR;
+    float* const x_mine = xch + ((uh * 2 + kh) * 2) * (6 * 64) + lane;
+    const float* const x_peer = xch + ((uh * 2 + (kh ^ 1)) * 2) * (6 * 64) + lane;
+    int is[2] = {0, 0};
+    for (int t = 0; t < total; ++t) {
+        const int s = dp_pick_a(is[0], nts[0], is[1], nts[1]) ? 0 : 1;
+        const int ts = is[s]++;
+        df_wait4(rdy + s * DF_WPS, ts + 1, err, spin_limit);
+        asm volatile("" ::: "memory");
+        const int slot = s * DP_DEPTH + ts % DP_DEPTH;
+        const float* const arow = smem + slot * P::tile + n * P::rowp + kh * KH + 4 * kq;
+        const int* const idp = reinterpret_cast<const int*>(smem + P::ids_off) + slot * DP_ROWS + 4 * kq + 2 * kh;
+        const int gv0 = idp[0], gv1 = idp[1];
+        f4v acc[3] = {(f4v){s_r, s_r, s_r, s_r}, (f4v){s_z, s_z, s_z, s_z}, (f4v){s_n, s_n, s_n, s_n}};
+#pragma unroll
+        for (int k = 0; k < NS4; ++k) {
+            const float4 a4 = *reinterpret_cast<const float4*>(arow + 16 * k);
+            const float av[4] = {a4.x, a4.y, a4.z, a4.w};
+#pragma unroll
+            for (int e = 0; e < 4; ++e)
+#pragma unroll
+                for (int g = 0; g < 3; ++g) acc[g] = __builtin_amdgcn_mfma_f32_16x16x4f32(av[e], wgt[g][k][e], acc[g], 0, 0, 0);
+        }
+        float* const xm = x_mine + (t & 1) * (6 * 64);
+#pragma unroll
+        for (int g = 0; g < 3; ++g) { xm[(2 * g) * 64] = kh ? acc[g][0] : acc[g][2]; xm[(2 * g + 1) * 64] = kh ? acc[g][1] : acc[g][3]; }
+        asm volatile("s_waitcnt lgkmcnt(0)" ::: "memory");
+        if (lane == 0) {
+            df_flag_st(xr + uh * 2 + kh, t + 1);
+            df_flag_st(dn + s * DF_NCW + cw, ts + 1);
+        }
+        {
+            unsigned spins = 0;
+            while (df_flag_ld(xr + uh * 2 + (kh ^ 1)) < t + 1) {
+                __builtin_amdgcn_s_sleep(DF_CSLEEP_N);
+                if (++spins > 4 * spin_limit) { __hip_atomic_fetch_or(err, 2, __ATOMIC_RELAXED, __HIP_MEMORY_SCOPE_AGENT); break; }
+                if ((spins & 1023) == 0 && __hip_atomic_load(err, __ATOMIC_RELAXED, __HIP_MEMORY_SCOPE_AGENT) != 0) break;
+            }
+        }
+        asm volatile("" ::: "memory");
+        const float* const xp = x_peer + (t & 1) * (6 * 64);
+        float o[3][2];
+#pragma unroll
+        for (int g = 0; g < 3; ++g) { o[g][0] = xp[(2 * g) * 64]; o[g][1] = xp[(2 * g + 1) * 64]; }
+        asm volatile("s_waitcnt lgkmcnt(0)" ::: "memory");
+#pragma unroll
+        for (int i = 0; i < 2; ++i) {
+            const int gv = i ? gv1 : gv0;
+            if ((unsigned)gv < (unsigned)num_nodes) {
+                float own[3];
+#pragma unroll
+                for (int g = 0; g < 3; ++g) own[g] = kh ? (i ? acc[g][3] : acc[g][2]) : (i ? acc[g][1] : acc[g][0]);
+                const float p_r = own[0] + o[0][i], p_z = own[1] + o[1][i], p_n = own[2] + o[2][i];
+                pgran_t* po = p_out + df_idx(gv, pld, unit);
+                const pgran_t pv = {epoch, __float_as_uint(p_r), __float_as_uint(p_z), __float_as_uint(p_n)};
+                asm volatile("global_store_dwordx4 %0, %1, off sc1" :: "v"(po), "v"(pv) : "memory");
+                if (aux_out) {
+                    float* ao = aux_out + df_idx(gv, 3 * H, unit);
+                    ao[0] = p_r; ao[H] = p_z; ao[2 * H] = p_n;
+                }
+            }
+        }
+    }
+}
+
 template <int KPT>
 __global__ void __launch_bounds__(DF_THREADS, DF_THREADS / 256) dataflow_kernel(const int32_t* __restrict__ plan, DfArgs S) {
     extern __shared__ __attribute__((aligned(16))) float smem[];
@@ -1081,6 +1292,14 @@
         c = rem / NS; sl = rem - c * NS;
     }
     const DfCell& C = S.cell[c];
+    constexpr bool P16 = KPT <= 16;
+    const bool proj16 = P16 && C.kind == DF_PROJECTION;
+    if (proj16 && S.nroles == 0 && S.pshare > 1) {
+        if (pair & 1) return;
+        pair >>= 1;
+    }
+    static_assert(!P16 || DpLds<KPT>::end <= DF_NLS * (DF_NSLOT * Slot::words + DF_GIRING * DF_RB * 3 * DF_JS + DF_RB * 8 * 16),
+                  "the projection role's tiles lie below the flag words");
     DfLds lds;
     lds.ring = smem;
     lds.giring = lds.ring + DF_NLS * DF_NSLOT * Slot::words;
@@ -1090,8 +1309,8 @@
     lds.dn = flags + DF_NLW;
     lds.local = flags + DF_NLW + DF_NLS * DF_NCW;
     lds.bias = reinterpret_cast<float*>(flags + 32);
-    if (tid < DF_NLW + DF_NLS * DF_NCW + 1) flags[tid] = 0;
-    static_assert(DF_NLW + DF_NLS * DF_NCW + 1 <= 32, "flag words");
+    if (tid < 32) flags[tid] = 0;
+    static_assert(DF_NLW + DF_NLS * DF_NCW + 1 <= DP_XR && DP_XR + 4 <= 32, "flag words");
     if (tid >= 64 && tid < 64 + 3 * DF_JS) lds.bias[tid - 64] = C.bias[((tid - 64) / DF_JS) * (16 * KPT) + sl * DF_JS + (tid - 64) % DF_JS];
     if (S.nroles > 0 && wave == 0) {
         unsigned xcc;
@@ -1105,7 +1324,8 @@
                 const int b = b0 + (tid & 63);
                 const unsigned r = b < S.nroles ? S.role[b] : DF_IDLE_ROLE;
                 const int rc = (int)((r >> 5) & 31u);
-                const bool member = r != DF_IDLE_ROLE && (int)(r >> 10) == pair && (rc == c || rc == C.partner);
+                const bool member = r != DF_IDLE_ROLE && ((rc == c && (int)(r >> 10) == pair) ||
+                                                          (rc == C.partner && (int)(r >> 10) == (P16 && S.pshare > 1 ? pair >> 1 : pair)));
                 unsigned spins = 0;
                 bool have = !member;
                 unsigned theirs = xcc;
@@ -1126,12 +1346,23 @@
         if (wave < 8) S.dbg[2 * gridDim.x + 8 * (int64_t)wave + 7] = 0x100000000ull | __builtin_amdgcn_s_getreg(4 | (0 << 6) | (31 << 11));
     __syncthreads();
     const int variant = C.variant;
+    if constexpr (P16) {
+        if (proj16) {
+            float* const xch = smem + df_lds_bytes<KPT>() / 4;
+            if (wave < DF_NCW) df_proj16_compute<KPT>(S, C, sl, pair, smem, lds.rdy, xch, wave);
+            else df_proj16_loader<KPT>(S, C, pair, smem, lds.rdy, (wave - DF_NCW) % DF_WPS, (wave - DF_NCW) / DF_WPS);
+            if (DF_PROF && S.dbg && tid == 0) S.dbg[2 * blockIdx.x + 1] = wall_clock64();
+            return;
+        }
+    }
     if (wave < DF_NCW) {
         const int cw = wave;
         switch ((variant >> 2) & 3) {
             case DFK_REC0: df_compute<KPT, DFK_REC0>(S, C, sl, pair, lds, cw); break;
             case DFK_RECP: df_compute<KPT, DFK_RECP>(S, C, sl, pair, lds, cw); break;
-            default: df_compute<KPT, DFK_PROJ>(S, C, sl, pair, lds, cw); break;
+            default:
+                if constexpr (!P16) df_compute<KPT, DFK_PROJ>(S, C, sl, pair, lds, cw);
+                break;
         }
     } else {
         const int set = (wave - DF_NCW) / DF_WPS;
@@ -1141,7 +1372,7 @@
 #define DF_LOADER_CASE(K, RR, EX) case (K) * 4 + ((RR) == 2 ? 2 : 0) + ((EX) ? 1 : 0): df_loader<KPT, K, RR, EX>(plan, S, C, sl, grp, lds, w, set); break;
             if (variant == DFK_REC0 * 4 + 2) { df_loader_fast<KPT, DFK_REC0>(plan, S, C, sl, grp, lds, w, set); }
             else if (variant == DFK_RECP * 4 + 2) { df_loader_fast<KPT, DFK_RECP>(plan, S, C, sl, grp, lds, w, set); }
-            else if ((variant >> 2) == DFK_PROJ) { df_loader_fast<KPT, DFK_PROJ>(plan, S, C, sl, grp, lds, w, set); }
+            else if ((variant >> 2) == DFK_PROJ) { if constexpr (!P16) df_loader_fast<KPT, DFK_PROJ>(plan, S, C, sl, grp, lds, w, set); }
             else if constexpr (KPT <= 16) {
                 if (variant >= 16) {
                     if (((variant >> 2) & 3) == DFK_REC0) df_loader<KPT, DFK_REC0, -1, false, true>(plan, S, C, sl, grp, lds, w, set);
@@ -1152,7 +1383,7 @@
                     DF_LOADER_CASE(DFK_REC0, -1, false) DF_LOADER_CASE(DFK_REC0, -1, true)
                     DF_LOADER_CASE(DFK_RECP, 2, false) DF_LOADER_CASE(DFK_RECP, 2, true)
                     DF_LOADER_CASE(DFK_RECP, -1, false) DF_LOADER_CASE(DFK_RECP, -1, true)
-                    default: df_loader<KPT, DFK_PROJ, -1, false>(plan, S, C, sl, grp, lds, w, set); break;
+                    default: break;
                 }
             } else {
                 if (tid % 64 == 0) __hip_atomic_fetch_or(S.err, 8, __ATOMIC_RELAXED, __HIP_MEMORY_SCOPE_AGENT);
@@ -1163,13 +1394,9 @@
     if (DF_PROF && S.dbg && tid == 0) S.dbg[2 * blockIdx.x + 1] = wall_clock64();
 }
 
-template <int KPT> size_t df_lds_bytes() {
-    return (size_t)DF_NLS * (DF_NSLOT * DfSlot<KPT>::words + DF_GIRING * DF_RB * 3 * DF_JS + DF_RB * 8 * 16) * 4 + 128 + 3 * DF_JS * 4 + 128;
-}
-
-struct DfPackPos { int sl, g, k4, unit, ks, kp; };
-__device__ __forceinline__ DfPackPos df_pack_pos(int64_t idx, int H, bool transposed) {
-    (void)transposed;
+constexpr int DF_PACK_PROJ16 = 3;
+struct DfPackPos { int sl, g, k4, unit, ks, kp, k0; };
+__device__ __forceinline__ DfPackPos df_pack_pos(int64_t idx, int H, int layout) {
     DfPackPos P;
     P.kp = H >> 3;
     const int nk4 = P.kp >> 2, nq = 3 * nk4;
@@ -1178,18 +1405,24 @@
     const int q = (int)(rest % nq);
     P.sl = (int)(rest / nq);
     P.g = q / nk4; P.k4 = q - P.g * nk4;
-    P.unit = P.sl * DF_JS + 8 * (tc >> 6) + 4 * ((tc >> 5) & 1) + (tc & 3); P.ks = (tc >> 2) & 7;
+    if (layout == DF_PACK_PROJ16) {
+        P.unit = P.sl * DF_JS + 16 * (tc >> 7) + (tc & 15); P.ks = (tc >> 6) & 1;
+        P.k0 = P.ks * (H >> 1) + 16 * P.k4 + 4 * ((tc >> 4) & 3);
+    } else {
+        P.unit = P.sl * DF_JS + 8 * (tc >> 6) + 4 * ((tc >> 5) & 1) + (tc & 3); P.ks = (tc >> 2) & 7;
+        P.k0 = P.ks * P.kp + 4 * P.k4;
+    }
     return P;
 }
 
 __global__ void __launch_bounds__(256) df_pack_kernel(const float* __restrict__ W, float4* __restrict__ out, int H, int64_t total,
                                                        int transposed) {
     for (int64_t idx = (int64_t)blockIdx.x * blockDim.x + threadIdx.x; idx < total; idx += (int64_t)gridDim.x * blockDim.x) {
-        const DfPackPos P = df_pack_pos(idx, H, transposed != 0);
+        const DfPackPos P = df_pack_pos(idx, H, transposed);
         const int sl = P.sl, g = P.g, k4 = P.k4, unit = P.unit, ks = P.ks, kp8 = P.kp;
         (void)sl;
-        if (!transposed) {
-            out[idx] = *reinterpret_cast<const float4*>(W + (int64_t)(g * H + unit) * H + ks * kp8 + 4 * k4);
+        if (transposed != 1) {
+            out[idx] = *reinterpret_cast<const float4*>(W + (int64_t)(g * H + unit) * H + P.k0);
         } else {
             const float* src = W + (int64_t)(g * H + ks * kp8 + 4 * k4) * H + unit;
             out[idx] = make_float4(src[0], src[H], src[2 * (int64_t)H], src[3 * (int64_t)H]);
@@ -1211,10 +1444,10 @@
     }
     float4* __restrict__ out = reinterpret_cast<float4*>(J.out);
     for (int64_t idx = (int64_t)blockIdx.x * blockDim.x + threadIdx.x; idx < total; idx += (int64_t)gridDim.x * blockDim.x) {
-        const DfPackPos P = df_pack_pos(idx, H, J.transposed != 0);
+        const DfPackPos P = df_pack_pos(idx, H, J.transposed);
         const int g = P.g, k4 = P.k4, unit = P.unit, ks = P.ks, kp8 = P.kp;
-        if (!J.transposed) {
-            out[idx] = *reinterpret_cast<const float4*>(W + (int64_t)(g * H + unit) * H + ks * kp8 + 4 * k4);
+        if (J.transposed != 1) {
+            out[idx] = *reinterpret_cast<const float4*>(W + (int64_t)(g * H + unit) * H + P.k0);
         } else {
             const float* src = W + (int64_t)(g * H + ks * kp8 + 4 * k4) * H + unit;
             out[idx] = make_float4(src[0], src[H], src[2 * (int64_t)H], src[3 * (int64_t)H]);
@@ -1263,15 +1496,27 @@
     return DAGNN_OK;
 }
 
-extern "C" int dagnn_dataflow_groups(int num_cus, int num_dirs, int num_stacked, int H, int64_t B) {
+static int df_groups_for(int num_cus, int num_dirs, int num_stacked, int H, int64_t B, int shared) {
     if (num_cus <= 0 || num_dirs < 1 || num_dirs > DAGNN_MAX_DIRS || num_stacked < 1 || H <= 0 || (H % 64) || H > 320 || B <= 0)
         return 0;
     const int kcells = num_dirs * (2 * num_stacked - 1);
     if (kcells > DF_MAX_KCELLS) return 0;
-    int64_t g = (int64_t)DF_NLS * (num_cus / (kcells * (H / DF_JS)));
+    const int NS = H / DF_JS, L = num_stacked;
+    const bool pairs = shared && H <= 256;
+    int sets = 0;
+    while (sets < DF_MAX_GROUPS / DF_NLS && num_dirs * NS * (L * (sets + 1) + (L - 1) * (pairs ? (sets + 2) / 2 : sets + 1)) <= num_cus) ++sets;
+    int64_t g = (int64_t)DF_NLS * sets;
     if (g > DF_MAX_GROUPS) g = DF_MAX_GROUPS;
     if (g > B) g = B;
     return (int)g;
+}
+
+extern "C" int dagnn_dataflow_groups(int num_cus, int num_dirs, int num_stacked, int H, int64_t B) {
+    return df_groups_for(num_cus, num_dirs, num_stacked, H, B, 0);
+}
+
+extern "C" int dagnn_dataflow_groups_shared(int num_cus, int num_dirs, int num_stacked, int H, int64_t B) {
+    return df_groups_for(num_cus, num_dirs, num_stacked, H, B, 1);
 }
 
 extern "C" int dagnn_dataflow_schedule(const dagnn_plan* pl, void* ws_, size_t ws_bytes, int groups, int cost_layer,
@@ -1325,11 +1570,17 @@
 
 extern "C" int dagnn_pack_dataflow_transposed(const float* w, float* out, int H, void* stream) { return df_pack(w, out, H, 1, stream); }
 
+extern "C" int dagnn_pack_dataflow_proj(const float* w, float* out, int H, void* stream) {
+    if (H > 256) return DAGNN_EINVAL;
+    return df_pack(w, out, H, DF_PACK_PROJ16, stream);
+}
+
 extern "C" int dagnn_pack_dataflow_batch(const dagnn_df_pack_job* jobs, int njob, int H, void* stream) {
     if (!jobs || njob <= 0 || njob > DAGNN_MAX_PACK_JOBS || H <= 0 || (H % 64) || H > 320) return DAGNN_EINVAL;
     DfPackJobs P;
     for (int q = 0; q < njob; ++q) {
-        if (!jobs[q].w || !jobs[q].out) return DAGNN_EINVAL;
+        if (!jobs[q].w || !jobs[q].out || jobs[q].transposed < 0 || jobs[q].transposed > DF_PACK_PROJ16) return DAGNN_EINVAL;
+        if (jobs[q].transposed == DF_PACK_PROJ16 && H > 256) return DAGNN_EINVAL;
         if (jobs[q].transposed == 2 && (!jobs[q].aux || jobs[q].rows <= 0 || jobs[q].cols <= 0 || jobs[q].cols > 256)) return DAGNN_EINVAL;
         P.j[q] = jobs[q];
     }
@@ -1441,6 +1692,8 @@
     S.status = (const int32_t*)a->plan_status;
     const int32_t* plan = (const int32_t*)pl->data;
     unsigned grid = (unsigned)(df_sets_for(G) * nc * (H / DF_JS));
+    S.pshare = (H > 256 || (a->num_cus > 0 && (int64_t)df_sets_for(G) * nc * (H / DF_JS) <= a->num_cus)) ? 1 : 2;
+    const bool shared = H <= 256 && S.pshare > 1;
     S.nroles = 0; S.xcc_tab = (gran_t*)a->xcc_table;
     if (a->num_cus >= 8 && a->num_cus <= DF_MAX_WGS && a->xcc_table && df_sets_for(G) < 64 && nc <= 31) {
         const int NS = H / DF_JS, sets = df_sets_for(G), cap = a->num_cus / 8;
@@ -1449,7 +1702,21 @@
         for (int b = 0; b < DF_MAX_WGS; ++b) S.role[b] = DF_IDLE_ROLE;
         bool ok = true;
         int top = 0;
-        for (int pass = 0; pass < 2 && ok; ++pass)
+        for (int pp = 0; shared && 2 * pp < sets && ok; ++pp)
+            for (int c = 0; c < nc && ok; ++c) {
+                if (S.cell[c].kind != DF_RECURRENT || S.cell[c].partner < 0) continue;
+                const int nset = 2 * pp + 1 < sets ? 2 : 1;
+                int x = 0;
+                while (x < 8 && fill[x] + NS * (nset + 1) > cap) ++x;
+                if (x == 8) { ok = false; break; }
+                for (int m = 0; m <= nset; ++m)
+                    for (int sl = 0; sl < NS; ++sl) {
+                        const int b = fill[x]++ * 8 + (x + xrot) % 8;
+                        S.role[b] = (unsigned short)(m < nset ? ((2 * pp + m) << 10) | (c << 5) | sl : (pp << 10) | (S.cell[c].partner << 5) | sl);
+                        if (b + 1 > top) top = b + 1;
+                    }
+            }
+        for (int pass = shared ? 1 : 0; pass < 2 && ok; ++pass)
             for (int set = 0; set < sets && ok; ++set)
                 for (int c = 0; c < nc && ok; ++c) {
                     if (S.cell[c].kind != DF_RECURRENT || (S.cell[c].partner >= 0) != (pass == 0)) continue;
@@ -1473,9 +1740,9 @@
 #define DF_LAUNCH(KPT)                                                                                                   \
     do {                                                                                                                 \
         const void* fn = reinterpret_cast<const void*>(dataflow_kernel<KPT>);                                            \
-        const hipError_t ea = hipFuncSetAttribute(fn, hipFuncAttributeMaxDynamicSharedMemorySize, (int)df_lds_bytes<KPT>()); \
+        const hipError_t ea = hipFuncSetAttribute(fn, hipFuncAttributeMaxDynamicSharedMemorySize, (int)df_lds_total<KPT>()); \
         if (ea != hipSuccess) return DAGNN_EHIP(ea);                                                                     \
-        hipLaunchKernelGGL((dataflow_kernel<KPT>), dim3(grid), dim3(DF_THREADS), df_lds_bytes<KPT>(), st, plan, S);      \
+        hipLaunchKernelGGL((dataflow_kernel<KPT>), dim3(grid), dim3(DF_THREADS), df_lds_total<KPT>(), st, plan, S);      \
     } while (0)
 #if defined(DF_WIDE_TU)
     DF_LAUNCH(20);
diff --git a/dagnn_amd/engine.py b/dagnn_amd/engine.py
--- a/dagnn_amd/engine.py
+++ b/dagnn_amd/engine.py
@@ -473,6 +473,18 @@
     return out
 
 
+PACK_PROJ16 = 3
+
+
+def pack_dataflow_proj(w: torch.Tensor, H: int) -> torch.Tensor:
+    w = _dev(w, "weight", torch.float32)
+    if tuple(w.shape) != (3 * H, H):
+        raise DagnnHipError("pack_dataflow_proj needs a [3H, H] matrix, got %s" % (tuple(w.shape),))
+    out = torch.empty(3 * H * H, dtype=torch.float32, device=w.device)
+    check(_lib.load().dagnn_pack_dataflow_proj(w.data_ptr(), out.data_ptr(), H, _stream(w)), "dagnn_pack_dataflow_proj")
+    return out
+
+
 def pack_dataflow_batch(mats, H: int, gains=()):
     lib = _lib.load()
     outs, jobs, keep = [], [], []
@@ -483,7 +495,7 @@
         o = torch.empty(3 * H * H, dtype=torch.float32, device=w.device)
         keep.append(w)
         outs.append(o)
-        jobs.append(_lib.DfPackJob(w.data_ptr(), o.data_ptr(), None, 1 if tr else 0, 0, 0))
+        jobs.append(_lib.DfPackJob(w.data_ptr(), o.data_ptr(), None, int(tr), 0, 0))
     for ew, key, out in gains:
         ew, key = _dev(ew, "edge_encoder.weight", torch.float32), _dev(key, "key weights", torch.float32)
         keep += [ew, key]
@@ -536,11 +548,17 @@
     return max(n - r, 8) if r > 0 else n
 
 
+PROJ_SHARE_STACKED = 2
+
+
 def dataflow_groups(device, num_dirs: int, num_stacked: int, H: int, B: int, training: bool = False) -> int:
     if not DATAFLOW or not (H <= 256 or (H == 320 and DF_WIDE)):
         return 0
     cus = effective_cus(device, training)
-    g = _lib.load().dagnn_dataflow_groups(cus, int(num_dirs), int(num_stacked), int(H), int(B))
+    lib = _lib.load()
+    g = lib.dagnn_dataflow_groups(cus, int(num_dirs), int(num_stacked), int(H), int(B))
+    if g > 0 and not training and int(num_stacked) == PROJ_SHARE_STACKED:
+        g = max(g, lib.dagnn_dataflow_groups_shared(cus, int(num_dirs), int(num_stacked), int(H), int(B)))
     return min(g, DF_GROUPS) if DF_GROUPS > 0 else g
 
 
diff --git a/dagnn_amd/host_plan.py b/dagnn_amd/host_plan.py
--- a/dagnn_amd/host_plan.py
+++ b/dagnn_amd/host_plan.py
@@ -180,6 +180,26 @@
 DF_RB = 4
 
 
+def dataflow_cus(sets: int, num_dirs: int, L: int, H: int) -> int:
+    psets = (sets + 1) // 2 if H <= 256 else sets
+    return num_dirs * (H // 32) * (L * sets + (L - 1) * psets)
+
+
+def pack_dataflow_proj_host(w: np.ndarray, H: int) -> np.ndarray:
+    w = np.asarray(w, dtype=np.float32).reshape(3 * H, H)
+    ns4 = H // 32
+    tc = np.arange(256)
+    unit = 16 * (tc >> 7) + (tc & 15)
+    k0 = ((tc >> 6) & 1) * (H // 2) + 4 * ((tc >> 4) & 3)
+    out = np.empty((H // 32, 3, ns4, 256, 4), dtype=np.float32)
+    for sl in range(H // 32):
+        for g in range(3):
+            for s in range(ns4):
+                for e in range(4):
+                    out[sl, g, s, :, e] = w[g * H + 32 * sl + unit, k0 + 16 * s + e]
+    return out.reshape(-1)
+
+
 def dataflow_layout(N: int, B: int, G: int) -> Dict[str, int]:
     o = 16
     L: Dict[str, int] = {}
diff --git a/include/dagnn_hip.h b/include/dagnn_hip.h
--- a/include/dagnn_hip.h
+++ b/include/dagnn_hip.h
@@ -193,6 +193,7 @@
 } dagnn_dataflow_args;
 
 int dagnn_dataflow_groups(int num_cus, int num_dirs, int num_stacked, int H, int64_t B);
+int dagnn_dataflow_groups_shared(int num_cus, int num_dirs, int num_stacked, int H, int64_t B);
 size_t dagnn_dataflow_bytes(int64_t N, int64_t B, int groups);
 int dagnn_dataflow_schedule(const dagnn_plan* plan , void* workspace, size_t workspace_bytes, int groups,
                             int cost_layer, int cost_row, const int32_t* plan_status , void* stream);
@@ -200,6 +201,7 @@
 int dagnn_dataflow_run_wide(const dagnn_plan* plan , const dagnn_dataflow_args* args , void* stream);
 int dagnn_pack_dataflow(const float* w , float* out , int H, void* stream);
 int dagnn_pack_dataflow_transposed(const float* w , float* out , int H, void* stream);
+int dagnn_pack_dataflow_proj(const float* w , float* out , int H, void* stream);
 typedef struct dagnn_df_pack_job {
     const float* w;
     float* out;
```

Measured after the change: 107,900, median of 6. 1.04x the previous value.
